# PacificBiosciences/pb-StarPhase

Measured on AMD Instinct MI355X. Metric: HiFi reads/sec diplotyped (HLA+CYP2D6), higher is better.
Workload: dtype int32; 1 GPU; BASELINE configs[1] + configs[2] as ONE sample per step: HLA-A/-B 10000 HiFi reads vs IMGT/HLA v0.14.1 (11,199 DNA alleles) + CYP2D6 2000 targeted reads (39 templates), the six configs[2] scenarios in turn; a new sample uploaded every step; reads -> diplotypes; hla_reads=10000, cyp2d6_reads=2000, cyp2d6_lanes=6, hla_lanes=2, cyp2d6_consensus=launch pairs

## Files before the change

### pb-starphase_amd/csrc/sp_consensus.hip

```cpp
#include "sp_internal.h"
#include <atomic>
#include <cstdlib>
#include "sp_wfa.hip.h"
#include <algorithm>
#include <cstddef>
#include <cstring>
#include <map>
#include <string>

namespace {

constexpr int CB = 64;
constexpr int CH = 32;
#ifndef SP_K8_WAVES
#define SP_K8_WAVES 8
#endif
#ifndef SP_K8_MIN_WAVES
#define SP_K8_MIN_WAVES 4
#endif
constexpr int CWAVES = SP_K8_WAVES;
#ifndef SP_K8_DBG_READS
#define SP_K8_DBG_READS 16384
#endif
#define SP_K8_DBG_LAUNCHES (4194304 / SP_K8_DBG_READS)
#ifndef SP_K8_CW
#define SP_K8_CW 256
#endif
constexpr int CW = SP_K8_CW;
static_assert(CW % 64 == 0 && CW >= 64 && CW <= 512, "window length");
constexpr int CWIN = 512;
constexpr int RWORDS = (2 * CW + 320) / 16;
constexpr int NQ = 56;
constexpr int NWORK = 4;
constexpr int MAXKIDS = 16;
constexpr int CLUSTER = 64;
constexpr int RSLICES = 16;
constexpr int RGROUP = 16;
constexpr int QSV = 2 * (CW + 1) * 5, QSL = 2 * CW * 4, QE = QSV + QSL + 2 * (CW + 1);
enum { F_ACTIVE = 1, F_FINISHED = 2, F_LOST = 4 };
enum { M_NONE = 0, M_INIT = 1, M_WINDOW = 2, M_EXPAND = 3 };

struct CWork {
    int32_t mode, done;
    int32_t node, in_slot;
    int32_t T, n, replay;
    int32_t dual, split_at;
    int32_t go[2];
    int32_t n_kids, pad;
    int32_t pre_go[2];
    int32_t kid_node[MAXKIDS];
    int8_t  kid_base[MAXKIDS][2];
    int8_t  kid_split[MAXKIDS];
    uint8_t spec[2][CW];
};
struct CNode {
    int32_t used, id, complete;
    int32_t T, cur;
    int32_t dual, split_at, stopped[2], len[2];
    int32_t n, a, q;
    int16_t have_out, la_valid;
    int32_t wcap;
    long long cost0;
    long long rest;
    long long rest_out;
    uint32_t ev[2][5];
    int32_t pex_n, pex_L;
    int8_t  pex_kid[MAXKIDS];
    int32_t pad_head[2];
    int32_t dc[CW + 1];
    uint8_t spec[2][CW];
    int32_t pad_[3];
    __device__ __forceinline__ long long cost_at(int j) const { return cost0 + (long long)dc[j]; }
};
constexpr int NODE_HEAD_WORDS = 40, NODE_WORDS = (int)(sizeof(CNode) / 4), NODE_TAPE_WORDS = NODE_WORDS - NODE_HEAD_WORDS;
static_assert(offsetof(CNode, dc) == 4 * NODE_HEAD_WORDS && sizeof(CNode) % 16 == 0, "CNode layout");
struct CSearch {
    int32_t threshold, farthest, next_id, best_node, inflight, max_queue, per_size, wo_constraint;
    int32_t windows, cut_windows, expansions, pops_mod;
    long long pops, best_final;
    long long ticks[4];
    long long step_ticks, gap_ticks, last_end;
    int32_t compound, compound_ok;
    long long gap_ctl_ticks;
    int32_t steps, side_windows, side_expansions, adopted;
#ifdef SP_K8_PF_PROBE
    int32_t pf_win, pf_replay, pf_exp, pf_pad;
    unsigned long long idle_mask;
#endif
};
struct ConsMeta { int32_t e, c0, flags, pad; };
struct ConsRes { int32_t best, dual, split_at, len1, len2, pad; };

constexpr int CMAXP = 24;
struct ConsParams {
    int n, first, first_block, n_blocks, rpw;
    int first_cluster, n_clusters;
    int acc_block;
    int min_count, delta, et, allow_dual, window, cmp_len; double min_af;
    int cap, cs;
    uint8_t* C;
    CWork* work; CSearch* srch; CNode* nodes;
    uint32_t* la;
    uint8_t* processed;
    uint8_t* out_cons;
    struct ConsRes* out_res; CSearch* out_srch;
};
struct ReadInfo { const uint32_t* w; const uint32_t* np; int n, off; int off0, pad; };
struct PlaceMemo { int valid, M, off, c0; uint32_t text[512 / 16 + 2]; };
template <int MAXP> struct ConsBatchT {
    ConsParams p[MAXP]; int n_prob;
    const ReadInfo* info;
    PlaceMemo* memo;
    uint16_t* H;
    ConsMeta* meta;
    unsigned long long* PV;
    uint32_t* PE;
    unsigned long long* PL;
    uint32_t* PC;
    uint32_t* PR;
    uint32_t* Q;
    unsigned long long* dbg;
    uint32_t* prog;
    unsigned long long* step_t;
    uint32_t* sync;
    uint32_t* ready;
    uint32_t step_cap;
    int total;
    int nside;
    int k8_compound;
};
template <> struct ConsBatchT<0> {
    const ConsParams* p; const int* block_prob; int n_prob;
    const ReadInfo* info; PlaceMemo* memo; uint16_t* H; ConsMeta* meta; unsigned long long* PV; uint32_t* PE; unsigned long long* PL; uint32_t* PC; uint32_t* PR; uint32_t* Q; unsigned long long* dbg; uint32_t* prog; unsigned long long* step_t; uint32_t* sync; uint32_t* ready; uint32_t step_cap; const int* cluster_prob; int total; int nside; int k8_compound;
};
struct ConsSetup { SeqSetView reads; const uint32_t* idx; const int32_t* offsets; int n, first, cmp_len, pad_; };

struct ReadView { const uint32_t* w; const uint32_t* np; int n; };

__device__ __forceinline__ int h_load(const uint16_t* H, size_t at) { const uint16_t v = H[at]; return v == 0xFFFF ? SP_NEG : (int)v; }
__device__ __forceinline__ void h_store(uint16_t* H, size_t at, int h) { H[at] = h < 0 ? (uint16_t)0xFFFF : (uint16_t)h; }

__device__ __forceinline__ int read_base(const ReadView& rv, int h) {
    const uint32_t sh = (uint32_t)(h & 15) << 1;
    if (rv.np && ((rv.np[h >> 4] >> sh) & 1u)) return 4;
    return (int)((rv.w[h >> 4] >> sh) & 3u);
}

__device__ __forceinline__ uint32_t vote_units(int d) { return d == 1 ? 12u : d == 2 ? 6u : d == 3 ? 4u : 3u; }

struct Dwfa { int H, e, c0, flags; };

template <class RB, class EXT>
__device__ __forceinline__ void dwfa_push_t(Dwfa& d, int n, RB rb, EXT extend, int T, int nb, int et, int lane) {
    const int k = lane - CH;
    if (d.H >= 0 && d.H + k == T - 1 && d.H < n && rb(d.H) == nb) d.H += 1;
    while (!__ballot(d.H >= 0 && d.H + k == T)) {
        const int c = d.H, up = spw::from_lower(d.H, SP_NEG), dn = spw::from_upper(d.H, SP_NEG);
        int best = SP_NEG;
        if (c >= 0 && c < n && c + k < T) best = c + 1;
        if (up >= 0 && up + k <= T && up + k >= 0 && up > best) best = up;
        if (dn >= 0 && dn < n && dn + 1 + k >= 0 && dn + 1 > best) best = dn + 1;
        if (!__ballot(best >= 0)) { d.flags |= F_LOST; return; }
        d.H = best; d.e += 1;
        extend(d, T);
    }
    if (et && __ballot(d.H == n)) d.flags |= F_FINISHED;
}

template <class EXT>
__device__ __forceinline__ void dwfa_catchup_t(Dwfa& d, int n, EXT extend, int span, int lane) {
    const int k = lane - CH;
    extend();
    while (!__ballot(d.H >= 0 && d.H + k == span)) {
        const int c = d.H, up = spw::from_lower(d.H, SP_NEG), dn = spw::from_upper(d.H, SP_NEG);
        int best = SP_NEG;
        if (c >= 0 && c < n && c + k < span) best = c + 1;
        if (up >= 0 && up + k <= span && up + k >= 0 && up > best) best = up;
        if (dn >= 0 && dn < n && dn + 1 + k >= 0 && dn + 1 > best) best = dn + 1;
        if (!__ballot(best >= 0)) { d.flags |= F_LOST; break; }
        d.H = best; d.e += 1;
        extend();
    }
}

template <class RB, class CA>
__device__ __noinline__ int find_start_scan(int rn, RB rb, CA ca, int off, int end, int W, int L, int lane) {
    const int ws = off - W > 0 ? off - W : 0, M = end - ws;
    if (L > rn) L = rn;
    if (M <= 0 || L <= 0 || off <= ws) return off < end ? off : end;
    unsigned long long peq[4];
    {
        const int code = lane < L ? rb(L - 1 - lane) : 7;
#pragma unroll
        for (int b = 0; b < 4; ++b) peq[b] = __ballot(code == b);
    }
    const int q = (M + CB - 1) / CB;
    const int jlo = lane * q + 1, jhi = min(M, jlo + q - 1);
    unsigned long long key = ~0ull;
    if (jlo <= M) {
        const unsigned long long ones = L == 64 ? ~0ull : ((1ull << L) - 1), top = 1ull << (L - 1);
        unsigned long long Pv = ones, Mv = 0;
        int score = L;
        const int centre = off - W / 2;
        for (int j = max(1, jlo - 2 * L); j <= jhi; ++j) {
            const int x = ca(end - j);
            const unsigned long long Eq = x == 0 ? peq[0] : x == 1 ? peq[1] : x == 2 ? peq[2] : peq[3];
            const unsigned long long Xv = Eq | Mv;
            const unsigned long long Xh = (((Eq & Pv) + Pv) ^ Pv) | Eq;
            unsigned long long Ph = Mv | ~(Xh | Pv), Mh = Pv & Xh;
            if (Ph & top) ++score; else if (Mh & top) --score;
            Ph <<= 1; Mh <<= 1;
            Pv = (Mh | ~(Xv | Ph)) & ones; Mv = Ph & Xv & ones;
            if (j >= jlo && j >= end - off) {
                const int p = end - j, dist = p > centre ? p - centre : centre - p;
                const unsigned long long kk = ((unsigned long long)score << 44) | ((unsigned long long)dist << 22) | (unsigned long long)p;
                key = kk < key ? kk : key;
            }
        }
    }
#pragma unroll
    for (int o = 32; o > 0; o >>= 1) { const unsigned long long other = __shfl_xor(key, o); key = other < key ? other : key; }
    return (int)(key & ((1ull << 22) - 1));
}

__device__ __noinline__ int find_start_diag(int pc, int L_, int M_, int off_, int end_, int W_, int lane, const uint32_t* tr_, uint8_t* score_) {
    const int L = __builtin_amdgcn_readfirstlane(L_), M = __builtin_amdgcn_readfirstlane(M_), off = __builtin_amdgcn_readfirstlane(off_), W = __builtin_amdgcn_readfirstlane(W_), end = __builtin_amdgcn_readfirstlane(end_);
    typedef __attribute__((address_space(3))) uint8_t lds_u8;
    spw::lds_cu32* tr = (spw::lds_cu32*)(uintptr_t)spw::lds_addr(tr_);
    lds_u8* score = (lds_u8*)(uintptr_t)spw::lds_addr(reinterpret_cast<const uint32_t*>(score_));
    const int i = lane + 1;
    int prev1 = i, prev2 = i;
    uint32_t tw = tr[0], tw_next = tw;
    const bool last_row = lane == L - 1;
    for (int d = 1; d <= L + M; ++d) {
        const int j = d - i;
        const int up = spw::from_lower(prev1, 0), diag = spw::from_lower(prev2, 0);
        if (j >= 1 && ((j - 1) & 15) == 0) tw = tw_next;
        int cur = i;
        if (j >= 1 && j <= M) {
            const int tc = (int)((tw >> (((j - 1) & 15) << 1)) & 3u);
            const int a = diag + (pc != tc ? 1 : 0), bmin = (up < prev1 ? up : prev1) + 1;
            cur = a < bmin ? a : bmin;
            if (last_row) score[j - 1] = (uint8_t)cur;
        }
        if (j >= 0 && (j & 15) == 0) tw_next = tr[j >> 4];
        prev2 = prev1; prev1 = cur;
    }
    spw::wave_lds_sync();
    const int centre = off - W / 2;
    unsigned long long key = ~0ull;
    for (int j = end - off + lane; j <= M; j += SP_WAVE) {
        if (j < 1) continue;
        const int p = end - j, dist = p > centre ? p - centre : centre - p;
        const unsigned long long kk = ((unsigned long long)score[j - 1] << 44) | ((unsigned long long)dist << 22) | (unsigned long long)p;
        key = kk < key ? kk : key;
    }
#pragma unroll
    for (int o = 32; o > 0; o >>= 1) { const unsigned long long other = __shfl_xor(key, o); key = other < key ? other : key; }
    return (int)(key & ((1ull << 22) - 1));
}

__device__ __noinline__ int find_start_diag2(int pa, int pb, int L_, int M_, int off_, int end_, int W_, int lane, const uint32_t* tr_, uint8_t* score_) {
    const int L = __builtin_amdgcn_readfirstlane(L_), M = __builtin_amdgcn_readfirstlane(M_), off = __builtin_amdgcn_readfirstlane(off_), W = __builtin_amdgcn_readfirstlane(W_), end = __builtin_amdgcn_readfirstlane(end_);
    typedef __attribute__((address_space(3))) uint8_t lds_u8;
    spw::lds_cu32* tr = (spw::lds_cu32*)(uintptr_t)spw::lds_addr(tr_);
    lds_u8* score = (lds_u8*)(uintptr_t)spw::lds_addr(reinterpret_cast<const uint32_t*>(score_));
    const int ia = 2 * lane + 1, ib = ia + 1;
    int a1 = ia, a2 = ia, b1 = ib, b2 = ib;
    uint32_t tw = tr[0], tw_next = tw;
    int t_prev = 0;
    for (int d = 1; d <= L + M; ++d) {
        const int ja = d - ia, jb = ja - 1;
        const int up_a = spw::from_lower(b1, 0), diag_a = spw::from_lower(b2, 0);
        if (ja >= 1 && ((ja - 1) & 15) == 0) tw = tw_next;
        int cur_a = ia, cur_b = ib, tc = 0;
        if (ja >= 1 && ja <= M) {
            tc = (int)((tw >> (((ja - 1) & 15) << 1)) & 3u);
            const int x = diag_a + (pa != tc ? 1 : 0), y = (up_a < a1 ? up_a : a1) + 1;
            cur_a = x < y ? x : y;
            if (ia == L) score[ja - 1] = (uint8_t)cur_a;
        }
        if (jb >= 1 && jb <= M) {
            const int x = a2 + (pb != t_prev ? 1 : 0), y = (a1 < b1 ? a1 : b1) + 1;
            cur_b = x < y ? x : y;
            if (ib == L) score[jb - 1] = (uint8_t)cur_b;
        }
        if (ja >= 0 && (ja & 15) == 0) tw_next = tr[ja >> 4];
        t_prev = tc;
        a2 = a1; a1 = cur_a; b2 = b1; b1 = cur_b;
    }
    spw::wave_lds_sync();
    const int centre = off - W / 2;
    unsigned long long key = ~0ull;
    for (int j = end - off + lane; j <= M; j += SP_WAVE) {
        if (j < 1) continue;
        const int p = end - j, dist = p > centre ? p - centre : centre - p;
        const unsigned long long kk = ((unsigned long long)score[j - 1] << 44) | ((unsigned long long)dist << 22) | (unsigned long long)p;
        key = kk < key ? kk : key;
    }
#pragma unroll
    for (int o = 32; o > 0; o >>= 1) { const unsigned long long other = __shfl_xor(key, o); key = other < key ? other : key; }
    return (int)(key & ((1ull << 22) - 1));
}

constexpr int ACT_CONS = 512;
constexpr int ACT_READ = 2 * (CW + 1) > 640 ? ((2 * (CW + 1) + 63) / 64) * 64 : 640;
struct ActScratch {
    uint8_t rcache[ACT_READ];
    uint32_t cpack[ACT_CONS / 16 + 2];
    uint32_t rpack[ACT_READ / 16 + 2];
    uint32_t npack[ACT_READ / 16 + 2];
    uint8_t score[ACT_CONS];
    const uint32_t* staged;
#ifdef SP_K8_TIMING
    long long tk[4];
#endif
};


template <class T> __device__ __forceinline__ T coh_load(const T* p) { return __hip_atomic_load(p, __ATOMIC_RELAXED, __HIP_MEMORY_SCOPE_AGENT); }
template <class T> __device__ __forceinline__ void coh_store(T* p, T v) { __hip_atomic_store(p, v, __ATOMIC_RELAXED, __HIP_MEMORY_SCOPE_AGENT); }
template <class T> __device__ __forceinline__ void put(T* p, T v, bool coh) { if (coh) coh_store(p, v); else *p = v; }

struct ConsAccess {
    const uint8_t* win; int w0; const uint8_t* C; int cap, split_at, i, ov_pos, ov_base;
    const uint32_t* pk;
    __device__ __forceinline__ bool word16(int pos, uint32_t& out) const {
        const int y = pos - w0;
        if (y < 0 || y + 16 > CWIN + CW || (ov_pos >= pos && ov_pos < pos + 16)) return false;
        out = __builtin_amdgcn_alignbit(pk[(y >> 4) + 1], pk[y >> 4], (uint32_t)(y & 15) << 1);
        return true;
    }
    __device__ __forceinline__ int at(int pos) const {
        if (pos == ov_pos) return ov_base;
        const int y = pos - w0;
        if ((unsigned)y < (unsigned)(CWIN + CW)) return (int)win[y];
        return (int)coh_load((i == 1 && pos < split_at) ? &C[pos] : &C[(size_t)i * cap + pos]);
    }
};

__device__ __noinline__ Dwfa activate_late(ReadView rv, ConsAccess cacc, ActScratch* Ap, PlaceMemo* memo, int off, int len, int window, int cmp_len, int et, int lane) {
    ActScratch& A = *Ap;
    typedef __attribute__((address_space(3))) uint32_t lds_u32;
    typedef __attribute__((address_space(3))) uint8_t lds_u8;
    lds_u32* const L_rpack = (lds_u32*)(uintptr_t)spw::lds_addr(A.rpack);
    lds_u32* const L_npack = (lds_u32*)(uintptr_t)spw::lds_addr(A.npack);
    lds_u32* const L_cpack = (lds_u32*)(uintptr_t)spw::lds_addr(A.cpack);
    lds_u32* const L_score32 = (lds_u32*)(uintptr_t)spw::lds_addr(reinterpret_cast<const uint32_t*>(A.score));
    lds_u8* const L_rcache = (lds_u8*)(uintptr_t)spw::lds_addr(reinterpret_cast<const uint32_t*>(A.rcache));
    Dwfa d;
#ifdef SP_K8_TIMING
    long long tq = wall_clock64();
#define ACT_T(k) do { const long long _n = wall_clock64(); if (lane == 0) A.tk[k] += _n - tq; tq = _n; } while (0)
#else
#define ACT_T(k) do { } while (0)
#endif
    auto ca = [&](int pos) { return cacc.at(pos); };
    const int ws = off - window > 0 ? off - window : 0;
    if (A.staged != rv.w) {
        const int rwords0 = ((rv.n < ACT_READ ? rv.n : ACT_READ) + 15) >> 4;
        for (int w = lane; w < ACT_READ / 16 + 2; w += SP_WAVE) { L_rpack[w] = w < rwords0 ? rv.w[w] : 0u; L_npack[w] = (rv.np && w < rwords0) ? rv.np[w] : 0u; }
        spw::wave_lds_sync();
        for (int x = lane; x < rv.n && x < ACT_READ; x += SP_WAVE) {
            const uint32_t sh = (uint32_t)(x & 15) << 1;
            L_rcache[x] = ((L_npack[x >> 4] >> sh) & 1u) ? (uint8_t)4 : (uint8_t)((L_rpack[x >> 4] >> sh) & 3u);
        }
        if (lane == 0) A.staged = rv.w;
    }
    spw::wave_lds_sync();
    auto rbc = [&](int h) { return h < ACT_READ ? (int)L_rcache[h] : read_base(rv, h); };
    ACT_T(0);
    {
        const int ws0 = off - window > 0 ? off - window : 0, M = len - ws0, L = cmp_len < rv.n ? cmp_len : rv.n;
        if (M <= 0 || L <= 0 || off <= ws0) d.c0 = off < len ? off : len;
        else if (M > ACT_CONS) d.c0 = find_start_scan(rv.n, rbc, ca, off, len, window, cmp_len, lane);
        else {
            for (int w = lane; w < ((M + 15) >> 4) + 1; w += SP_WAVE) {
                uint32_t word = 0, fw;
                const int left = M - w * 16;
                if (left <= 0) word = 0;
                else if (cacc.word16(len - w * 16 - 16, fw)) {
                    fw = ((fw >> 2) & 0x33333333u) | ((fw & 0x33333333u) << 2);
                    fw = ((fw >> 4) & 0x0F0F0F0Fu) | ((fw & 0x0F0F0F0Fu) << 4);
                    word = __builtin_bswap32(fw);
                    if (left < 16) word &= (1u << (left << 1)) - 1u;
                }
                else for (int b = 0; b < 16; ++b) { const int j = w * 16 + b + 1; if (j <= M) word |= (uint32_t)(ca(len - j) & 3) << (b << 1); }
                L_cpack[w] = word;
            }
            spw::wave_lds_sync();
            const int nw = ((M + 15) >> 4) + 1;
            PlaceMemo* mm = memo + cacc.i;
            auto peek = [](const int* q) { return __hip_atomic_load(q, __ATOMIC_RELAXED, __HIP_MEMORY_SCOPE_AGENT); };
            const uint32_t seen = lane < nw ? (uint32_t)peek(reinterpret_cast<const int*>(&mm->text[lane])) : 0u;
            const int m_c0 = peek(&mm->c0), m_valid = peek(&mm->valid), m_M = peek(&mm->M), m_off = peek(&mm->off);
            bool known = m_valid && m_M == M && m_off == off;
            if (known) known = __ballot(lane < nw && seen != L_cpack[lane]) == 0;
            ACT_T(0);
            int exact_c0 = -1;
            constexpr int LV_MAX = 12;
            const int lv_nd = M - L + 1 + 2 * LV_MAX;
            if (!known && rv.np == nullptr && M >= L && lv_nd <= 8 * SP_WAVE) {
                lds_u32* const ppack = L_score32;
                const int npw = (L + 15) >> 4;
                if (lane < 10) {
                    uint32_t pw = 0;
                    if (lane < npw) for (int b = 0; b < 16; ++b) { const int u = lane * 16 + b; if (u < L) pw |= (uint32_t)(rbc(L - 1 - u) & 3) << (b << 1); }
                    ppack[lane] = pw;
                }
                spw::wave_lds_sync();
                const int npl = (lv_nd + SP_WAVE - 1) / SP_WAVE, centre = off - window / 2;
                auto slide = [&](int r, int dd) {
                    const int lim = L < M - dd ? L : M - dd;
                    while (r < lim) {
                        const int t = r + dd;
                        const uint32_t pwd = __builtin_amdgcn_alignbit(ppack[(r >> 4) + 1], ppack[r >> 4], (uint32_t)(r & 15) << 1);
                        const uint32_t twd = __builtin_amdgcn_alignbit(L_cpack[(t >> 4) + 1], L_cpack[t >> 4], (uint32_t)(t & 15) << 1);
                        const uint32_t diff = pwd ^ twd;
                        const int same = diff ? (__builtin_ctz(diff) >> 1) : 16;
                        r += same;
                        if (same < 16) break;
                    }
                    return r < lim ? r : lim;
                };
                int reach[8];
#pragma unroll
                for (int c = 0; c < 8; ++c) {
                    const int x = c * SP_WAVE + lane, dd = x - LV_MAX;
                    reach[c] = (c < npl && x < lv_nd && dd >= 0 && dd <= M) ? slide(0, dd) : -1;
                }
                for (int e = 0; e <= LV_MAX; ++e) {
                    unsigned long long key = ~0ull;
#pragma unroll
                    for (int c = 0; c < 8; ++c) {
                        const int x = c * SP_WAVE + lane, dd = x - LV_MAX;
                        if (c < npl && x < lv_nd && dd >= 0 && dd + L >= len - off && dd <= M - L && reach[c] >= L) {
                            const int p = len - dd - L, dist = p > centre ? p - centre : centre - p;
                            const unsigned long long kk = ((unsigned long long)dist << 22) | (unsigned long long)p;
                            key = kk < key ? kk : key;
                        }
                    }
#pragma unroll
                    for (int o = 32; o > 0; o >>= 1) { const unsigned long long other = __shfl_xor(key, o); key = other < key ? other : key; }
                    if (key != ~0ull) { exact_c0 = (int)(key & ((1ull << 22) - 1)); break; }
                    if (e == LV_MAX) break;
                    int nxt[8];
#pragma unroll
                    for (int c = 0; c < 8; ++c) {
                        nxt[c] = -1;
                        if (c < npl) {
                            const int x = c * SP_WAVE + lane, dd = x - LV_MAX;
                            int left = __shfl_up(reach[c], 1), up = __shfl_down(reach[c], 1);
                            const int wrap_l = c > 0 ? __shfl(reach[c > 0 ? c - 1 : 0], SP_WAVE - 1) : -1, wrap_u = c + 1 < 8 ? __shfl(reach[c + 1 < 8 ? c + 1 : 7], 0) : -1;
                            if (lane == 0) left = wrap_l;
                            if (lane == SP_WAVE - 1) up = (c + 1 < npl) ? wrap_u : -1;
                            int best = reach[c] >= 0 ? reach[c] + 1 : -1;
                            if (up >= 0 && up + 1 > best) best = up + 1;
                            if (left > best) best = left;
                            if (x < lv_nd && dd <= M && best >= 0) {
                                const int lim = L < M - dd ? L : M - dd;
                                nxt[c] = slide(best < lim ? best : lim, dd);
                            }
                        }
                    }
#pragma unroll
                    for (int c = 0; c < 8; ++c) reach[c] = nxt[c];
                }
                spw::wave_lds_sync();
            }
            if (known) d.c0 = m_c0;
            else if (exact_c0 >= 0) {
                d.c0 = exact_c0;
                if (lane < nw) mm->text[lane] = L_cpack[lane];
                if (lane == 0) { mm->valid = 1; mm->M = M; mm->off = off; mm->c0 = d.c0; }
            }
            else {
                if (L <= SP_WAVE) d.c0 = find_start_diag(lane < L ? rbc(L - 1 - lane) : 7, L, M, off, len, window, lane, A.cpack, A.score);
                else d.c0 = find_start_diag2(2 * lane + 1 <= L ? rbc(L - 2 * lane - 1) : 7, 2 * lane + 2 <= L ? rbc(L - 2 * lane - 2) : 7, L, M, off, len, window, lane, A.cpack, A.score);
                if (lane < nw) mm->text[lane] = L_cpack[lane];
                if (lane == 0) { mm->valid = 1; mm->M = M; mm->off = off; mm->c0 = d.c0; }
            }
            spw::wave_lds_sync();
        }
    }
    ACT_T(1);
    d.H = lane == CH ? 0 : SP_NEG; d.e = 0; d.flags = F_ACTIVE | ((et && rv.n == 0) ? F_FINISHED : 0);
    const int c0 = d.c0, span = len - c0, cwinlen = len - ws;
    const bool packed = rv.np == nullptr && cwinlen <= ACT_CONS;
    if (span > 0 && !(d.flags & F_FINISHED) && !(et && rv.n <= span + CB) && packed) {
        for (int w = lane; w < ACT_CONS / 16 + 2; w += SP_WAVE) {
            uint32_t word = 0;
            const int left = cwinlen - w * 16;
            if (left <= 0) word = 0;
            else if (cacc.word16(ws + w * 16, word)) { if (left < 16) word &= (1u << (left << 1)) - 1u; }
            else { word = 0; for (int b = 0; b < 16; ++b) { const int x = w * 16 + b; if (x < cwinlen) word |= (uint32_t)(ca(ws + x) & 3) << (b << 1); } }
            L_cpack[w] = word;
        }
        spw::wave_lds_sync();
        ACT_T(2);
        const int kk = lane - CH, cbase = c0 - ws;
        dwfa_catchup_t(d, rv.n, [&]() {
            for (;;) {
                int left = rv.n - d.H; { const int l2 = span - (d.H + kk); left = l2 < left ? l2 : left; }
                const bool go = d.H >= 0 && left > 0;
                int nm = 0;
                if (go) {
                    const int pr = d.H, pc = cbase + d.H + kk;
                    const uint32_t a = __builtin_amdgcn_alignbit(L_rpack[(pr >> 4) + 1], L_rpack[pr >> 4], (uint32_t)(pr & 15) << 1);
                    const uint32_t b = __builtin_amdgcn_alignbit(L_cpack[(pc >> 4) + 1], L_cpack[pc >> 4], (uint32_t)(pc & 15) << 1);
                    const uint32_t x = a ^ b, mm = (x | (x >> 1)) & 0x55555555u;
                    nm = mm ? (__builtin_ctz(mm) >> 1) : 16;
                    nm = nm < left ? nm : left;
                    d.H += nm;
                }
                if (!__ballot(go && nm == 16 && left > 16)) break;
            }
        }, span, lane);
    } else if (span > 0 && !(d.flags & F_FINISHED) && !(et && rv.n <= span + CB)) {
        const int kk = lane - CH;
        dwfa_catchup_t(d, rv.n, [&]() {
            for (;;) {
                bool go = d.H >= 0 && d.H < rv.n && d.H + kk < span;
                if (go) { const int x = rbc(d.H); go = x < 4 && x == ca(d.c0 + d.H + kk); }
                if (!__ballot(go)) break;
                if (go) d.H += 1;
            }
        }, span, lane);
    } else {
        for (int Tl = 1; Tl <= span; ++Tl) {
            if (d.flags & (F_FINISHED | F_LOST)) break;
            dwfa_push_t(d, rv.n, rbc, [&](Dwfa& x, int Tc) {
                const int kk = lane - CH;
                for (;;) {
                    bool go = x.H >= 0 && x.H < rv.n && x.H + kk < Tc;
                    if (go) { const int b = rbc(x.H); go = b < 4 && b == ca(x.c0 + x.H + kk); }
                    if (!__ballot(go)) break;
                    if (go) x.H += 1;
                }
            }, Tl, ca(c0 + Tl - 1), et, lane);
        }
    }
    ACT_T(3);
    return d;
}

constexpr int KID_LA_KIDS = 4, KID_LA = CW / KID_LA_KIDS;
#ifndef SP_K8_KID_W0
#define SP_K8_KID_W0 32
#endif
constexpr int KID_W0 = SP_K8_KID_W0 < KID_LA ? SP_K8_KID_W0 : KID_LA;
#ifndef SP_K8_RAMP
#define SP_K8_RAMP 2
#endif
#ifndef SP_K8_KID_CALM
#define SP_K8_KID_CALM 6
#endif
constexpr int KID_CALM = SP_K8_KID_CALM;
struct UsedWords {
    int used, has_la, a_end, b_end, total;
    __device__ __forceinline__ UsedWords(int mode, int n, int n_kids) {
        used = mode == M_EXPAND ? n_kids : (mode == M_WINDOW ? n + 1 + n_kids : 1);
        has_la = mode != M_EXPAND || n_kids <= KID_LA_KIDS;
        a_end = 2 * used * 5; b_end = a_end + (has_la ? QSL : 0); total = b_end + 2 * used;
    }
    __device__ __forceinline__ int at(int c) const {
        if (c < a_end) { const int i = c / (used * 5), rem = c % (used * 5); return (i * (CW + 1) + rem / 5) * 5 + rem % 5; }
        if (c < b_end) return QSV + (c - a_end);
        const int r = c - b_end;
        return r < used ? QSV + QSL + r : QSV + QSL + (CW + 1) + (r - used);
    }
};
template <class BT> __device__ __forceinline__ uint32_t block_word(const BT& B, size_t blk, int o) {
    constexpr int EV = 2 * (CW + 1), EL = 2 * CW, EC = CW + 1;
    if (o < QSV) { const int e = o / 5, f = o % 5; return f < 4 ? (uint32_t)((B.PV[blk * EV + e] >> (16 * f)) & 0xFFFFull) : B.PE[blk * EV + e]; }
    if (o < QSV + QSL) { const int e = (o - QSV) / 4, f = (o - QSV) % 4; return (uint32_t)((B.PL[blk * EL + e] >> (16 * f)) & 0xFFFFull); }
    if (o < QSV + QSL + EC) return B.PC[blk * EC + (o - QSV - QSL)];
    return B.PR[blk * EC + (o - QSV - QSL - EC)];
}
#ifndef SP_K8_WRAMP0
#define SP_K8_WRAMP0 64
#endif
constexpr int WRAMP0 = SP_K8_WRAMP0;
constexpr int BULK_MARGIN_PLACED = 2;
constexpr int BULK_MARGIN = 8;
#ifndef SP_K8_AUTO_BATCHES
#define SP_K8_AUTO_BATCHES 1
#endif
constexpr int PERSIST_AUTO_BATCHES = SP_K8_AUTO_BATCHES;
#ifndef SP_K8_LIGHT
#define SP_K8_LIGHT 64
#endif
constexpr int PERSIST_LIGHT = SP_K8_LIGHT;
#ifndef SP_K8_DIRECT_BLOCKS
#define SP_K8_DIRECT_BLOCKS (680 * 8 / SP_K8_WAVES)
#endif
constexpr int DIRECT_BLOCKS = SP_K8_DIRECT_BLOCKS;
constexpr int32_t SP_K8_AGAIN = -777;
constexpr int PERSIST_BLOCKS = 128 * 8 / CWAVES;

template <int MAXP> __device__ __forceinline__ int block_problem(const ConsBatchT<MAXP>& B, int block) {
    int pi = 0;
    if constexpr (MAXP == 0) pi = B.block_prob[block];
    else {
#pragma unroll
        for (int i = 1; i < MAXP; ++i) if (i < B.n_prob && block >= B.p[i].first_block) pi = i;
    }
    return pi;
}
template <int MAXP> __device__ __forceinline__ int block_problem(const ConsBatchT<MAXP>& B) { return block_problem<MAXP>(B, (int)blockIdx.x); }

__device__ __forceinline__ size_t state_plane(int node, int slot, int cons) { return (size_t)((node * 2 + slot) * 2 + cons); }

__device__ __forceinline__ int read_cost(const Dwfa& a0, const Dwfa& a1, bool dualrun) {
    int c = -1;
    if (a0.flags & F_ACTIVE) c = a0.e;
    if (dualrun && (a1.flags & F_ACTIVE) && (c < 0 || a1.e < c)) c = a1.e;
    return c < 0 ? 0 : c;
}

template <int MAXP>
__device__ __forceinline__ void cons_step_body(const ConsBatchT<MAXP>& B, const int wrow) {
    __shared__ unsigned long long lv[2][CW + 1];
    __shared__ uint32_t le[2][CW + 1];
    __shared__ unsigned long long ll[2][CW];
    __shared__ uint32_t lc[CW + 1], lr[CW + 1];
    __shared__ uint8_t cwin[2][CWIN + CW];
    __shared__ uint32_t rwin[CWAVES][2][RWORDS + 2];
    __shared__ uint32_t cpk[2][(CWIN + CW) / 16 + 2];
    __shared__ ActScratch act[CWAVES];
    __shared__ CWork wk_s;
    const int pi = block_problem<MAXP>(B);
    const ConsParams P = B.p[pi];
    const bool coh = B.sync != nullptr;
    if (coh) {
        for (int x = threadIdx.x; x < (int)(sizeof(CWork) / 4); x += blockDim.x) ((uint32_t*)&wk_s)[x] = coh_load(((const uint32_t*)P.work) + x);
        __syncthreads();
    }
    const CWork* Wp = coh ? &wk_s : P.work + wrow;
    const int mode = Wp->mode;
    if (P.work->done || mode == M_NONE) return;
    if (wrow > 0 && P.n_blocks > DIRECT_BLOCKS) return;
    if (B.step_t && threadIdx.x == 0) atomicMin(&B.step_t[2 * pi], (unsigned long long)wall_clock64());
    const int lane = threadIdx.x & 63, wave = threadIdx.x >> 6;
    const int T = Wp->T, n = (mode == M_WINDOW || mode == M_EXPAND) ? Wp->n : 0;
    const int pre = mode == M_EXPAND ? n : 0;
    const int node = Wp->node, in_slot = Wp->in_slot;
    const int dual_in = Wp->dual, split_at = Wp->split_at;
    const int go0 = Wp->go[0], go1 = Wp->go[1];
    const int n_kids = (mode == M_EXPAND || mode == M_WINDOW) ? Wp->n_kids : 0;
    const uint8_t* Cn = P.C + (size_t)node * 2 * P.cs;
    for (int x = threadIdx.x; x < 2 * (CW + 1); x += blockDim.x) { (&lv[0][0])[x] = 0; (&le[0][0])[x] = 0; }
    for (int x = threadIdx.x; x < 2 * CW; x += blockDim.x) (&ll[0][0])[x] = 0;
    for (int x = threadIdx.x; x < CW + 1; x += blockDim.x) { lc[x] = 0; lr[x] = 0; }
    const int w0 = T - CWIN;
    for (int x = threadIdx.x; x < 2 * (CWIN + CW); x += blockDim.x) {
        const int i = x / (CWIN + CW), y = x % (CWIN + CW), pos = w0 + y;
        uint8_t v = 0;
        if (pos >= T) v = (pos - T < n) ? Wp->spec[dual_in ? i : 0][pos - T] : 0;
        else if (pos >= 0) v = coh_load((i == 1 && dual_in && pos >= split_at) ? &Cn[(size_t)P.cs + pos] : &Cn[pos]);
        cwin[i][y] = v;
    }
    __syncthreads();
    constexpr int CPW = (CWIN + CW) / 16 + 2;
    for (int x = threadIdx.x; x < 2 * CPW; x += blockDim.x) {
        const int i = x / CPW, w = x % CPW;
        uint32_t word = 0;
        for (int b = 0; b < 16; ++b) { const int y = w * 16 + b; if (y < CWIN + n) word |= (uint32_t)(cwin[i][y] & 3u) << (b << 1); }
        cpk[i][w] = word;
    }
    __syncthreads();
    const size_t plane = (size_t)B.total;
    for (int rr = 0; rr < P.rpw; ++rr) {
        const int r = (((int)blockIdx.x - P.first_block) * CWAVES + wave) * P.rpw + rr;
        if (r >= P.n) break;
        const size_t g = (size_t)P.first + r;
#ifdef SP_K8_TIMING
        const long long wt0 = wall_clock64();
        if (lane == 0) { act[wave].tk[0] = act[wave].tk[1] = act[wave].tk[2] = act[wave].tk[3] = 0; }
#endif
        const ReadInfo ri = B.info[g];
        ReadView rv; rv.w = ri.w; rv.np = ri.np; rv.n = ri.n;
        if (lane == 0) act[wave].staged = nullptr;
        Dwfa d0, d1;
        d0.H = SP_NEG; d0.e = 0; d0.c0 = 0; d0.flags = 0; d1 = d0;
        if (mode == M_INIT) {
            if (ri.off < 0) { d0.flags = F_ACTIVE | ((P.et && rv.n == 0) ? F_FINISHED : 0); d0.H = lane == CH ? 0 : SP_NEG; }
        } else {
            const size_t p0 = state_plane(node, in_slot, 0) * plane + g;
            const ConsMeta m0 = B.meta[p0];
            d0.H = h_load(B.H, p0 * CB + lane); d0.e = m0.e; d0.c0 = m0.c0; d0.flags = m0.flags;
            if (dual_in) {
                const size_t p1 = state_plane(node, in_slot, 1) * plane + g;
                const ConsMeta m1 = B.meta[p1];
                d1.H = h_load(B.H, p1 * CB + lane); d1.e = m1.e; d1.c0 = m1.c0; d1.flags = m1.flags;
            }
        }
        int rbase = 0;
        {
            int lo = 0x7FFFFFFF;
            if (d0.flags & F_ACTIVE) { const int x = T - d0.c0 - CB; lo = x < lo ? x : lo; }
            if (dual_in && (d1.flags & F_ACTIVE)) { const int x = T - d1.c0 - CB; lo = x < lo ? x : lo; }
            if (lo == 0x7FFFFFFF || lo < 0) lo = 0;
            rbase = (lo >> 4) << 4;
            const int w_first = rbase >> 4, w_last = (rv.n + 15) >> 4;
            if (lane < RWORDS + 2) {
                const int w = w_first + lane;
                rwin[wave][0][lane] = w <= w_last + 1 ? rv.w[w] : 0u;
                rwin[wave][1][lane] = (rv.np && w <= w_last + 1) ? rv.np[w] : 0u;
            }
            spw::wave_lds_sync();
        }
        auto rb = [&](int h) -> int {
            const int x = h - rbase;
            if ((unsigned)x < (unsigned)(RWORDS * 16)) {
                const uint32_t sh = (uint32_t)(x & 15) << 1;
                if ((rwin[wave][1][x >> 4] >> sh) & 1u) return 4;
                return (int)((rwin[wave][0][x >> 4] >> sh) & 3u);
            }
            return read_base(rv, h);
        };
        auto vote = [&](const Dwfa& a, const Dwfa& o, bool dualrun, int i, int col, int slot) {
            if (!(a.flags & F_ACTIVE) || (a.flags & (F_FINISHED | F_LOST))) return;
            if (dualrun && (o.flags & F_ACTIVE) && !(o.flags & F_LOST) && o.e < a.e) return;
            const int Tl = col - a.c0, k = lane - CH;
            const bool tip = a.H >= 0 && a.H + k == Tl;
            const int code = (tip && a.H < rv.n) ? rb(a.H) : 5;
            int dc = 0; unsigned long long word = 0;
#pragma unroll
            for (int b = 0; b < 4; ++b) { const bool s = __ballot(code == b) != 0; dc += s; word |= s ? (1ull << (16 * b)) : 0ull; }
            const bool ended = __ballot(tip) != 0 && __ballot(code == 4) == 0;
            if (lane == 0) {
                if (dc) atomicAdd(&lv[i][slot], word * vote_units(dc));
                else if (ended) atomicAdd(&le[i][slot], 12u);
            }
        };
        bool use_pk = mode == M_WINDOW;
        auto extender = [&](const ConsAccess& cacc, int i) {
            return [&cacc, i, &rb, wave, rbase, w0, lane, &use_pk, &rv](Dwfa& d, int Tc) {
                const int k = lane - CH;
                for (;;) {
                    int left = rv.n - d.H; { const int l2 = Tc - (d.H + k); left = l2 < left ? l2 : left; }
                    const bool go = d.H >= 0 && left > 0;
                    int nm = 0; bool more = false;
                    if (go) {
                        const int xr = d.H - rbase, yc = d.c0 + d.H + k - w0;
                        if (use_pk && xr >= 0 && xr < RWORDS * 16 && yc >= 0 && yc < CWIN + CW) {
                            const uint32_t a = __builtin_amdgcn_alignbit(rwin[wave][0][(xr >> 4) + 1], rwin[wave][0][xr >> 4], (uint32_t)(xr & 15) << 1);
                            const uint32_t nn = __builtin_amdgcn_alignbit(rwin[wave][1][(xr >> 4) + 1], rwin[wave][1][xr >> 4], (uint32_t)(xr & 15) << 1);
                            const uint32_t b = __builtin_amdgcn_alignbit(cpk[i][(yc >> 4) + 1], cpk[i][yc >> 4], (uint32_t)(yc & 15) << 1);
                            const uint32_t xo = a ^ b, mm = ((xo | (xo >> 1)) | nn) & 0x55555555u;
                            nm = mm ? (__builtin_ctz(mm) >> 1) : 16;
                            nm = nm < left ? nm : left;
                            more = nm == 16 && left > 16;
                        } else {
                            const int x = rb(d.H);
                            nm = (x < 4 && x == cacc.at(d.c0 + d.H + k)) ? 1 : 0;
                            more = nm == 1 && left > 1;
                        }
                        d.H += nm;
                    }
                    if (!__ballot(more)) break;
                }
            };
        };
        auto column = [&](Dwfa& a0, Dwfa& a1, bool dualrun, int g0, int g1, int nb0, int nb1, int len, const ConsAccess& c0a, const ConsAccess& c1a) {
            if (g0) {
                if (a0.flags & F_ACTIVE) { if (!(a0.flags & (F_FINISHED | F_LOST))) dwfa_push_t(a0, rv.n, rb, extender(c0a, c0a.i), len - a0.c0, nb0, P.et, lane); }
                else if (ri.off == len) { a0 = activate_late(rv, c0a, &act[wave], B.memo + 2 * ((size_t)wrow * plane + g), ri.off0, len, P.window, P.cmp_len, P.et, lane); spw::wave_lds_sync(); }
            }
            if (dualrun && g1) {
                if (a1.flags & F_ACTIVE) { if (!(a1.flags & (F_FINISHED | F_LOST))) dwfa_push_t(a1, rv.n, rb, extender(c1a, c1a.i), len - a1.c0, nb1, P.et, lane); }
                else if (ri.off == len) { a1 = activate_late(rv, c1a, &act[wave], B.memo + 2 * ((size_t)wrow * plane + g), ri.off0, len, P.window, P.cmp_len, P.et, lane); spw::wave_lds_sync(); }
            }
            if (dualrun) {
                const int both = (a0.flags & F_ACTIVE) && (a1.flags & F_ACTIVE) && !(a0.flags & F_LOST) && !(a1.flags & F_LOST);
                if (both) {
                    if (a0.e > a1.e + P.delta) a0.flags |= F_LOST;
                    else if (a1.e > a0.e + P.delta) a1.flags |= F_LOST;
                }
            }
        };
        auto final_extra = [&](const Dwfa& a0, const Dwfa& a1, bool dualrun, int len0, int len1) -> int {
            if (P.et) return 0;
            int best = -1;
#pragma unroll
            for (int i = 0; i < 2; ++i) {
                if (i == 1 && !dualrun) continue;
                const Dwfa& a = i ? a1 : a0;
                if (!(a.flags & F_ACTIVE)) continue;
                int s = a.e;
                if (!(a.flags & F_LOST)) {
                    const int k = lane - CH, Tl = (i ? len1 : len0) - a.c0;
                    int rest = (a.H >= 0 && a.H + k == Tl) ? rv.n - a.H : (1 << 30);
#pragma unroll
                    for (int o = 32; o > 0; o >>= 1) { const int other = __shfl_xor(rest, o); rest = other < rest ? other : rest; }
                    if (rest < (1 << 30)) s += rest;
                }
                if (best < 0 || s < best) best = s;
            }
            return best < 0 ? 0 : best - read_cost(a0, a1, dualrun);
        };
        auto store = [&](const Dwfa& a, int nd, int slot, int i) {
            const size_t p = state_plane(nd, slot, i) * plane + g;
            if (lane == 0) { ConsMeta m; m.e = a.e; m.c0 = a.c0; m.flags = a.flags; m.pad = 0; B.meta[p] = m; }
            h_store(B.H, p * CB + lane, a.H);
        };
        ConsAccess ca0, ca1;
        ca0.win = &cwin[0][0]; ca0.w0 = w0; ca0.C = Cn; ca0.cap = P.cs; ca0.split_at = split_at; ca0.i = 0; ca0.ov_pos = -1; ca0.ov_base = 0; ca0.pk = &cpk[0][0];
        ca1 = ca0; ca1.win = &cwin[1][0]; ca1.i = 1; ca1.pk = &cpk[1][0];

        auto win_pass = [&](Dwfa& d0, Dwfa& d1, const bool dualrun, const int go0, const int go1, const int n, const bool quiet) {
        if (!quiet && mode == M_INIT) { vote(d0, d1, false, 0, 0, 0); }
        auto match_run = [&](int x0, int i, int j0, int len) -> int {
            if (x0 < 0 || x0 + len + 16 > RWORDS * 16) return 0;
            const int nblk = (len + 15) >> 4;
            const int blk = lane < nblk ? lane : 0;
            const int x = x0 + (blk << 4), jj = j0 + (blk << 4);
            const uint32_t a = __builtin_amdgcn_alignbit(rwin[wave][0][(x >> 4) + 1], rwin[wave][0][x >> 4], (uint32_t)(x & 15) << 1);
            const uint32_t nn = __builtin_amdgcn_alignbit(rwin[wave][1][(x >> 4) + 1], rwin[wave][1][x >> 4], (uint32_t)(x & 15) << 1);
            const uint32_t b = __builtin_amdgcn_alignbit(cpk[i][CWIN / 16 + (jj >> 4) + 1], cpk[i][CWIN / 16 + (jj >> 4)], (uint32_t)(jj & 15) << 1);
            const uint32_t xr = a ^ b, mm = ((xr | (xr >> 1)) | nn) & 0x55555555u;
            int run = mm ? (__builtin_ctz(mm) >> 1) : 16;
            const int room = len - (blk << 4);
            run = run < room ? run : room;
            const unsigned long long stop = __ballot(lane < nblk && run < 16 && run < room);
            if (!stop) return len;
            const int t = __builtin_ctzll(stop);
            return (t << 4) + __builtin_amdgcn_readlane(run, t);
        };
        static_assert(sizeof(((ActScratch*)nullptr)->rcache) >= 2 * (CW + 1), "edit-count profile");
        uint16_t* const ewp = reinterpret_cast<uint16_t*>(act[wave].rcache);
        auto bulk_push = [&](Dwfa& d, int i, const ConsAccess& cacc, int Tl0, int cols, int jbase) -> bool {
            auto ext = extender(cacc, i);
            const int k = lane - CH, span = Tl0 + cols;
            int reached = Tl0;
            const bool record = jbase >= 0;
            if (record && lane == 0) ewp[jbase] = (uint16_t)d.e;
            for (;;) {
                ext(d, span);
                int far = spw::wave_max(d.H >= 0 ? d.H + k : -1);
                far = far < span ? far : span;
                if (record) for (int c = reached + 1 + lane; c <= far; c += SP_WAVE) ewp[jbase + c - Tl0] = (uint16_t)d.e;
                reached = far > reached ? far : reached;
                if (reached >= span) break;
                const int c = d.H, up = spw::from_lower(d.H, SP_NEG), dn = spw::from_upper(d.H, SP_NEG);
                int best = SP_NEG;
                if (c >= 0 && c < rv.n && c + k < span) best = c + 1;
                if (up >= 0 && up + k <= span && up + k >= 0 && up > best) best = up;
                if (dn >= 0 && dn < rv.n && dn + 1 + k >= 0 && dn + 1 > best) best = dn + 1;
                if (!__ballot(best >= 0)) return false;
                d.H = best; d.e += 1;
            }
            spw::wave_lds_sync();
            return true;
        };
        int bulk = -1;
        int wsave_H = 0, wsave_e = 0, wsave_j = 0;
        int want_bulk = BULK_MARGIN;
        int j = 0;
#ifdef SP_K8_TIMING
        int slow_cols = 0, multi_tip = 0, zero_run = 0, fast_iters = 0;
        long long tb_fast = 0, tb_col = 0, tb_vote = 0, tb_mark = 0, tb_bulk = 0;
#ifdef SP_K8_DBG_PARTS
        const long long tb_pre = wall_clock64() - wt0;
#define K8_T0() tb_mark = wall_clock64()
#define K8_T(acc) do { const long long _n = wall_clock64(); acc += _n - tb_mark; tb_mark = _n; } while (0)
#else
#define K8_T0() tb_mark = clock64()
#define K8_T(acc) do { const long long _n = clock64(); acc += _n - tb_mark; tb_mark = _n; } while (0)
#endif
#else
#define K8_T0() do { } while (0)
#define K8_T(acc) do { } while (0)
#endif
        while (j < n) {
            K8_T0();
            if (want_bulk > 0) {
                const int margin = want_bulk; want_bulk = 0;
                if (!quiet && mode == M_WINDOW && dualrun && go0 && go1 && n - j >= 8 && (d0.flags & F_ACTIVE) && (d1.flags & F_ACTIVE) &&
                    !((d0.flags | d1.flags) & (F_FINISHED | F_LOST)) && (d0.e >= d1.e + margin || d1.e >= d0.e + margin)) {
                    const int wi = d0.e > d1.e ? 0 : 1;
                    Dwfa& w = wi ? d1 : d0;
                    const int Tl0 = T + j - w.c0;
                    if ((!P.et || rv.n > Tl0 + (n - j) + CB) && w.e < 60000) {
                        wsave_H = w.H; wsave_e = w.e; wsave_j = j;
                        if (bulk_push(w, wi, wi ? ca1 : ca0, Tl0, n - j, j)) { bulk = wi; w.e = wsave_e; }
                        else { w.H = wsave_H; w.e = wsave_e; }
                    }
                }
            }
            K8_T(tb_bulk);
            int m = n - j;
            int tl0 = -1, th0 = 0, tl1 = -1, th1 = 0;
#pragma unroll
            for (int i = 0; i < 2; ++i) {
                if (i == 1 && !dualrun) continue;
                if (!(i ? go1 : go0)) continue;
                if (i == bulk) continue;
                if (m == 0) continue;
                const Dwfa& a = i ? d1 : d0;
                if (a.flags & F_ACTIVE) {
                    if (a.flags & (F_FINISHED | F_LOST)) continue;
                    const int Tl = T + j - a.c0, k = lane - CH;
                    const unsigned long long tm = __ballot(a.H >= 0 && a.H + k == Tl);
                    if (__builtin_popcountll(tm) != 1) {
#ifdef SP_K8_TIMING
                        multi_tip += 1;
#endif
                        m = 0; continue; }
                    const int tl = __builtin_ctzll(tm), h = __builtin_amdgcn_readlane(a.H, tl);
                    int room = rv.n - h; room = room < m ? room : m;
                    const int run = room > 0 ? match_run(h - rbase, i, j, room) : 0;
                    m = run < m ? run : m;
                    if (i) { tl1 = tl; th1 = h; } else { tl0 = tl; th0 = h; }
                } else if (ri.off > T + j && ri.off <= T + n) {
                    const int before = ri.off - T - 1 - j;
                    m = before < m ? before : m;
                }
            }
            if (m > 0) {
#pragma unroll
                for (int i = 0; i < 2; ++i) {
                    const int tl = i ? tl1 : tl0, th = i ? th1 : th0;
                    if (tl < 0) continue;
                    Dwfa& a = i ? d1 : d0; const Dwfa& o = i ? d0 : d1;
                    bool speaks = true;
                    if (dualrun && (o.flags & F_ACTIVE) && !(o.flags & F_LOST) && o.e < a.e) speaks = false;
                    if (speaks && !quiet) for (int x = lane + 1; x <= m; x += SP_WAVE) {
                        const int pos = th + x;
                        if (pos < rv.n) { const int code = rb(pos); if (code < 4) atomicAdd(&lv[i][j + x], 12ull << (16 * code)); }
                        else if (!P.et) atomicAdd(&le[i][j + x], 12u);
                    }
                    if (lane == tl) a.H += m;
                    if (P.et && th + m == rv.n) a.flags |= F_FINISHED;
                }
                if (bulk >= 0) {
                    Dwfa& w = bulk ? d1 : d0; const Dwfa& b = bulk ? d0 : d1;
                    if (!(w.flags & F_LOST)) {
                        int hit = -1;
                        if (!(b.flags & F_LOST)) {
                            const int thr = b.e + P.delta;
                            for (int base = 0; base < m; base += SP_WAVE) {
                                const int x = j + 1 + base + lane;
                                const unsigned long long over = __ballot(x <= j + m && (int)ewp[x] > thr);
                                if (over) { hit = j + 1 + base + __builtin_ctzll(over); break; }
                            }
                        }
                        if (hit >= 0) { w.flags |= F_LOST; w.e = (int)ewp[hit]; } else w.e = (int)ewp[j + m];
                    }
                }
                j += m;
                K8_T(tb_fast);
#ifdef SP_K8_TIMING
                fast_iters += 1;
#endif
                continue;
            }
            K8_T(tb_fast);
#ifdef SP_K8_TIMING
            slow_cols += 1;
#endif
            const int before = read_cost(d0, d1, dualrun);
            const int active_before = (d0.flags & F_ACTIVE) + (d1.flags & F_ACTIVE);
            if (bulk >= 0) {
                Dwfa& w = bulk ? d1 : d0; const Dwfa& b = bulk ? d0 : d1;
                if (!(w.flags & F_LOST)) w.e = (int)ewp[j + 1];
                column(d0, d1, dualrun, bulk != 0, bulk != 1, cwin[0][CWIN + j], cwin[1][CWIN + j], T + j + 1, ca0, ca1);
                if (!(w.flags & F_LOST) && ((b.flags & F_LOST) || w.e <= b.e)) {
                    w.H = wsave_H; w.e = wsave_e;
                    (void)bulk_push(w, bulk, bulk ? ca1 : ca0, T + wsave_j - w.c0, j + 1 - wsave_j, -1);
                    bulk = -1;
                }
            } else
                column(d0, d1, dualrun, go0, go1, cwin[0][CWIN + j], cwin[1][CWIN + j], T + j + 1, ca0, ca1);
            const int grow = read_cost(d0, d1, dualrun) - before;
            if (grow && lane == 0 && !quiet) atomicAdd(&lc[j + 1], (uint32_t)grow);
            K8_T(tb_col);
            if (!quiet && go0 && bulk != 0) vote(d0, d1, dualrun, 0, T + j + 1, j + 1);
            if (!quiet && dualrun && go1 && bulk != 1) vote(d1, d0, dualrun, 1, T + j + 1, j + 1);
            K8_T(tb_vote);
            j += 1;
            if (bulk < 0 && (d0.flags & F_ACTIVE) + (d1.flags & F_ACTIVE) != active_before) want_bulk = BULK_MARGIN_PLACED;
        }
#pragma unroll
        for (int i = 0; i < 2; ++i) {
            if (quiet) continue;
            if (mode == M_WINDOW && n_kids > 0) continue;
            if (i == 1 && !dualrun) continue;
            if (mode != M_INIT && !(i ? go1 : go0)) continue;
            const Dwfa& a = i ? d1 : d0; const Dwfa& o = i ? d0 : d1;
            if (!(a.flags & F_ACTIVE) || (a.flags & (F_FINISHED | F_LOST))) continue;
            if (dualrun && (o.flags & F_ACTIVE) && !(o.flags & F_LOST) && o.e < a.e) continue;
            const int Tl = T + n - a.c0, k = lane - CH;
            unsigned long long tips = __ballot(a.H >= 0 && a.H + k == Tl && a.H < rv.n);
            for (int cnt = 0; tips && cnt < 2; ++cnt) {
                const int tl = __builtin_ctzll(tips); tips &= tips - 1;
                const int h = __builtin_amdgcn_readlane(a.H, tl);
                for (int x = lane; x < CW - 1 && h + 1 + x < rv.n; x += SP_WAVE) {
                    const int b = rb(h + 1 + x);
                    if (b < 4) atomicAdd(&ll[i][x], 1ull << (16 * b));
                }
            }
        }
        {
            const int len0 = go0 || mode == M_INIT ? T + n : coh_load(&P.nodes[node].len[0]), len1 = go1 ? T + n : coh_load(&P.nodes[node].len[1]);
            const int extra = final_extra(d0, d1, dualrun, len0, len1);
            if (extra && lane == 0 && !quiet) atomicAdd(&lr[n], (uint32_t)extra);
        }
        if (!quiet) {
            const int out_slot = mode == M_INIT ? in_slot : in_slot ^ 1;
            store(d0, node, out_slot, 0);
            if (dualrun) store(d1, node, out_slot, 1);
        }
        spw::wave_lds_sync();
#ifdef SP_K8_TIMING
#ifdef SP_K8_DBG_PARTS
        if (!quiet && B.dbg && lane == 0 && Wp->pad < SP_K8_DBG_LAUNCHES / 2 && g < SP_K8_DBG_READS) {
#else
        if (!quiet && B.dbg && lane == 0 && Wp->pad < SP_K8_DBG_LAUNCHES && g < SP_K8_DBG_READS) {
#endif
            const unsigned long long dt = (unsigned long long)(wall_clock64() - wt0);
            const unsigned long long placed = ri.off > T && ri.off <= T + n;
            auto cl = [](long long v, long long cap) { return (unsigned long long)(v > cap ? cap : v); };
#ifdef SP_K8_DBG_PARTS
            B.dbg[((size_t)Wp->pad * SP_K8_DBG_READS + g) * 2] = cl((long long)dt, 0xFFFFFF) | (cl(slow_cols, 511) << 24) | (cl(multi_tip, 511) << 33) | (placed << 42) | ((unsigned long long)mode << 43) |
                                                            (cl(n, 511) << 45);
            B.dbg[((size_t)Wp->pad * SP_K8_DBG_READS + g) * 2 + 1] = cl(tb_pre >> 1, 1023) | (cl(tb_fast >> 1, 4095) << 10) | (cl(tb_col >> 1, 4095) << 22) | (cl(tb_vote >> 1, 4095) << 34) |
                                                            (cl(tb_bulk >> 1, 4095) << 46) | (cl(fast_iters, 63) << 58);
            (void)tb_pre;
#elif defined(SP_K8_DBG_EDITS)
            B.dbg[(size_t)Wp->pad * SP_K8_DBG_READS + g] = cl((long long)dt, 0xFFFFFF) | (cl((act[wave].tk[0] + act[wave].tk[2]) >> 5, 511) << 24) | (cl(act[wave].tk[1] >> 5, 511) << 33) | (placed << 42) |
                                                            ((unsigned long long)mode << 43) | (cl(n, 511) << 45) | (cl(act[wave].tk[3] >> 5, 1023) << 54);
#else
            B.dbg[(size_t)Wp->pad * SP_K8_DBG_READS + g] = cl((long long)dt, 0xFFFFFF) | (cl(slow_cols, 511) << 24) | (cl(multi_tip, 511) << 33) | (placed << 42) | ((unsigned long long)mode << 43) |
                                                            (cl(n, 511) << 45) | (cl(tb_col >> 10, 1023) << 54);
#endif
            (void)tb_fast; (void)tb_vote; (void)tb_bulk; (void)fast_iters;
        }
#endif
        };
        auto expand_kids = [&](const Dwfa& d0, const Dwfa& d1, const int TB, const int s0) {
            const int base_cost = read_cost(d0, d1, dual_in != 0);
            for (int k = 0; k < n_kids; ++k) {
                Dwfa e0 = d0, e1 = d1;
                const int kb0 = Wp->kid_base[k][0], kb1 = Wp->kid_base[k][1], ksplit = Wp->kid_split[k];
                if (ksplit) e1 = e0;
                const bool kdual = dual_in || ksplit;
                ConsAccess k0 = ca0, k1 = ca1;
                k0.ov_pos = kb0 >= 0 ? TB : -1; k0.ov_base = kb0;
                k1.ov_pos = kb1 >= 0 ? TB : -1; k1.ov_base = kb1;
                if (ksplit) { k1.i = 0; }
                column(e0, e1, kdual, kb0 >= 0, kb1 >= 0, kb0, kb1, TB + 1, k0, k1);
                if (kb0 >= 0) vote(e0, e1, kdual, 0, TB + 1, s0 + k);
                if (kdual && kb1 >= 0) vote(e1, e0, kdual, 1, TB + 1, s0 + k);
                if (n_kids <= KID_LA_KIDS && (P.n < 256 || (r & 3) == 0)) {
#pragma unroll
                    for (int i = 0; i < 2; ++i) {
                        if (i == 1 && !kdual) continue;
                        if ((i ? kb1 : kb0) < 0) continue;
                        const Dwfa& a = i ? e1 : e0; const Dwfa& o = i ? e0 : e1;
                        if (!(a.flags & F_ACTIVE) || (a.flags & (F_FINISHED | F_LOST))) continue;
                        if (kdual && (o.flags & F_ACTIVE) && !(o.flags & F_LOST) && o.e < a.e) continue;
                        const int Tl = TB + 1 - a.c0, kd = lane - CH;
                        unsigned long long tips = __ballot(a.H >= 0 && a.H + kd == Tl && a.H < rv.n);
                        unsigned long long* const kl = &ll[0][0] + (size_t)(k * 2 + i) * KID_LA;
                        for (int cnt = 0; tips && cnt < 2; ++cnt) {
                            const int tl = __builtin_ctzll(tips); tips &= tips - 1;
                            const int h = __builtin_amdgcn_readlane(a.H, tl);
                            for (int x = lane; x < KID_LA - 1 && h + 1 + x < rv.n; x += SP_WAVE) {
                                const int b = rb(h + 1 + x);
                                if (b < 4) atomicAdd(&kl[x], 1ull << (16 * b));
                            }
                        }
                    }
                }
                const int grow = read_cost(e0, e1, kdual) - base_cost;
                const int len0 = kb0 >= 0 ? TB + 1 : (go0 ? TB : coh_load(&P.nodes[node].len[0]));
                const int len1 = kb1 >= 0 ? TB + 1 : (go1 ? TB : coh_load(&P.nodes[node].len[1]));
                const int extra = final_extra(e0, e1, kdual, len0, len1);
                if (lane == 0) { if (grow) atomicAdd(&lc[s0 + k], (uint32_t)grow); if (extra) atomicAdd(&lr[s0 + k], (uint32_t)extra); }
                const int kn = Wp->kid_node[k];
                store(e0, kn, 0, 0);
                if (kdual) store(e1, kn, 0, 1);
            }
            spw::wave_lds_sync();
        };
        if (mode == M_EXPAND) {
            if (pre > 0) { use_pk = true; win_pass(d0, d1, dual_in != 0, Wp->pre_go[0], Wp->pre_go[1], pre, true); use_pk = false; }
            expand_kids(d0, d1, T + pre, 0);
#ifdef SP_K8_DBG_PARTS
            if (B.dbg && lane == 0 && Wp->pad < SP_K8_DBG_LAUNCHES / 2 && g < SP_K8_DBG_READS) {
                const unsigned long long dt = (unsigned long long)(wall_clock64() - wt0);
                B.dbg[((size_t)Wp->pad * SP_K8_DBG_READS + g) * 2] = (dt > 0xFFFFFF ? 0xFFFFFFull : dt) | ((unsigned long long)(n_kids > 511 ? 511 : n_kids) << 24) | (3ull << 43) | ((unsigned long long)(pre > 511 ? 511 : pre) << 45);
                B.dbg[((size_t)Wp->pad * SP_K8_DBG_READS + g) * 2 + 1] = 0;
            }
#endif
            continue;
        }

        win_pass(d0, d1, dual_in != 0, go0, go1, n, false);
        if (n_kids > 0) {
            use_pk = false;
            if (lane == 0) act[wave].staged = nullptr;
            spw::wave_lds_sync();
            expand_kids(d0, d1, T + n, n + 1);
        }
    }
    __syncthreads();
    const UsedWords uw(mode, n, n_kids);
    if (P.n_blocks <= DIRECT_BLOCKS) {
        const size_t blk = (size_t)P.acc_block + (size_t)wrow;
        for (int x = threadIdx.x; x < 2 * uw.used; x += blockDim.x) {
            const int i = x / uw.used, e = i * (CW + 1) + x % uw.used;
            const unsigned long long v = (&lv[0][0])[e]; const uint32_t w = (&le[0][0])[e];
            if (v) atomicAdd(&B.PV[blk * 2 * (CW + 1) + e], v);
            if (w) atomicAdd(&B.PE[blk * 2 * (CW + 1) + e], w);
        }
        if (uw.has_la) for (int x = threadIdx.x; x < 2 * CW; x += blockDim.x) { const unsigned long long v = (&ll[0][0])[x]; if (v) atomicAdd(&B.PL[blk * 2 * CW + x], v); }
        for (int x = threadIdx.x; x < uw.used; x += blockDim.x) {
            if (lc[x]) atomicAdd(&B.PC[blk * (CW + 1) + x], lc[x]);
            if (lr[x]) atomicAdd(&B.PR[blk * (CW + 1) + x], lr[x]);
        }
        if (B.step_t && threadIdx.x == 0) atomicMax(&B.step_t[2 * pi + 1], (unsigned long long)wall_clock64());
        return;
    }
    for (int x = threadIdx.x; x < 2 * uw.used; x += blockDim.x) {
        const int i = x / uw.used, e = i * (CW + 1) + x % uw.used;
        B.PV[(size_t)blockIdx.x * 2 * (CW + 1) + e] = (&lv[0][0])[e];
        B.PE[(size_t)blockIdx.x * 2 * (CW + 1) + e] = (&le[0][0])[e];
    }
    if (uw.has_la) for (int x = threadIdx.x; x < 2 * CW; x += blockDim.x) B.PL[(size_t)blockIdx.x * 2 * CW + x] = (&ll[0][0])[x];
    for (int x = threadIdx.x; x < uw.used; x += blockDim.x) { B.PC[(size_t)blockIdx.x * (CW + 1) + x] = lc[x]; B.PR[(size_t)blockIdx.x * (CW + 1) + x] = lr[x]; }
    if (B.step_t && threadIdx.x == 0) atomicMax(&B.step_t[2 * pi + 1], (unsigned long long)wall_clock64());
}

template <int MAXP>
__global__ void __launch_bounds__(CWAVES * SP_WAVE, SP_K8_MIN_WAVES) cons_step_kernel(ConsBatchT<MAXP> B) { cons_step_body<MAXP>(B, (int)blockIdx.y); }
template <int MAXP>
__global__ void __launch_bounds__(CWAVES * SP_WAVE, 2) cons_step_wide_kernel(ConsBatchT<MAXP> B) { cons_step_body<MAXP>(B, (int)blockIdx.y); }

template <int MAXP>
__global__ void __launch_bounds__(512) cons_reduce_kernel(ConsBatchT<MAXP> B) {
    const int cluster = (int)blockIdx.x / RSLICES, slice = (int)blockIdx.x % RSLICES;
    int pi = 0;
    if constexpr (MAXP == 0) pi = B.cluster_prob[cluster];
    else {
#pragma unroll
        for (int i = 1; i < MAXP; ++i) if (i < B.n_prob && cluster >= B.p[i].first_cluster) pi = i;
    }
    const ConsParams P = B.p[pi];
    const int mode = P.work->mode;
    if (P.work->done || mode == M_NONE) return;
    const UsedWords uw(mode, mode == M_WINDOW ? P.work->n : 0, mode == M_EXPAND ? P.work->n_kids : 0);
    if (P.n_blocks <= DIRECT_BLOCKS) return;
    const int cl = cluster - P.first_cluster;
    const int members = P.n_blocks - cl * CLUSTER < CLUSTER ? P.n_blocks - cl * CLUSTER : CLUSTER;
    const size_t blk0 = (size_t)P.first_block + (size_t)cl * CLUSTER;
    constexpr int NG = CLUSTER / RGROUP;
    const int per = (uw.total + RSLICES - 1) / RSLICES;
    const int c_lo = slice * per, c_hi = c_lo + per < uw.total ? c_lo + per : uw.total;
    for (int idx = threadIdx.x; idx < (c_hi - c_lo) * NG; idx += blockDim.x) {
        const int o = uw.at(c_lo + idx / NG), m0 = (idx % NG) * RGROUP;
        uint32_t v[RGROUP];
#pragma unroll
        for (int m = 0; m < RGROUP; ++m) v[m] = m0 + m < members ? block_word(B, blk0 + m0 + m, o) : 0u;
        uint32_t sum = 0;
#pragma unroll
        for (int m = 0; m < RGROUP; ++m) sum += v[m];
#pragma unroll
        for (int d = 1; d < NG; d <<= 1) sum += __shfl_xor(sum, d);
        if (idx % NG == 0) B.Q[(size_t)cluster * QE + o] = sum;
    }
}

struct ColVotes { uint32_t w[4], end; };

__device__ __forceinline__ int col_candidates(const uint32_t* w5, int col, int cap, int et, int min_count, double min_af, int out[4]) {
    if (col >= cap) return 0;
    int order[4] = { 0, 1, 2, 3 };
#pragma unroll
    for (int a = 0; a < 4; ++a)
#pragma unroll
        for (int b = a + 1; b < 4; ++b) if (w5[order[b]] > w5[order[a]]) { const int t = order[a]; order[a] = order[b]; order[b] = t; }
    const uint32_t w1 = w5[order[0]], total = w5[0] + w5[1] + w5[2] + w5[3];
    const bool go = et ? w1 > 0 : (total > w5[4] && w1 > 0);
    if (!go) return 0;
    uint32_t need = 12u * (uint32_t)min_count; if (w1 < need) need = w1;
    int n = 0;
    out[n++] = order[0];
#pragma unroll
    for (int a = 1; a < 4; ++a) { const uint32_t w = w5[order[a]]; if (w > 0 && w >= need && (double)w >= min_af * (double)total) out[n++] = order[a]; }
    return n;
}

__device__ __forceinline__ int col_candidates_packed(const uint32_t* w5, int col, int cap, int et, int min_count, double min_af, uint32_t& packed) {
    packed = 0;
    if (col >= cap) return 0;
    uint32_t wa = w5[0], wb = w5[1], wc = w5[2], wd = w5[3]; uint32_t ca = 0, cb = 1, cc = 2, cd = 3;
#define SP_CSW(x, y, cx, cy) if (y > x) { const uint32_t tw_ = x; x = y; y = tw_; const uint32_t tc_ = cx; cx = cy; cy = tc_; }
    SP_CSW(wa, wb, ca, cb) SP_CSW(wa, wc, ca, cc) SP_CSW(wa, wd, ca, cd) SP_CSW(wb, wc, cb, cc) SP_CSW(wb, wd, cb, cd) SP_CSW(wc, wd, cc, cd)
#undef SP_CSW
    const uint32_t total = wa + wb + wc + wd;
    const bool go = et ? wa > 0 : (total > w5[4] && wa > 0);
    if (!go) return 0;
    uint32_t need = 12u * (uint32_t)min_count; if (wa < need) need = wa;
    int n = 1; packed = ca;
    const double floor_w = min_af * (double)total;
    if (wb > 0 && wb >= need && (double)wb >= floor_w) { packed |= cb << (2 * n); ++n; }
    if (wc > 0 && wc >= need && (double)wc >= floor_w) { packed |= cc << (2 * n); ++n; }
    if (wd > 0 && wd >= need && (double)wd >= floor_w) { packed |= cd << (2 * n); ++n; }
    return n;
}

template <int MAXP>
__device__ __forceinline__ void cons_control_body(const ConsBatchT<MAXP>& B) {
    extern __shared__ uint8_t proc[];
    __shared__ uint32_t acc[QE];
    uint32_t (*sv)[CW + 1][5] = reinterpret_cast<uint32_t (*)[CW + 1][5]>(acc);
    uint32_t (*sl)[CW][4] = reinterpret_cast<uint32_t (*)[CW][4]>(acc + QSV);
    uint32_t* sc = acc + QSV + QSL; uint32_t* sr = sc + (CW + 1);
    __shared__ CNode nh[NQ];
    __shared__ CWork wks[NWORK];
    __shared__ CSearch ss;
    __shared__ int copy_from[NWORK], copy_len[NWORK], need_la[NWORK], replay_of[NWORK];
    struct KidCopy { int from, T, n, nk, dual; int8_t node[4], b0[4], b1[4], sp[4]; uint8_t spec[2][CW]; };
    static_assert(KID_LA_KIDS <= 4, "KidCopy");
    __shared__ KidCopy kcopy[NWORK];
    const int pi = blockIdx.x;
    const ConsParams P = B.p[pi];
    const int tid = threadIdx.x;
    const bool coh = B.sync != nullptr;
    const int nside = (coh || P.n_blocks > DIRECT_BLOCKS) ? 0 : (B.nside < NWORK - 1 ? B.nside : NWORK - 1);
    const int n_orders = 1 + nside;
    CWork& wk = wks[0];
    const long long tk0 = wall_clock64();
    for (int x = tid; x < NQ * NODE_HEAD_WORDS; x += blockDim.x)
        ((uint32_t*)&nh[x / NODE_HEAD_WORDS])[x % NODE_HEAD_WORDS] = ((const uint32_t*)&P.nodes[x / NODE_HEAD_WORDS])[x % NODE_HEAD_WORDS];
    for (int x = tid; x < n_orders * (int)(sizeof(CWork) / 4); x += blockDim.x) ((uint32_t*)wks)[x] = ((const uint32_t*)P.work)[x];
    for (int x = tid; x < (int)(sizeof(CSearch) / 4); x += blockDim.x) ((uint32_t*)&ss)[x] = ((const uint32_t*)P.srch)[x];
    const int proc_words = (P.cap + 2 + 3) / 4;
    for (int x = tid; x < proc_words; x += blockDim.x) ((uint32_t*)proc)[x] = ((const uint32_t*)P.processed)[x];
    for (int x = tid; x < QE; x += blockDim.x) acc[x] = 0;
    if (tid < NWORK) { copy_from[tid] = -1; copy_len[tid] = 0; need_la[tid] = -1; replay_of[tid] = -1; kcopy[tid].nk = 0; if (tid >= n_orders) wks[tid].mode = M_NONE; }
    __syncthreads();
    if (wk.done) return;
    auto tape_word_used = [](const CNode& x, int w) {
        if (!x.used) return false;
        if (w == 0) return true;
        if (x.n <= 0) return false;
        if (w < CW + 1) return w <= x.n;
        const int sw = w - (CW + 1);
        return sw < 2 * (CW / 4) && (sw % (CW / 4)) * 4 < x.n;
    };
    for (int x = tid; x < NQ * NODE_TAPE_WORDS; x += blockDim.x) {
        const int k = x / NODE_TAPE_WORDS, w = x % NODE_TAPE_WORDS;
        if (tape_word_used(nh[k], w)) ((uint32_t*)&nh[k])[NODE_HEAD_WORDS + w] = ((const uint32_t*)&P.nodes[k])[NODE_HEAD_WORDS + w];
    }
    auto load_votes = [&](const int w) {
        const int mode_in = wks[w].mode, n_in = (mode_in == M_WINDOW || mode_in == M_EXPAND) ? wks[w].n : 0;
        if (mode_in == M_NONE) return;
        const UsedWords uw(mode_in, n_in, wks[w].n_kids);
        if (P.n_blocks <= DIRECT_BLOCKS) {
            const int u = uw.used, ev = 2 * u, el = uw.has_la ? 2 * CW : 0, E = ev + ev + el + u + u;
            const size_t blk = (size_t)P.acc_block + (size_t)w;
            for (int c = tid; c < E; c += blockDim.x) {
                if (c < ev || (c >= 2 * ev && c < 2 * ev + el)) {
                    const bool exact = c < ev;
                    const int e = exact ? (c / u) * (CW + 1) + c % u : c - 2 * ev;
                    unsigned long long* src = exact ? B.PV + blk * 2 * (CW + 1) + e : B.PL + blk * 2 * CW + e;
                    const unsigned long long sum = coh ? __hip_atomic_exchange(src, 0ull, __ATOMIC_RELAXED, __HIP_MEMORY_SCOPE_AGENT) : *src;
                    if (sum) {
                        if (!coh) *src = 0ull;
                        uint32_t* dst = exact ? acc + e * 5 : acc + QSV + e * 4;
#pragma unroll
                        for (int f = 0; f < 4; ++f) dst[f] = (uint32_t)((sum >> (16 * f)) & 0xFFFFull);
                    }
                } else {
                    uint32_t* src; uint32_t* dst;
                    if (c < 2 * ev) { const int cc = c - ev, e = (cc / u) * (CW + 1) + cc % u; src = B.PE + blk * 2 * (CW + 1) + e; dst = acc + e * 5 + 4; }
                    else if (c < 2 * ev + el + u) { const int e = c - 2 * ev - el; src = B.PC + blk * (CW + 1) + e; dst = acc + QSV + QSL + e; }
                    else { const int e = c - 2 * ev - el - u; src = B.PR + blk * (CW + 1) + e; dst = acc + QSV + QSL + (CW + 1) + e; }
                    const uint32_t sum = coh ? __hip_atomic_exchange(src, 0u, __ATOMIC_RELAXED, __HIP_MEMORY_SCOPE_AGENT) : *src;
                    if (sum) { if (!coh) *src = 0u; *dst = sum; }
                }
            }
        } else {
            const int parts = P.n_clusters;
            for (int c = tid; c < uw.total; c += blockDim.x) {
                const int o = uw.at(c);
                uint32_t sum = 0;
                for (int c0 = 0; c0 < parts; c0 += 8) {
                    uint32_t v[8];
#pragma unroll
                    for (int q = 0; q < 8; ++q) v[q] = c0 + q < parts ? B.Q[(size_t)(P.first_cluster + c0 + q) * QE + o] : 0u;
#pragma unroll
                    for (int q = 0; q < 8; ++q) sum += v[q];
                }
                acc[o] = sum;
            }
        }
    };
    const int lane = tid & (SP_WAVE - 1);
    auto cands = [&](const uint32_t* w5, int col, int out[4]) { return col_candidates(w5, col, P.cap, P.et, P.min_count, P.min_af, out); };
    auto node_free = [&](int k) {
        const int np = nh[k].pex_n;
        for (int j = 0; j < np; ++j) { CNode& c = nh[nh[k].pex_kid[j]]; c.used = 0; c.complete = 0; }
        nh[k].pex_n = 0; nh[k].used = 0; nh[k].complete = 0;
    };
    uint8_t* Cb = P.C;
    int la_fresh = -1;
    auto trim_queue = [&]() {
        for (;;) {
            const bool waits = lane < NQ && nh[lane].used == 1 && !nh[lane].complete;
            const int wlen = waits ? nh[lane].T + nh[lane].q : 0;
            const bool live = waits && wlen >= ss.threshold;
            if (waits && !live) node_free(lane);
            if (__builtin_popcountll(__ballot(live)) <= ss.max_queue) break;
            int shortest = live ? wlen : 0x7FFFFFFF;
#pragma unroll
            for (int o = 32; o > 0; o >>= 1) { const int other = __shfl_xor(shortest, o); shortest = other < shortest ? other : shortest; }
            if (lane == 0) ss.threshold = shortest + 1;
            spw::wave_lds_sync();
        }
    };
    auto adopt = [&](const int parent, const int n_kids, const bool kids_wait, auto kid) {
        const int others = __builtin_popcountll(__ballot(lane < NQ && nh[lane].used == 1 && !nh[lane].complete)) - 1 - (kids_wait ? n_kids : 0);
        const int kid_w0 = others <= KID_CALM ? KID_LA : KID_W0;
        if (lane < n_kids) {
            CNode& c = nh[kid(lane)];
            c.used = 1; c.id = ss.next_id + lane;
            c.wcap = n_kids <= KID_LA_KIDS ? kid_w0 : WRAMP0;
        }
        spw::wave_lds_sync();
        if (lane == 0) {
            ss.next_id += n_kids;
            nh[parent].pex_n = 0;
            node_free(parent);
            ss.expansions += 1;
        }
        spw::wave_lds_sync();
        trim_queue();
    };
    struct Plan { int kind, nk, nc0, nc1, cut, L; uint32_t cd0, cd1; bool ends; };
    auto cands_p = [&](const uint32_t* w5, int col, uint32_t& packed) { return col_candidates_packed(w5, col, P.cap, P.et, P.min_count, P.min_af, packed); };
    auto plan_of = [&](const CNode& x) -> Plan {
        Plan p;
        const bool has = x.q > 0 || x.n > 0, stood = !has || (x.a == x.n && x.have_out);
        p.cut = stood ? -1 : x.a;
        p.L = (has && stood ? x.T + x.n : x.T) + (p.cut > 0 ? p.cut : 0);
        p.nc0 = p.nc1 = 0; p.cd0 = p.cd1 = 0; p.ends = false;
        if (!x.stopped[0]) { p.nc0 = cands_p(x.ev[0], p.L, p.cd0); p.ends = p.ends || p.nc0 == 0; }
        if (x.dual && !x.stopped[1]) { p.nc1 = cands_p(x.ev[1], p.L, p.cd1); p.ends = p.ends || p.nc1 == 0; }
        if (!x.dual) p.nk = p.nc0 + (P.allow_dual ? p.nc0 * (p.nc0 - 1) / 2 : 0);
        else p.nk = (p.nc0 || p.nc1) ? (p.nc0 ? p.nc0 : 1) * (p.nc1 ? p.nc1 : 1) : 0;
        p.kind = p.nk == 0 ? 0 : p.nk == 1 ? 1 : 2;
        return p;
    };
    auto kid_of = [&](const Plan& pl, const int dual, const int k, int& b0, int& b1, int& sp) {
        auto code = [](uint32_t packed, int j) { return (int)((packed >> (2 * j)) & 3u); };
        sp = 0;
        if (!dual) {
            if (k < pl.nc0) { b0 = code(pl.cd0, k); b1 = -1; }
            else { int pa = 0, pb = 1; for (int j = pl.nc0; j < k; ++j) if (++pb >= pl.nc0) { ++pa; pb = pa + 1; } b0 = code(pl.cd0, pa); b1 = code(pl.cd0, pb); sp = 1; }
        } else { const int n1 = pl.nc1 ? pl.nc1 : 1, a2 = k / n1, b2 = k - a2 * n1; b0 = pl.nc0 ? code(pl.cd0, a2) : -1; b1 = pl.nc1 ? code(pl.cd1, b2) : -1; }
    };
    auto kids_from_sums = [&](const CWork& w, const int mark, const int L, const long long par_cost, const int my_j, const int s0) {
        if (my_j >= 0) {
            const CNode& par = nh[w.node];
            const int k = my_j;
            CNode& c = nh[w.kid_node[k]];
            c.used = mark; c.complete = 0; c.id = 0; c.T = L + 1; c.cur = 0; c.pex_n = 0; c.pex_L = 0;
            c.dual = par.dual || w.kid_split[k]; c.split_at = w.kid_split[k] ? L : par.split_at;
#pragma unroll
            for (int i = 0; i < 2; ++i) {
                const bool was_going = (i == 0 || par.dual) && !par.stopped[i];
                int st = par.stopped[i], ln = par.len[i];
                if (w.kid_base[k][i] >= 0) { st = 0; ln = L + 1; }
                else if (was_going) { st = 1; ln = L; }
                c.stopped[i] = st; c.len[i] = ln;
            }
            if (!c.dual) c.stopped[1] = 1;
            c.n = c.a = c.q = 0; c.have_out = 0; c.la_valid = w.n_kids <= KID_LA_KIDS ? 1 : 0; c.wcap = WRAMP0;
            c.cost0 = par_cost + (long long)sc[s0 + k]; c.dc[0] = 0; c.rest = sr[s0 + k]; c.rest_out = 0;
            for (int i = 0; i < 2; ++i) for (int bq = 0; bq < 5; ++bq) c.ev[i][bq] = sv[i][s0 + k][bq];
        }
        if (w.n_kids <= KID_LA_KIDS) {
            const uint32_t* flat = &sl[0][0][0];
            for (int y = lane; y < w.n_kids * 2 * KID_LA * 4; y += SP_WAVE) {
                const int k = y / (2 * KID_LA * 4), i = (y / (KID_LA * 4)) & 1, xb = y % (KID_LA * 4);
                P.la[(size_t)w.kid_node[k] * 2 * CW * 4 + (size_t)i * CW * 4 + xb] = flat[y];
            }
            __threadfence_block();
        }
        spw::wave_lds_sync();
    };
    auto take_result = [&](const int w) {
        const CWork& wo = wks[w];
        const int mode_in = wo.mode, n_in = (mode_in == M_WINDOW || mode_in == M_EXPAND) ? wo.n : 0;
        const bool side = w > 0;
        if (mode_in == M_INIT) {
            la_fresh = wo.node;
            CNode& x = nh[wo.node];
            if (lane == 0) {
                x.used = 1; x.id = ss.next_id++; x.complete = 0; x.T = 0; x.cur = wo.in_slot; x.dual = 0; x.split_at = -1;
                x.stopped[0] = 0; x.stopped[1] = 1; x.len[0] = x.len[1] = 0; x.n = x.a = x.q = 0; x.have_out = 0; x.la_valid = 1; x.wcap = CW;
                x.cost0 = 0; x.dc[0] = 0; x.rest = sr[0]; x.rest_out = 0; x.pex_n = 0; x.pex_L = 0;
            }
            if (lane < 10) x.ev[lane / 5][lane % 5] = sv[lane / 5][0][lane % 5];
            for (int y = lane; y < 2 * CW * 4; y += SP_WAVE) P.la[(size_t)wo.node * 2 * CW * 4 + y] = (&sl[0][0][0])[y];
        } else if (mode_in == M_WINDOW) {
            CNode& x = nh[wo.node];
            const int n = n_in, T = wo.T;
            int a = n;
            if (!wo.replay && n > 1) {
                for (int base = 0; base < n; base += SP_WAVE) {
                    const int col = base + lane;
                    bool ok = true;
                    if (col >= 1 && col < n) {
#pragma unroll
                        for (int i = 0; i < 2; ++i) {
                            if (i == 1 && !x.dual) continue;
                            if (!wo.go[i]) continue;
                            int c4[4];
                            const int nc = cands(sv[i][col], T + col, c4);
                            if (nc != 1 || c4[0] != wo.spec[i][col]) ok = false;
                        }
                    }
                    const unsigned long long bad = __ballot(!ok);
                    if (bad) { a = base + __builtin_ctzll(bad); break; }
                }
            }
            for (int col = lane; col < a; col += SP_WAVE) {
#pragma unroll
                for (int i = 0; i < 2; ++i) if ((i == 0 || x.dual) && wo.go[i]) put(&Cb[((size_t)wo.node * 2 + i) * P.cs + T + col], wo.spec[i][col], coh);
            }
            if (!wo.replay) {
                long long carry = 0;
                for (int base = 0; base < a; base += SP_WAVE) {
                    const int col = base + lane;
                    long long c = col < a ? (long long)sc[col + 1] : 0;
#pragma unroll
                    for (int o = 1; o < SP_WAVE; o <<= 1) { const long long up = __shfl_up(c, o); if (lane >= o) c += up; }
                    if (col < a) x.dc[col + 1] = (int32_t)(carry + c);
                    carry += __shfl(c, SP_WAVE - 1);
                }
                for (int col = lane; col < n; col += SP_WAVE) { x.spec[0][col] = wo.spec[0][col]; x.spec[1][col] = wo.spec[1][col]; }
            }
            if (lane < 10) x.ev[lane / 5][lane % 5] = sv[lane / 5][a][lane % 5];
            if (lane == 0) {
                ss.windows += 1; if (a < n) ss.cut_windows += 1;
                x.n = n; x.a = wo.replay ? n : a;
                x.have_out = (a == n) ? (wo.n_kids > 0 ? 2 : 1) : 0;
                if (a == n) x.rest_out = sr[n];
            }
            if (wo.n_kids > 0) {
                spw::wave_lds_sync();
                bool take = a == n && B.k8_compound != 2;
                int my_j = -1, nk = 0;
                if (take) {
                    Plan pl;
                    pl.nc0 = pl.nc1 = 0; pl.cd0 = pl.cd1 = 0; bool ends = false;
                    if (!x.stopped[0]) { pl.nc0 = cands_p(sv[0][n], T + n, pl.cd0); ends = ends || pl.nc0 == 0; }
                    if (x.dual && !x.stopped[1]) { pl.nc1 = cands_p(sv[1][n], T + n, pl.cd1); ends = ends || pl.nc1 == 0; }
                    if (!x.dual) nk = pl.nc0 + (P.allow_dual ? pl.nc0 * (pl.nc0 - 1) / 2 : 0);
                    else nk = (pl.nc0 || pl.nc1) ? (pl.nc0 ? pl.nc0 : 1) * (pl.nc1 ? pl.nc1 : 1) : 0;
                    take = !ends && nk >= 2 && nk <= wo.n_kids;
                    if (take) {
                        bool found = true;
                        if (lane < nk) {
                            int b0, b1, sp;
                            kid_of(pl, x.dual, lane, b0, b1, sp);
                            for (int j = 0; j < wo.n_kids; ++j) if (wo.kid_base[j][0] == b0 && wo.kid_base[j][1] == b1 && wo.kid_split[j] == sp) my_j = j;
                            found = my_j >= 0;
                        }
                        take = __ballot(!found) == 0;
                    }
                }
                if (take) {
                    kids_from_sums(wo, 2, T + n, x.cost_at(n), lane < nk ? my_j : -1, n + 1);
                    for (int k = 0; k < nk; ++k) { const int j = __builtin_amdgcn_readlane(my_j, k); if (lane == 0) x.pex_kid[k] = (int8_t)wo.kid_node[j]; }
                    if (lane < wo.n_kids) { bool mine = false; for (int k = 0; k < nk; ++k) mine = mine || __builtin_amdgcn_readlane(my_j, k) == lane; if (!mine) { nh[wo.kid_node[lane]].used = 0; nh[wo.kid_node[lane]].complete = 0; } }
                    if (lane == 0) {
                        x.pex_n = nk; x.pex_L = T + n; ss.compound_ok += 1;
                        KidCopy& kc = kcopy[w];
                        kc.from = wo.node; kc.T = T; kc.n = n; kc.nk = nk; kc.dual = x.dual;
                    }
                    if (lane < nk) { KidCopy& kc = kcopy[w]; kc.node[lane] = (int8_t)wo.kid_node[my_j]; kc.b0[lane] = wo.kid_base[my_j][0]; kc.b1[lane] = wo.kid_base[my_j][1]; kc.sp[lane] = wo.kid_split[my_j]; }
                    for (int col = lane; col < n; col += SP_WAVE) { kcopy[w].spec[0][col] = wo.spec[0][col]; kcopy[w].spec[1][col] = wo.spec[1][col]; }
                } else if (lane < wo.n_kids) { nh[wo.kid_node[lane]].used = 0; nh[wo.kid_node[lane]].complete = 0; }
                spw::wave_lds_sync();
            } else if (a == n) {
                if (!side) la_fresh = wo.node;
                for (int y = lane; y < 2 * CW * 4; y += SP_WAVE) P.la[(size_t)wo.node * 2 * CW * 4 + y] = (&sl[0][0][0])[y];
                if (side) __threadfence_block();
            }
        } else if (mode_in == M_EXPAND) {
#ifdef SP_K8_TRACE
            if (lane == 0 && pi == 0) { printf("EXP%s L %d pre %d kids %d parcost %lld :", side ? " (side)" : "", wo.T + n_in, n_in, wo.n_kids, nh[wo.node].cost_at(nh[wo.node].q)); for (int k = 0; k < wo.n_kids; ++k) printf(" [%d/%d sc %u sr %u ev %u %u %u %u %u]", wo.kid_base[k][0], wo.kid_base[k][1], sc[k], sr[k], sv[0][k][0], sv[0][k][1], sv[0][k][2], sv[0][k][3], sv[0][k][4]); printf("\n"); }
#endif
            const long long par_cost = nh[wo.node].cost_at(nh[wo.node].q);
            if (!side) {
                kids_from_sums(wo, 1, wo.T + n_in, par_cost, lane < wo.n_kids ? lane : -1, 0);
                adopt(wo.node, wo.n_kids, true, [&](int k) { return (int)wo.kid_node[k]; });
            } else {
                kids_from_sums(wo, 2, wo.T + n_in, par_cost, lane < wo.n_kids ? lane : -1, 0);
                if (lane == 0) {
                    CNode& par = nh[wo.node];
                    par.pex_n = wo.n_kids; par.pex_L = wo.T + n_in;
                    for (int k = 0; k < wo.n_kids; ++k) par.pex_kid[k] = (int8_t)wo.kid_node[k];
                }
            }
        }
        spw::wave_lds_sync();
    };
    auto copy_window_kids = [&](const int w) {
        const KidCopy& kc = kcopy[w];
        if (kc.nk <= 0) return;
        const int whole = kc.T >> 4, L = kc.T + kc.n;
        for (int k = 0; k < kc.nk; ++k) {
            const bool split = kc.sp[k] != 0;
            for (int i = 0; i < 2; ++i) {
                if (i == 1 && !(kc.dual || split)) continue;
                const int si = (i == 1 && split) ? 0 : i;
                const uint8_t* srow = P.C + ((size_t)kc.from * 2 + si) * P.cs;
                uint8_t* dst = P.C + ((size_t)kc.node[k] * 2 + i) * P.cs;
                for (int y = tid; y < whole; y += blockDim.x) reinterpret_cast<uint4*>(dst)[y] = reinterpret_cast<const uint4*>(srow)[y];
                for (int y = (whole << 4) + tid; y <= L; y += blockDim.x) {
                    int v;
                    if (y < kc.T) v = srow[y];
                    else if (y < L) v = kc.spec[kc.dual ? si : 0][y - kc.T];
                    else v = i ? kc.b1[k] : kc.b0[k];
                    if (v >= 0) dst[y] = (uint8_t)v;
                }
            }
        }
    };
    for (int w = n_orders - 1; w >= 0; --w) {
        if (wks[w].mode == M_NONE) continue;
        load_votes(w);
        __syncthreads();
        if (tid < SP_WAVE) take_result(w);
        __syncthreads();
        copy_window_kids(w);
        if (w > 0) {
            for (int x = tid; x < QE; x += blockDim.x) acc[x] = 0;
            __syncthreads();
        }
    }
    const long long tk1 = wall_clock64();
    long long tk2 = tk1, tk3 = tk1;
#ifdef SP_K8_SEARCH_TICKS
    long long ts_pick = 0, ts_block = 0, ts_iters = 0;
#endif
    if (tid < SP_WAVE) {
        tk2 = wall_clock64();
        if (lane == 0) { const int steps_made = wk.pad + 1; for (int w = 0; w < n_orders; ++w) { wks[w].mode = M_NONE; wks[w].n = 0; wks[w].replay = 0; wks[w].n_kids = 0; } wk.pad = steps_made; }
        spw::wave_lds_sync();
        auto act = [&](const int xi, const int w, const Plan& pl, unsigned long long& free_bits) -> int {
            CNode& x = nh[xi];
            CWork& W = wks[w];
            const bool side = w > 0;
            const int cut = pl.cut;
            if ((x.q > 0 || x.n > 0) && cut < 0) {
                const int xn = x.n;
                if (xn > 1) x.wcap = SP_K8_RAMP * x.wcap < CW ? SP_K8_RAMP * x.wcap : CW;
                const long long c_end = x.cost_at(xn);
                const int la_ok = x.have_out == 1 ? 1 : 0;
                x.T += xn; x.cur ^= 1; x.cost0 = c_end; x.dc[0] = 0; x.rest = x.rest_out; x.n = x.a = x.q = 0; x.have_out = 0; x.la_valid = la_ok;
            }
            const int dual = x.dual, cur = x.cur, split_at = x.split_at, xT = x.T;
            const int pre_go0 = !x.stopped[0] ? 1 : 0, pre_go1 = (dual && !x.stopped[1]) ? 1 : 0;
            auto order_replay = [&]() {
                W.mode = M_WINDOW; W.node = xi; W.in_slot = cur; W.T = xT; W.n = x.a; W.replay = 1;
                W.dual = dual; W.split_at = split_at; W.go[0] = pre_go0; W.go[1] = pre_go1;
                replay_of[w] = xi;
                ss.inflight = xi;
            };
#ifdef SP_K8_NO_PRE
            if (!side && cut >= 0 && (SP_K8_NO_PRE == 0 || (SP_K8_NO_PRE == 1 && dual) || (SP_K8_NO_PRE == 2 && !dual))) { order_replay(); return 1; }
#endif
            const int L = pl.L;
            if (!side) {
                if (!x.stopped[0] && pl.nc0 == 0) { x.stopped[0] = 1; x.len[0] = L; }
                if (dual && !x.stopped[1] && pl.nc1 == 0) { x.stopped[1] = 1; x.len[1] = L; }
            }
            if (pl.nk == 0) {
                if (cut >= 0) { order_replay(); return 1; }
                const long long fc = x.cost0 + (P.et ? 0 : x.rest);
                if (ss.best_node < 0 || fc < ss.best_final) { if (ss.best_node >= 0) node_free(ss.best_node); ss.best_node = xi; ss.best_final = fc; x.complete = 1; }
                else node_free(xi);
                return 0;
            }
            const int nc0 = pl.nc0, nc1 = pl.nc1;
            auto code = [](uint32_t packed, int j) { return (int)((packed >> (2 * j)) & 3u); };
            if (pl.nk == 1 && cut >= 0) { order_replay(); return 1; }
            if (pl.nk == 1) {
                const int b0 = nc0 ? code(pl.cd0, 0) : -1, b1 = (dual && nc1) ? code(pl.cd1, 0) : -1;
                W.mode = M_WINDOW; W.node = xi; W.in_slot = cur; W.T = L; W.replay = 0; W.dual = dual; W.split_at = split_at;
                W.go[0] = b0 >= 0; W.spec[0][0] = (uint8_t)(b0 >= 0 ? b0 : 0); W.go[1] = b1 >= 0; W.spec[1][0] = (uint8_t)(b1 >= 0 ? b1 : 0);
                need_la[w] = x.la_valid ? xi : -1;
                W.n = 1;
                x.n = 0; x.a = 0; x.q = 0;
                if (!side) ss.inflight = xi;
                return 1;
            }
            W.mode = M_EXPAND; W.node = xi; W.in_slot = cur; W.T = xT; W.n = cut > 0 ? cut : 0; W.dual = dual; W.split_at = split_at; W.replay = 0;
            W.go[0] = nc0 > 0; W.go[1] = nc1 > 0; W.pre_go[0] = pre_go0; W.pre_go[1] = pre_go1;
            if (cut > 0) replay_of[w] = xi;
            int made = 0;
            for (int k = 0; k < pl.nk && made < MAXKIDS; ++k) {
                if (!free_bits) break;
                int b0, b1, sp;
                kid_of(pl, dual, k, b0, b1, sp);
                const int kn = __builtin_ctzll(free_bits); free_bits &= free_bits - 1;
                nh[kn].used = side ? 2 : 1; nh[kn].complete = 0; nh[kn].pex_n = 0;
                W.kid_node[made] = kn; W.kid_base[made][0] = (int8_t)b0; W.kid_base[made][1] = (int8_t)b1; W.kid_split[made] = (int8_t)sp;
                ++made;
            }
            W.n_kids = made;
            copy_from[w] = xi; copy_len[w] = L;
            return 1;
        };
        unsigned long long main_kids = 0;
        for (int guard = 0; ; ++guard) {
            if (guard > 100000) { if (lane == 0) wk.done = 1; break; }
#ifdef SP_K8_SEARCH_TICKS
            const long long ts0 = wall_clock64(); ts_iters += 1;
#endif
            int xi = ss.inflight;
            if (xi < 0) {
                long long kc = 0x7FFFFFFFFFFFFFFFll; int kt = -1, kid = 0x7FFFFFFF, kx = -1;
                if (lane < NQ && nh[lane].used == 1 && !nh[lane].complete) { const CNode& p = nh[lane]; kc = p.cost_at(p.q); kt = p.T + p.q; kid = p.id; kx = lane; }
                auto less = [](long long c1, int t1, int i1, long long c2, int t2, int i2) { return c1 < c2 || (c1 == c2 && (t1 > t2 || (t1 == t2 && i1 < i2))); };
                long long bc = kc; int bt = kt, bid = kid, bx = kx;
                long long sc2 = 0x7FFFFFFFFFFFFFFFll; int st2 = -1, sid2 = 0x7FFFFFFF, sx2 = -1;
                const unsigned long long waiting = __ballot(kx >= 0);
                if (__builtin_popcountll(waiting) == 1) {
                    const int only = __builtin_ctzll(waiting);
                    bc = ((long long)__builtin_amdgcn_readlane((int)(kc >> 32), only) << 32) | (unsigned int)__builtin_amdgcn_readlane((int)kc, only);
                    bt = __builtin_amdgcn_readlane(kt, only); bid = __builtin_amdgcn_readlane(kid, only); bx = only;
                    xi = only;
                } else {
#pragma unroll
                    for (int o = 32; o > 0; o >>= 1) {
                        const long long oc = __shfl_xor(bc, o); const int ot = __shfl_xor(bt, o), oi = __shfl_xor(bid, o), ox = __shfl_xor(bx, o);
                        if (ox >= 0 && (bx < 0 || less(oc, ot, oi, bc, bt, bid))) { bc = oc; bt = ot; bid = oi; bx = ox; }
                    }
                    xi = bx;
                    if (xi < 0) { if (lane == 0) wk.done = 1; break; }
                    sc2 = (kx == xi) ? 0x7FFFFFFFFFFFFFFFll : kc; st2 = kt; sid2 = kid; sx2 = (kx == xi) ? -1 : kx;
#pragma unroll
                    for (int o = 32; o > 0; o >>= 1) {
                        const long long oc = __shfl_xor(sc2, o); const int ot = __shfl_xor(st2, o), oi = __shfl_xor(sid2, o), ox = __shfl_xor(sx2, o);
                        if (ox >= 0 && (sx2 < 0 || less(oc, ot, oi, sc2, st2, sid2))) { sc2 = oc; st2 = ot; sid2 = oi; sx2 = ox; }
                    }
                }
                CNode& x = nh[xi];
                if (ss.best_node >= 0 && bc >= ss.best_final) { if (lane == 0) wk.done = 1; break; }
                const int linear0 = x.a - x.q;
                bool again = false, freed = false;
                int Lc = bt;
                for (;;) {
                    const int L = Lc, q = x.q, a = x.a;
                    const int wo = ss.wo_constraint;
                    const int jc = wo - 1 - ss.pops_mod;
                    const int linear = a - q;
                    const int want = linear > 0 ? (linear < SP_WAVE ? linear : SP_WAVE) : 1;
                    bool can = lane < want && L + lane >= ss.threshold && proc[L + lane] < ss.per_size && lane <= jc;
                    if (can && (lane > 0 || again)) {
                        const long long cj = x.cost_at(q + lane);
                        can = (sx2 < 0 || less(cj, L + lane, ss.next_id + lane - 1, sc2, st2, sid2)) && !(ss.best_node >= 0 && cj >= ss.best_final);
                    }
                    const unsigned long long no = ~__ballot(can);
                    const int m = no ? __builtin_ctzll(no) : SP_WAVE;
                    if (m == 0) { if (!again) { if (lane == 0) node_free(xi); freed = true; } break; }
                    if (lane < m) proc[L + lane] += 1;
                    if (lane == 0) {
                        ss.pops += m;
                        { int pm = ss.pops_mod + m; if (pm >= wo) pm %= wo; ss.pops_mod = pm; }
                        if (L + m - 1 > ss.farthest) ss.farthest = L + m - 1;
                        if (jc < m && ss.farthest > ss.threshold) ss.threshold = ss.farthest;
                        if (linear > 0) { x.q = q + m; x.id = ss.next_id + m - 1; ss.next_id += m; }
                    }
                    spw::wave_lds_sync();
                    if (!(linear > 0 && m == SP_WAVE && q + m < a)) break;
                    again = true; Lc = L + m;
                }
                if (freed) { spw::wave_lds_sync(); continue; }
                if (linear0 > 0) continue;
            } else if (lane == 0) ss.inflight = -1;
            spw::wave_lds_sync();
            int stop = 0;
#ifdef SP_K8_SEARCH_TICKS
            const long long ts1 = wall_clock64(); ts_pick += ts1 - ts0;
#endif
            {
                const CNode& x = nh[xi];
                if (x.q < x.a) {
                    if (lane == 0) { nh[xi].q += 1; nh[xi].id = ss.next_id++; }
                    spw::wave_lds_sync();
                    continue;
                }
                if (x.pex_n > 0) {
                    const int np = x.pex_n;
                    if (lane == 0) ss.adopted += 1;
                    adopt(xi, np, false, [&](int k) { return (int)nh[xi].pex_kid[k]; });
                    continue;
                }
            }
            const unsigned long long free_before = __ballot(lane < NQ && !nh[lane].used);
            unsigned long long free_nodes = free_before;
            if (lane == 0) { const Plan pl = plan_of(nh[xi]); stop = act(xi, 0, pl, free_nodes); }
            stop = __builtin_amdgcn_readfirstlane(stop);
            free_nodes = ((unsigned long long)(unsigned int)__builtin_amdgcn_readfirstlane((int)(free_nodes >> 32)) << 32) | (unsigned int)__builtin_amdgcn_readfirstlane((int)free_nodes);
            main_kids = free_before & ~free_nodes;
            spw::wave_lds_sync();
#ifdef SP_K8_SEARCH_TICKS
            ts_block += wall_clock64() - ts1;
#endif
            if (stop) break;
        }
        spw::wave_lds_sync();
        if (lane == 0 && !wk.done && wk.mode != M_NONE) ss.steps += 1;
        if (nside > 0 && !wk.done && wk.mode != M_NONE && __builtin_popcountll(__ballot(lane < NQ && nh[lane].used == 1 && !nh[lane].complete)) > 1) {
            Plan pl; pl.kind = 0; pl.nk = 0;
            bool cand = false;
            long long kc = 0x7FFFFFFFFFFFFFFFll; int kt = -1, kid = 0x7FFFFFFF;
            if (lane < NQ && nh[lane].used == 1 && !nh[lane].complete && lane != wk.node && !((main_kids >> lane) & 1ull) && nh[lane].q >= nh[lane].a && nh[lane].pex_n == 0) {
                const CNode& x = nh[lane];
                const int Lq = x.T + x.q;
                if (Lq >= ss.threshold && Lq < P.cap + 2 && proc[Lq] < ss.per_size) {
                    pl = plan_of(x);
                    cand = !pl.ends && ((pl.kind == 1 && pl.cut < 0) || (pl.kind == 2 && pl.nk <= MAXKIDS));
                    if (cand) { kc = x.cost_at(x.q); kt = Lq; kid = x.id; }
                }
            }
            const unsigned long long cm = __ballot(cand);
            if (cm) {
                auto less = [](long long c1, int t1, int i1, long long c2, int t2, int i2) { return c1 < c2 || (c1 == c2 && (t1 > t2 || (t1 == t2 && i1 < i2))); };
                int my_rank = 0;
                for (unsigned long long m = cm; m; m &= m - 1) {
                    const int b = __builtin_ctzll(m);
                    const long long oc = ((long long)__builtin_amdgcn_readlane((int)(kc >> 32), b) << 32) | (unsigned int)__builtin_amdgcn_readlane((int)kc, b);
                    const int ot = __builtin_amdgcn_readlane(kt, b), oi = __builtin_amdgcn_readlane(kid, b);
                    if (b != lane && less(oc, ot, oi, kc, kt, kid)) ++my_rank;
                }
                const unsigned long long free_nodes = __ballot(lane < NQ && !nh[lane].used);
                const int hidden = __builtin_popcountll(__ballot(lane < NQ && nh[lane].used == 2)), n_free = __builtin_popcountll(free_nodes);
                const int room = NQ - (ss.max_queue + 1) - MAXKIDS;
                const int n_cand = __builtin_popcountll(cm);
                int my_w = 0, my_skip = 0, accepted = 0, taken = 0, n_sw = 0, n_se = 0;
                for (int r = 0; r < n_cand && accepted < nside; ++r) {
                    const unsigned long long who = __ballot(cand && my_rank == r);
                    if (!who) continue;
                    const int b = __builtin_ctzll(who);
                    const int bkind = __builtin_amdgcn_readlane(pl.kind, b), bnk = __builtin_amdgcn_readlane(pl.nk, b);
                    if (bkind == 2 && (hidden + taken + bnk > room || n_free - taken < bnk + MAXKIDS)) continue;
                    if (lane == b) { my_w = 1 + accepted; my_skip = taken; }
                    ++accepted;
                    if (bkind == 2) { taken += bnk; ++n_se; } else ++n_sw;
                }
                if (lane == 0) { ss.side_windows += n_sw; ss.side_expansions += n_se; }
                if (my_w > 0) {
                    unsigned long long mine = free_nodes;
                    for (int j = 0; j < my_skip; ++j) mine &= mine - 1;
                    (void)act(lane, my_w, pl, mine);
                }
            }
        }
        spw::wave_lds_sync();
        for (int w = 0; w < n_orders; ++w) {
            const int ro = replay_of[w];
            if (ro >= 0) {
                const CNode& x = nh[ro];
                for (int jq = lane; jq < x.a; jq += SP_WAVE) { wks[w].spec[0][jq] = x.spec[0][jq]; wks[w].spec[1][jq] = x.spec[1][jq]; }
            }
        }
#ifdef SP_K8_PF_PROBE
        if (wk.mode == M_WINDOW || wk.mode == M_EXPAND) {
            bool idle = lane < NQ && nh[lane].used == 1 && !nh[lane].complete && lane != wk.node && nh[lane].q >= nh[lane].a;
            if (wk.mode == M_EXPAND) for (int k = 0; k < wk.n_kids; ++k) if (wk.kid_node[k] == lane) idle = false;
            const unsigned long long mask = __ballot(idle);
            if (lane == 0) {
                if ((ss.idle_mask >> wk.node) & 1ull) { if (wk.mode == M_EXPAND) ss.pf_exp += 1; else if (wk.replay) ss.pf_replay += 1; else ss.pf_win += 1; }
                ss.idle_mask = mask;
            }
        }
#endif
        spw::wave_lds_sync();
        tk3 = wall_clock64();
        for (int w = 0; w < n_orders; ++w) {
            const int nl = need_la[w];
            if (nl < 0) continue;
            CWork& W = wks[w];
            const uint32_t* la = (w == 0 && nl == la_fresh) ? &sl[0][0][0] : P.la + (size_t)nl * 2 * CW * 4;
            const int lim = nh[nl].wcap;
            const int hidden = __builtin_popcountll(__ballot(lane < NQ && nh[lane].used == 2)), n_free = __builtin_popcountll(__ballot(lane < NQ && !nh[lane].used));
            const int n_waiting = __builtin_popcountll(__ballot(lane < NQ && nh[lane].used == 1 && !nh[lane].complete));
            const bool may_branch = B.k8_compound && !coh && P.n_blocks <= DIRECT_BLOCKS && (lim < CW || n_waiting > 1 || B.k8_compound == 3) && hidden + KID_LA_KIDS <= NQ - (ss.max_queue + 1) - MAXKIDS && n_free >= KID_LA_KIDS + MAXKIDS;
            int nn = lim, bcol = -1, bn0 = 0, bn1 = 0; uint32_t bc0 = 0, bc1 = 0;
            for (int base = 0; base < lim; base += SP_WAVE) {
                const int col = base + lane;
                bool have = col >= 1 && col < lim && W.T + col < P.cap;
                int pick[2] = { 0, 0 };
                int n2[2] = { 0, 0 }; uint32_t pc[2] = { 0, 0 };
                if (have) {
#pragma unroll
                    for (int i = 0; i < 2; ++i) {
                        if (!W.go[i]) continue;
                        const uint4 wv = *reinterpret_cast<const uint4*>(la + ((size_t)i * CW + (col - 1)) * 4);
                        uint32_t wa = wv.x, wb = wv.y, wc = wv.z, wd = wv.w, ca = 0, cb = 1, cc = 2, cd = 3;
#define SP_CSW(x, y, cx, cy) if (y > x) { const uint32_t tw_ = x; x = y; y = tw_; const uint32_t tc_ = cx; cx = cy; cy = tc_; }
                        SP_CSW(wa, wb, ca, cb) SP_CSW(wa, wc, ca, cc) SP_CSW(wa, wd, ca, cd) SP_CSW(wb, wc, cb, cc) SP_CSW(wb, wd, cb, cd) SP_CSW(wc, wd, cc, cd)
#undef SP_CSW
                        if (wa == 0) have = false;
                        pick[i] = (int)ca;
                        const double share = B.k8_compound >= 10 ? 0.01 * (double)B.k8_compound : 0.25;
                        const double fair = (share > P.min_af ? share : P.min_af) * (double)(wa + wb + wc + wd);
                        int m = 1; uint32_t pk = ca;
                        if (wb >= 2 && (double)wb >= fair) { pk |= cb << (2 * m); ++m; }
                        if (wc >= 2 && (double)wc >= fair) { pk |= cc << (2 * m); ++m; }
                        if (wd >= 2 && (double)wd >= fair) { pk |= cd << (2 * m); ++m; }
                        n2[i] = m; pc[i] = pk;
                    }
                }
                unsigned long long miss = __ballot(!have);
                if (base == 0) miss &= ~1ull;
                int first = miss ? __builtin_ctzll(miss) : SP_WAVE;
                const unsigned long long brm = may_branch ? __ballot(have && col >= 1 && col <= CW - KID_LA_KIDS - 1 && (n2[0] > 1 || n2[1] > 1)) : 0ull;
                const int fb = brm ? __builtin_ctzll(brm) : SP_WAVE;
                if (fb < first) {
                    const int c0 = W.go[0] ? __builtin_amdgcn_readlane(n2[0], fb) : 0, c1 = (W.dual && W.go[1]) ? __builtin_amdgcn_readlane(n2[1], fb) : 0;
                    const int kids = !W.dual ? c0 + (P.allow_dual ? c0 * (c0 - 1) / 2 : 0) : (c0 ? c0 : 1) * (c1 ? c1 : 1);
                    if (kids >= 2 && kids <= KID_LA_KIDS) {
                        bcol = base + fb; bn0 = c0; bn1 = c1;
                        bc0 = (uint32_t)__builtin_amdgcn_readlane((int)pc[0], fb); bc1 = (uint32_t)__builtin_amdgcn_readlane((int)pc[1], fb);
                        first = fb;
                    }
                }
                if (col >= 1 && lane < first) { W.spec[0][col] = (uint8_t)pick[0]; W.spec[1][col] = (uint8_t)pick[1]; }
                if (miss || bcol >= 0) { nn = base + first; break; }
            }
            if (lane == 0) {
                W.n = nn < lim ? nn : lim;
            }
            if (bcol >= 1) {
                const unsigned long long free_mask = __ballot(lane < NQ && !nh[lane].used);
                if (lane == 0 && W.n == bcol) {
                    Plan fp; fp.nc0 = bn0; fp.nc1 = bn1; fp.cd0 = bc0; fp.cd1 = bc1;
                    const int kids = !W.dual ? bn0 + (P.allow_dual ? bn0 * (bn0 - 1) / 2 : 0) : (bn0 ? bn0 : 1) * (bn1 ? bn1 : 1);
                    unsigned long long fm = free_mask;
                    int made = 0;
                    for (int k = 0; k < kids && fm; ++k) {
                        int b0, b1, sp;
                        kid_of(fp, W.dual, k, b0, b1, sp);
                        const int kn = __builtin_ctzll(fm); fm &= fm - 1;
                        nh[kn].used = 2; nh[kn].complete = 0; nh[kn].pex_n = 0;
                        W.kid_node[made] = kn; W.kid_base[made][0] = (int8_t)b0; W.kid_base[made][1] = (int8_t)b1; W.kid_split[made] = (int8_t)sp;
                        ++made;
                    }
                    W.n_kids = made;
                    ss.compound += 1;
                }
                spw::wave_lds_sync();
            }
        }
    }
    __syncthreads();
    for (int w = 0; w < n_orders; ++w) {
        if (copy_from[w] < 0) continue;
        const CWork& W = wks[w];
        const int cfrom = copy_from[w], clen = copy_len[w];
        for (int k = 0; k < W.n_kids; ++k) {
            const int kn = W.kid_node[k];
            const bool split = W.kid_split[k] != 0;
            for (int i = 0; i < 2; ++i) {
                if (i == 1 && !(W.dual || split)) continue;
                const uint4* src = reinterpret_cast<const uint4*>(P.C + ((size_t)cfrom * 2 + ((i == 1 && split) ? 0 : i)) * P.cs);
                uint8_t* dst = P.C + ((size_t)kn * 2 + i) * P.cs;
                const int whole = clen >> 4, tail = clen & 15;
                for (int y = tid; y < whole + (tail ? 1 : 0); y += blockDim.x) {
                    uint4 v;
                    if (coh) {
                        const unsigned long long* s8 = reinterpret_cast<const unsigned long long*>(src + y);
                        const unsigned long long lo = coh_load(s8), hi = coh_load(s8 + 1);
                        v.x = (uint32_t)lo; v.y = (uint32_t)(lo >> 32); v.z = (uint32_t)hi; v.w = (uint32_t)(hi >> 32);
                    } else v = src[y];
                    if (y == whole && W.kid_base[k][i] >= 0) reinterpret_cast<uint8_t*>(&v)[tail] = (uint8_t)W.kid_base[k][i];
                    if (coh) {
                        unsigned long long* d8 = reinterpret_cast<unsigned long long*>(reinterpret_cast<uint4*>(dst) + y);
                        coh_store(d8, (unsigned long long)v.x | ((unsigned long long)v.y << 32)); coh_store(d8 + 1, (unsigned long long)v.z | ((unsigned long long)v.w << 32));
                    } else reinterpret_cast<uint4*>(dst)[y] = v;
                }
                if (tid == 0 && tail == 0 && W.kid_base[k][i] >= 0) put(&dst[clen], (uint8_t)W.kid_base[k][i], coh);
            }
        }
    }
    if (tid == 0) {
        const long long tk4 = wall_clock64(); ss.ticks[0] += tk1 - tk0; ss.ticks[1] += tk2 - tk1; ss.ticks[2] += tk3 - tk2; ss.ticks[3] += tk4 - tk3;
        if (B.step_t) {
            const long long st0 = (long long)coh_load(&B.step_t[2 * pi]), st1 = (long long)coh_load(&B.step_t[2 * pi + 1]);
            if (st1 > 0 && st0 <= st1) {
                ss.step_ticks += st1 - st0;
                if (ss.last_end > 0 && st0 >= ss.last_end) ss.gap_ticks += st0 - ss.last_end;
                if (tk0 >= st1) { ss.gap_ticks += tk0 - st1; ss.gap_ctl_ticks += tk0 - st1; }
            }
            put(&B.step_t[2 * pi], ~0ull, coh); put(&B.step_t[2 * pi + 1], 0ull, coh);
            ss.last_end = tk4;
        }
    }
#ifdef SP_K8_SEARCH_TICKS
    if (tid == 0) { ss.ticks[0] += 100 * ts_iters - (tk1 - tk0); ss.ticks[1] += ts_pick - (tk2 - tk1); ss.ticks[3] += ts_block - (wall_clock64() - tk3); }
#endif
    __syncthreads();
    for (int x = tid; x < NQ * NODE_HEAD_WORDS; x += blockDim.x)
        put(&((uint32_t*)&P.nodes[x / NODE_HEAD_WORDS])[x % NODE_HEAD_WORDS], ((const uint32_t*)&nh[x / NODE_HEAD_WORDS])[x % NODE_HEAD_WORDS], coh);
    for (int x = tid; x < NQ * NODE_TAPE_WORDS; x += blockDim.x) {
        const int k = x / NODE_TAPE_WORDS, w = x % NODE_TAPE_WORDS;
        if (tape_word_used(nh[k], w)) ((uint32_t*)&P.nodes[k])[NODE_HEAD_WORDS + w] = ((const uint32_t*)&nh[k])[NODE_HEAD_WORDS + w];
    }
    for (int x = tid; x < n_orders * (int)(sizeof(CWork) / 4); x += blockDim.x) put(&((uint32_t*)P.work)[x], ((const uint32_t*)wks)[x], coh);
    for (int x = tid; x < (int)(sizeof(CSearch) / 4); x += blockDim.x) ((uint32_t*)P.srch)[x] = ((const uint32_t*)&ss)[x];
    for (int x = tid; x < proc_words; x += blockDim.x) ((uint32_t*)P.processed)[x] = ((const uint32_t*)proc)[x];
    if (tid == 0 && B.prog) {
        __hip_atomic_store(B.prog + 2 * pi, (uint32_t)wk.pad, __ATOMIC_RELAXED, __HIP_MEMORY_SCOPE_SYSTEM);
        if (wk.done) __hip_atomic_store(B.prog + 2 * pi + 1, 1u, __ATOMIC_RELAXED, __HIP_MEMORY_SCOPE_SYSTEM);
    }
}

template <int MAXP>
__global__ void __launch_bounds__(1024) cons_control_kernel(ConsBatchT<MAXP> B) { cons_control_body<MAXP>(B); }

constexpr long long PERSIST_TIMEOUT = 400000000ll;
constexpr double PERSIST_READY_S = 0.5;
__device__ __forceinline__ bool persist_wait(const uint32_t* word, uint32_t at_least, uint32_t* abort_word) {
    const long long t0 = wall_clock64();
    for (uint32_t spins = 1;; ++spins) {
        if (__hip_atomic_load(word, __ATOMIC_RELAXED, __HIP_MEMORY_SCOPE_AGENT) >= at_least) return true;
        __builtin_amdgcn_s_sleep(1);
        if ((spins & 63u) == 0) {
            if (__hip_atomic_load(abort_word, __ATOMIC_RELAXED, __HIP_MEMORY_SCOPE_AGENT)) return false;
            if (wall_clock64() - t0 > PERSIST_TIMEOUT) { __hip_atomic_store(abort_word, 1u, __ATOMIC_RELAXED, __HIP_MEMORY_SCOPE_AGENT); return false; }
        }
    }
}

template <int MAXP>
__global__ void __launch_bounds__(CWAVES * SP_WAVE, SP_K8_MIN_WAVES) cons_step_persist_kernel(ConsBatchT<MAXP> B) {
    __shared__ int go_on;
    const int pi = block_problem<MAXP>(B);
    uint32_t* sy = B.sync + 4 * pi; uint32_t* abort_word = B.sync + 4 * B.n_prob;
    for (uint32_t k = 1;; ++k) {
        if (threadIdx.x == 0) go_on = persist_wait(sy + 0, k - 1, abort_word) ? 1 : 0;
        __syncthreads();
        if (!go_on) break;
        if (coh_load(&B.p[pi].work->done)) break;
        cons_step_body<MAXP>(B, 0);
        asm volatile("s_waitcnt vmcnt(0)" ::: "memory");
        __syncthreads();
        if (threadIdx.x == 0) __hip_atomic_fetch_add(sy + 1, 1u, __ATOMIC_RELAXED, __HIP_MEMORY_SCOPE_AGENT);
    }
}

template <int MAXP>
__global__ void __launch_bounds__(1024) cons_control_persist_kernel(ConsBatchT<MAXP> B) {
    __shared__ int go_on;
    const int pi = blockIdx.x;
    const uint32_t nb = (uint32_t)B.p[pi].n_blocks;
    uint32_t* sy = B.sync + 4 * pi; uint32_t* abort_word = B.sync + 4 * B.n_prob;
    if (threadIdx.x == 0 && B.ready) __hip_atomic_fetch_add(B.ready, 1u, __ATOMIC_RELAXED, __HIP_MEMORY_SCOPE_SYSTEM);
    for (uint32_t k = 1;; ++k) {
        if (threadIdx.x == 0) {
            go_on = persist_wait(sy + 1, nb * k, abort_word) ? 1 : 0;
            if (go_on && k > B.step_cap) { __hip_atomic_store(abort_word, 2u, __ATOMIC_RELAXED, __HIP_MEMORY_SCOPE_AGENT); go_on = 0; }
        }
        __syncthreads();
        if (!go_on) break;
        __builtin_amdgcn_fence(__ATOMIC_ACQUIRE, "agent");
        cons_control_body<MAXP>(B);
        asm volatile("s_waitcnt vmcnt(0)" ::: "memory");
        __syncthreads();
        const bool done = coh_load(&B.p[pi].work->done) != 0;
        if (threadIdx.x == 0) __hip_atomic_store(sy + 0, k, __ATOMIC_RELAXED, __HIP_MEMORY_SCOPE_AGENT);
        if (done) break;
    }
    if (threadIdx.x == 0 && B.prog) {
        const uint32_t ab = __hip_atomic_load(abort_word, __ATOMIC_RELAXED, __HIP_MEMORY_SCOPE_AGENT);
        if (ab) __hip_atomic_store(B.prog + 2 * pi + 1, 1u + ab, __ATOMIC_RELAXED, __HIP_MEMORY_SCOPE_SYSTEM);
    }
}

__global__ void cons_setup_kernel(ConsSetup S, ReadInfo* __restrict__ info) {
    const int r = blockIdx.x * blockDim.x + threadIdx.x;
    if (r >= S.n) return;
    const uint32_t rid = S.idx ? S.idx[r] : (uint32_t)r;
    ReadInfo ri;
    ri.w = S.reads.words + S.reads.word_off[rid];
    ri.np = S.reads.nplane ? S.reads.nplane + S.reads.word_off[rid] : nullptr;
    ri.n = S.reads.len[rid]; ri.off0 = S.offsets ? S.offsets[r] : -1; ri.off = ri.off0 < 0 ? -1 : ri.off0 + max(0, min(S.cmp_len, ri.n)); ri.pad = 0;
    info[S.first + r] = ri;
}

__global__ void cons_setup_many_kernel(const ConsSetup* __restrict__ S, int n_prob, int total, ReadInfo* __restrict__ info) {
    const int t = blockIdx.x * blockDim.x + threadIdx.x;
    if (t >= total) return;
    int lo = 0, hi = n_prob - 1;
    while (lo < hi) { const int mid = (lo + hi + 1) >> 1; if (S[mid].first <= t) lo = mid; else hi = mid - 1; }
    while (lo + 1 < n_prob && S[lo].n == 0 && S[lo + 1].first <= t) ++lo;
    const ConsSetup& q = S[lo];
    const int r = t - q.first;
    if (r < 0 || r >= q.n) return;
    const uint32_t rid = q.idx ? q.idx[r] : (uint32_t)r;
    ReadInfo ri;
    ri.w = q.reads.words + q.reads.word_off[rid];
    ri.np = q.reads.nplane ? q.reads.nplane + q.reads.word_off[rid] : nullptr;
    ri.n = q.reads.len[rid]; ri.off0 = q.offsets ? q.offsets[r] : -1; ri.off = ri.off0 < 0 ? -1 : ri.off0 + max(0, min(q.cmp_len, ri.n)); ri.pad = 0;
    info[t] = ri;
}

template <int MAXP>
__global__ void __launch_bounds__(SP_WAVE) cons_finalize_kernel(ConsBatchT<MAXP> B, uint8_t* is_cons1, int32_t* score1, int32_t* score2) {
    const int vblock = (int)blockIdx.x / CWAVES, wave = (int)blockIdx.x % CWAVES;
    const int pi = block_problem<MAXP>(B, vblock);
    const ConsParams P = B.p[pi];
    const int lane = threadIdx.x;
    const int best = P.srch->best_node;
    const size_t plane = (size_t)B.total;
    if (vblock == P.first_block && wave == 0) {
        for (int x = threadIdx.x; x < (int)(sizeof(CSearch) / 4); x += blockDim.x) ((uint32_t*)P.out_srch)[x] = ((const uint32_t*)P.srch)[x];
        if (threadIdx.x == 0) {
            ConsRes r; r.best = best; r.dual = 0; r.split_at = -1; r.len1 = r.len2 = 0; r.pad = 0;
            if (best >= 0) { const CNode* x = P.nodes + best; r.dual = x->dual; r.split_at = x->split_at; r.len1 = x->len[0]; r.len2 = x->dual ? x->len[1] : 0; }
            *P.out_res = r;
        }
        if (best >= 0) {
            const uint8_t* src = P.C + (size_t)best * 2 * P.cs;
#pragma unroll
            for (int i = 0; i < 2; ++i) {
                const uint32_t* s4 = reinterpret_cast<const uint32_t*>(src + (size_t)i * P.cs);
                uint8_t* dst = P.out_cons + (size_t)i * P.cap;
                for (int x = (int)threadIdx.x * 4; x < P.cap; x += (int)blockDim.x * 4) {
                    const uint32_t w = s4[x >> 2];
#pragma unroll
                    for (int q = 0; q < 4; ++q) if (x + q < P.cap) dst[x + q] = (uint8_t)(w >> (8 * q));
                }
            }
        }
    }
    for (int rr = 0; rr < P.rpw; ++rr) {
        const int r = ((vblock - P.first_block) * CWAVES + wave) * P.rpw + rr;
        if (r >= P.n) break;
        const size_t g = (size_t)P.first + r;
        int sc[2] = { -1, -1 };
        if (best >= 0) {
            const CNode* x = P.nodes + best;
            const int n = B.info[g].n, cur = x->cur, dual = x->dual;
#pragma unroll
            for (int i = 0; i < 2; ++i) {
                if (i == 1 && !dual) continue;
                const size_t p = state_plane(best, cur, i) * plane + g;
                const ConsMeta m = B.meta[p];
                if (!(m.flags & F_ACTIVE) || (m.flags & F_LOST)) continue;
                int e = m.e;
                if (!P.et) {
                    const int h = h_load(B.H, p * CB + lane), k = lane - CH;
                    int rest = (h >= 0 && h + k == x->len[i] - m.c0) ? n - h : (1 << 30);
#pragma unroll
                    for (int o = 32; o > 0; o >>= 1) { const int other = __shfl_xor(rest, o); rest = other < rest ? other : rest; }
                    if (rest < (1 << 30)) e += rest;
                }
                sc[i] = e;
            }
        }
        if (lane == 0) {
            score1[g] = sc[0]; score2[g] = sc[1];
            is_cons1[g] = !(sc[1] >= 0 && (sc[0] < 0 || sc[1] < sc[0]));
        }
    }
}

}

constexpr int PERSIST_MAX_BATCHES = 4;
struct PersistLease {
    int device = -1, taken = 0;
    static std::atomic<int>& used(int device) { static std::atomic<int> u[64]; return u[device & 63]; }
    static std::atomic<int>& batches(int device) { static std::atomic<int> b[64]; return b[device & 63]; }
    bool take(int dev, int budget, int want, int max_batches) {
        if (batches(dev).fetch_add(1) >= max_batches) { batches(dev).fetch_sub(1); return false; }
        std::atomic<int>& u = used(dev);
        int cur = u.load();
        while (cur + want <= budget) if (u.compare_exchange_weak(cur, cur + want)) { device = dev; taken = want; return true; }
        batches(dev).fetch_sub(1);
        return false;
    }
    void give_back() { if (taken) { used(device).fetch_sub(taken); batches(device).fetch_sub(1); taken = 0; } }
    ~PersistLease() { give_back(); }
};

template <int MAXP>
static int32_t run_chunk(sp_ctx* ctx, uint32_t n_prob, const sp_cons_problem* probs, sp_cons_output* outs) {
    hipStream_t st = ctx->stream;
    HostMarks hm(ctx);
    ConsBatchT<MAXP> B; std::memset(&B, 0, sizeof B);
    B.n_prob = (int)n_prob;
    std::vector<ConsParams> hp(n_prob);
    std::vector<int> block_prob, cluster_prob;
    std::vector<ConsSetup> setup(n_prob);
    std::vector<uint32_t> h_idx; std::vector<int32_t> h_off;
    std::vector<size_t> idx_at(n_prob), off_at(n_prob), c_at(n_prob), proc_at(n_prob);
    size_t total = 0, c_bytes = 0, proc_bytes = 0; int max_cap = 0, n_blocks = 0, n_clusters = 0;
    std::vector<int> expect(n_prob, 0);
    PersistLease lease;
    int persist_rpw = 0;
    int nside = std::max(0, std::min(ctx->k8_side_orders, NWORK - 1));
    {
        uint64_t nb_all = 0;
        for (uint32_t p = 0; p < n_prob; ++p) nb_all += ((probs[p].read_idx ? probs[p].n : probs[p].reads->n) + CWAVES - 1) / CWAVES;
        if (nb_all * CWAVES > (uint64_t)ctx->k8_side_max_blocks * 8) nside = 0;
    }
    struct InFlight {
        int dev; bool cand; int others = 0;
        static std::atomic<int>& count(int d) { static std::atomic<int> c[64]; return c[d & 63]; }
        static std::atomic<int>& cands(int d) { static std::atomic<int> c[64]; return c[d & 63]; }
        static std::atomic<long long>& overlap_ns(int d) { static std::atomic<long long> t[64]; return t[d & 63]; }
        static long long now_ns() { return std::chrono::duration_cast<std::chrono::nanoseconds>(std::chrono::steady_clock::now().time_since_epoch()).count(); }
        bool recent_overlap = false;
        InFlight(int d, bool candidate) : dev(d), cand(candidate) {
            others = count(dev).fetch_add(1);
            const long long t = now_ns();
            if (cand && cands(dev).fetch_add(1) > 0) overlap_ns(dev).store(t);
            const long long last = overlap_ns(dev).load();
            recent_overlap = last != 0 && t - last < 1000000000ll;
        }
        ~InFlight() { count(dev).fetch_sub(1); if (cand) cands(dev).fetch_sub(1); }
    } in_flight(ctx->device, n_prob > 0 && n_prob <= 8 && [&] { uint64_t f = 2 * (uint64_t)n_prob; for (uint32_t p = 0; p < n_prob; ++p) f += ((probs[p].read_idx ? probs[p].n : probs[p].reads->n) + CWAVES - 1) / CWAVES; return f > (uint64_t)PERSIST_LIGHT; }());
    uint64_t footprint = 2 * (uint64_t)n_prob;
    for (uint32_t p = 0; p < n_prob; ++p) footprint += ((probs[p].read_idx ? probs[p].n : probs[p].reads->n) + CWAVES - 1) / CWAVES;
    const bool light = footprint <= (uint64_t)PERSIST_LIGHT;
    const bool persist_wanted = ctx->k8_persistent == 1 || (ctx->k8_persistent == 2 && n_prob <= 8 && ctx->hw_queues_effective >= 16 && ctx->k8_persist_failures < 3 &&
                                                            !in_flight.recent_overlap && light);
    if (ctx->k8_persist_backoff > 0) --ctx->k8_persist_backoff;
    else if (persist_wanted && n_prob > 0) {
        bool small = true;
        for (uint32_t p = 0; p < n_prob; ++p) {
            const uint32_t n = probs[p].read_idx ? probs[p].n : probs[p].reads->n;
            const uint32_t nb = (n + CWAVES - 1) / CWAVES;
            small = small && nb <= (uint32_t)PERSIST_BLOCKS;
        }
        constexpr int WG_PER_CU = SP_K8_MIN_WAVES * 4 / CWAVES;
        int budget = WG_PER_CU * std::max(0, ctx->num_cus - 32); const int ctl = 2 * (int)n_prob;
        { const char* e = std::getenv("SP_K8_BUDGET"); if (e && *e) budget = std::atoi(e); }
        if (small && ctl < budget) {
            for (int scale = 1; scale <= 4 && !persist_rpw; ++scale) {
                uint64_t nb = 0;
                for (uint32_t p = 0; p < n_prob; ++p) { const uint32_t n = probs[p].read_idx ? probs[p].n : probs[p].reads->n; nb += (n + CWAVES * scale - 1) / (CWAVES * scale); }
                if ((int64_t)nb + ctl <= budget && lease.take(ctx->device, budget, (int)nb + ctl, (ctx->k8_persistent == 2 && !light) ? PERSIST_AUTO_BATCHES : PERSIST_MAX_BATCHES)) persist_rpw = scale;
                else if ((int64_t)nb + ctl <= budget) break;
            }
        }
    }
    for (uint32_t p = 0; p < n_prob; ++p) {
        const sp_cons_problem& q = probs[p];
        const uint32_t n = q.read_idx ? q.n : q.reads->n;
        ConsParams& P = hp[p];
        P.n = (int)n; P.cap = (int)outs[p].cap - 1;
        P.cs = (std::max(P.cap, 1) + 1 + 15) & ~15;
        P.first = (int)total; P.first_block = n_blocks;
        P.min_count = q.cfg.min_count; P.delta = q.cfg.dual_max_ed_delta; P.et = q.cfg.allow_early_termination != 0; P.allow_dual = q.cfg.allow_dual != 0;
        P.window = q.cfg.offset_window; P.cmp_len = q.cfg.offset_compare_length; P.min_af = q.cfg.min_af;
        P.rpw = persist_rpw ? persist_rpw : n > 65536 ? 4 : n > 32768 ? 2 : 1;
        const uint32_t per_block = (uint32_t)(CWAVES * P.rpw);
        const uint32_t nb = (n + per_block - 1) / per_block;
        P.n_blocks = (int)nb;
        P.first_cluster = n_clusters; P.n_clusters = (int)((nb + CLUSTER - 1) / CLUSTER);
        n_clusters += P.n_clusters;
        n_blocks += (int)nb;
        if (MAXP == 0) { block_prob.insert(block_prob.end(), nb, (int)p); cluster_prob.insert(cluster_prob.end(), (size_t)P.n_clusters, (int)p); }
        setup[p].reads = q.reads->view(); setup[p].n = (int)n; setup[p].first = (int)total;
        total += (size_t)nb * per_block;
        idx_at[p] = h_idx.size(); if (q.read_idx) h_idx.insert(h_idx.end(), q.read_idx, q.read_idx + n);
        off_at[p] = h_off.size(); if (q.offsets) h_off.insert(h_off.end(), q.offsets, q.offsets + n);
        c_at[p] = c_bytes; c_bytes += (size_t)NQ * 2 * (size_t)P.cs;
        proc_at[p] = proc_bytes; proc_bytes += ((size_t)std::max(P.cap, 1) + 2 + 15) & ~(size_t)15;
        max_cap = std::max(max_cap, P.cap);
        int reach = 0;
        for (uint32_t i = 0; i < n; ++i) {
            const uint32_t r = q.read_idx ? q.read_idx[i] : i;
            const int o = q.offsets && q.offsets[i] > 0 ? q.offsets[i] : 0;
            reach = std::max(reach, o + (r < q.reads->h_len.size() ? q.reads->h_len[r] : P.cap));
        }
        expect[p] = std::min(P.cap, reach);
    }
    if (n_blocks == 0) return SP_OK;
    const size_t planes = (size_t)NQ * 4;
    size_t in_bytes = 0, out_bytes = 0, zero_bytes = 0;
    auto place = [](size_t& total_bytes, size_t bytes) { const size_t at = (total_bytes + 15) & ~(size_t)15; total_bytes = at + bytes; return at; };
    const size_t in_idx = place(in_bytes, sizeof(uint32_t) * h_idx.size()), in_off = place(in_bytes, sizeof(int32_t) * h_off.size());
    const size_t in_work = place(in_bytes, sizeof(CWork) * NWORK * n_prob), in_srch = place(in_bytes, sizeof(CSearch) * n_prob);
    const size_t in_probs = place(in_bytes, MAXP == 0 ? sizeof(ConsParams) * n_prob : 0), in_bp = place(in_bytes, sizeof(int) * block_prob.size());
    const size_t in_cp = place(in_bytes, sizeof(int) * cluster_prob.size());
    const size_t in_setup = place(in_bytes, n_prob > 8 ? sizeof(ConsSetup) * n_prob : 0);
    const size_t out_srch = place(out_bytes, sizeof(CSearch) * n_prob), out_res = place(out_bytes, sizeof(ConsRes) * n_prob);
    const size_t out_is1 = place(out_bytes, total), out_sc = place(out_bytes, sizeof(int32_t) * 2 * total);
    std::vector<size_t> out_cons(n_prob);
    for (uint32_t p = 0; p < n_prob; ++p) out_cons[p] = place(out_bytes, (size_t)2 * std::max(hp[p].cap, 1));
    const size_t zero_nodes = place(zero_bytes, sizeof(CNode) * NQ * n_prob), zero_proc = place(zero_bytes, proc_bytes), zero_info = place(zero_bytes, sizeof(ReadInfo) * total), zero_memo = place(zero_bytes, sizeof(PlaceMemo) * 2 * total * (size_t)(1 + nside));
    const size_t zero_sync = place(zero_bytes, sizeof(uint32_t) * (4 * (size_t)n_prob + 4));
    uint8_t* d_in = (uint8_t*)sp_pool(ctx, "cons_in", in_bytes + 16); uint8_t* h_in = (uint8_t*)sp_host_pool(ctx, "cons_in", in_bytes + 16);
    uint8_t* d_out = (uint8_t*)sp_pool(ctx, "cons_out", out_bytes + 16); uint8_t* h_out = (uint8_t*)sp_host_pool(ctx, "cons_out", out_bytes + 16);
    uint8_t* d_zero = (uint8_t*)sp_pool(ctx, "cons_zero", zero_bytes + 16);
    if (!d_in || !h_in || !d_out || !h_out || !d_zero) return sp_fail(ctx, SP_ERR_OUT_OF_MEMORY, "sp_consensus staging");
    uint32_t* d_idx = (uint32_t*)(d_in + in_idx); int32_t* d_off = (int32_t*)(d_in + in_off);
    uint8_t* d_C = (uint8_t*)sp_pool(ctx, "cons_C", c_bytes);
    CWork* d_work = (CWork*)(d_in + in_work);
    CSearch* d_srch = (CSearch*)(d_in + in_srch);
    CNode* d_nodes = (CNode*)(d_zero + zero_nodes);
    uint32_t* d_la = (uint32_t*)sp_pool(ctx, "cons_la", sizeof(uint32_t) * (size_t)NQ * 2 * CW * 4 * n_prob);
    uint8_t* d_proc = d_zero + zero_proc;
    ReadInfo* d_info = (ReadInfo*)(d_zero + zero_info);
    B.memo = (PlaceMemo*)(d_zero + zero_memo);
    B.sync = persist_rpw ? (uint32_t*)(d_zero + zero_sync) : nullptr;
    B.info = d_info; B.total = (int)total;
    B.H = (uint16_t*)sp_pool(ctx, "cons_H", sizeof(uint16_t) * planes * total * CB);
    B.meta = (ConsMeta*)sp_pool(ctx, "cons_meta", sizeof(ConsMeta) * planes * total);
    const size_t wblocks = (size_t)n_blocks + (size_t)NWORK * n_prob;
    B.PV = (unsigned long long*)sp_pool(ctx, "cons_pv", sizeof(unsigned long long) * wblocks * 2 * (CW + 1));
    B.PE = (uint32_t*)sp_pool(ctx, "cons_pe", sizeof(uint32_t) * wblocks * 2 * (CW + 1));
    B.PL = (unsigned long long*)sp_pool(ctx, "cons_pl", sizeof(unsigned long long) * wblocks * 2 * CW);
    B.PC = (uint32_t*)sp_pool(ctx, "cons_pc", sizeof(uint32_t) * wblocks * (CW + 1));
    B.PR = (uint32_t*)sp_pool(ctx, "cons_pr", sizeof(uint32_t) * wblocks * (CW + 1));
    B.Q = (uint32_t*)sp_pool(ctx, "cons_q", sizeof(uint32_t) * (size_t)n_clusters * QE);
#ifdef SP_K8_TIMING
    B.dbg = (unsigned long long*)sp_pool(ctx, "cons_dbg", (size_t)SP_K8_DBG_LAUNCHES * SP_K8_DBG_READS * 8);
    (void)hipMemsetAsync(B.dbg, 0, (size_t)SP_K8_DBG_LAUNCHES * SP_K8_DBG_READS * 8, st);
#endif
    uint8_t* d_is1 = d_out + out_is1;
    int32_t* d_sc = (int32_t*)(d_out + out_sc);
    B.step_t = nullptr;
    if (ctx->profiling) {
        B.step_t = (unsigned long long*)sp_pool(ctx, "cons_step_t", sizeof(unsigned long long) * 2 * n_prob);
        if (B.step_t) {
            std::vector<unsigned long long> init((size_t)2 * n_prob);
            for (uint32_t p = 0; p < n_prob; ++p) { init[2 * p] = ~0ull; init[2 * p + 1] = 0ull; }
            unsigned long long* h_st = (unsigned long long*)sp_host_pool(ctx, "cons_step_t", sizeof(unsigned long long) * 2 * n_prob);
            if (h_st) { std::memcpy(h_st, init.data(), init.size() * 8); (void)hipMemcpyAsync(B.step_t, h_st, init.size() * 8, hipMemcpyHostToDevice, st); } else B.step_t = nullptr;
        }
    }
    uint32_t* h_prog = (uint32_t*)sp_host_pool(ctx, "cons_prog", sizeof(uint32_t) * 2 * n_prob);
    if (!h_prog) return sp_fail(ctx, SP_ERR_OUT_OF_MEMORY, "sp_consensus progress words");
    std::memset(h_prog, 0, sizeof(uint32_t) * 2 * n_prob);
    { void* dp = nullptr; SP_HIP_CHECK(ctx, hipHostGetDevicePointer(&dp, h_prog, 0)); B.prog = (uint32_t*)dp; }
    CWork* h_work = (CWork*)sp_host_pool(ctx, "cons_work", sizeof(CWork) * n_prob);
    CWork* h_work0 = (CWork*)(h_in + in_work); CSearch* h_srch0 = (CSearch*)(h_in + in_srch);
    const CSearch* h_srch = (const CSearch*)(h_out + out_srch);
    if (!d_idx || !d_off || !d_C || !d_work || !d_srch || !d_nodes || !d_la || !d_proc || !d_info || !B.H || !B.meta || !B.PV || !B.PE || !B.PL || !B.PC || !B.PR || !B.Q ||
        !h_work)
        return sp_fail(ctx, SP_ERR_OUT_OF_MEMORY, "sp_consensus buffers");
    for (uint32_t p = 0; p < n_prob; ++p) {
        setup[p].idx = probs[p].read_idx ? d_idx + idx_at[p] : nullptr;
        setup[p].offsets = probs[p].offsets ? d_off + off_at[p] : nullptr; setup[p].cmp_len = probs[p].cfg.offset_compare_length; setup[p].pad_ = 0;
        hp[p].C = d_C + c_at[p]; hp[p].work = d_work + (size_t)p * NWORK; hp[p].srch = d_srch + p; hp[p].nodes = d_nodes + (size_t)p * NQ;
        hp[p].la = d_la + (size_t)p * NQ * 2 * CW * 4; hp[p].processed = d_proc + proc_at[p];
        hp[p].acc_block = n_blocks + (int)p * NWORK;
        hp[p].out_cons = d_out + out_cons[p]; hp[p].out_res = (ConsRes*)(d_out + out_res) + p; hp[p].out_srch = (CSearch*)(d_out + out_srch) + p;
    }
    if constexpr (MAXP == 0) {
        std::memcpy(h_in + in_probs, hp.data(), sizeof(ConsParams) * n_prob);
        std::memcpy(h_in + in_bp, block_prob.data(), sizeof(int) * block_prob.size());
        std::memcpy(h_in + in_cp, cluster_prob.data(), sizeof(int) * cluster_prob.size());
        B.p = (const ConsParams*)(d_in + in_probs); B.block_prob = (const int*)(d_in + in_bp); B.cluster_prob = (const int*)(d_in + in_cp);
    } else {
        for (uint32_t p = 0; p < n_prob; ++p) B.p[p] = hp[p];
    }
    for (uint32_t p = 0; p < n_prob; ++p) {
        std::memset(&h_work0[(size_t)p * NWORK], 0, sizeof(CWork) * NWORK);
        CWork& w = h_work0[(size_t)p * NWORK]; w.mode = M_INIT; w.node = 0; w.in_slot = 0; w.split_at = -1;
        CSearch& s = h_srch0[p]; std::memset(&s, 0, sizeof s); s.best_node = -1; s.inflight = -1;
        const sp_cons_config& cf = probs[p].cfg;
        s.max_queue = cf.max_queue_size > 0 ? std::min(cf.max_queue_size, NQ - MAXKIDS - 2) : 20;
        s.per_size = cf.max_capacity_per_size > 0 ? std::min(cf.max_capacity_per_size, 255) : 10;
        s.wo_constraint = cf.max_nodes_wo_constraint > 0 ? cf.max_nodes_wo_constraint : 1000;
    }
    if (!h_idx.empty()) std::memcpy(h_in + in_idx, h_idx.data(), sizeof(uint32_t) * h_idx.size());
    if (!h_off.empty()) std::memcpy(h_in + in_off, h_off.data(), sizeof(int32_t) * h_off.size());
    if (n_prob > 8) std::memcpy(h_in + in_setup, setup.data(), sizeof(ConsSetup) * n_prob);
    SP_HIP_CHECK(ctx, hipMemcpyAsync(d_in, h_in, in_bytes, hipMemcpyHostToDevice, st));
    SP_HIP_CHECK(ctx, hipMemsetAsync(d_zero, 0, zero_bytes, st));
    {
        const size_t nb = (size_t)n_blocks, np = (size_t)n_prob * NWORK;
        SP_HIP_CHECK(ctx, hipMemsetAsync(B.PV + nb * 2 * (CW + 1), 0, sizeof(unsigned long long) * np * 2 * (CW + 1), st));
        SP_HIP_CHECK(ctx, hipMemsetAsync(B.PE + nb * 2 * (CW + 1), 0, sizeof(uint32_t) * np * 2 * (CW + 1), st));
        SP_HIP_CHECK(ctx, hipMemsetAsync(B.PL + nb * 2 * CW, 0, sizeof(unsigned long long) * np * 2 * CW, st));
        SP_HIP_CHECK(ctx, hipMemsetAsync(B.PC + nb * (CW + 1), 0, sizeof(uint32_t) * np * (CW + 1), st));
        SP_HIP_CHECK(ctx, hipMemsetAsync(B.PR + nb * (CW + 1), 0, sizeof(uint32_t) * np * (CW + 1), st));
    }
    if (n_prob > 8) hipLaunchKernelGGL(cons_setup_many_kernel, dim3((unsigned)((total + 255) / 256)), dim3(256), 0, st, (const ConsSetup*)(d_in + in_setup), (int)n_prob, (int)total, d_info);
    else for (uint32_t p = 0; p < n_prob; ++p)
        if (setup[p].n) hipLaunchKernelGGL(cons_setup_kernel, dim3((setup[p].n + 255) / 256), dim3(256), 0, st, setup[p], d_info);

    B.nside = persist_rpw ? 0 : nside;
    B.k8_compound = ctx->k8_compound;
    const dim3 grid((uint32_t)n_blocks, (uint32_t)(1 + B.nside)), block(CWAVES * SP_WAVE);
    const bool one_round = n_blocks <= (ctx->num_cus + ctx->num_cus / 4) * (8 / CWAVES);
    size_t proc_lds = ((size_t)max_cap + 2 + 15) & ~(size_t)15;
    {
        hipFuncAttributes fa;
        SP_HIP_CHECK(ctx, hipFuncGetAttributes(&fa, (const void*)cons_control_kernel<MAXP>));
        if (fa.sharedSizeBytes + proc_lds > 160 * 1024) return sp_fail(ctx, SP_ERR_TOO_LONG, "sp_consensus: cap must stay below ~65,000");
    }
    SP_HIP_CHECK(ctx, hipFuncSetAttribute((const void*)cons_control_kernel<MAXP>, hipFuncAttributeMaxDynamicSharedMemorySize, (int)proc_lds));
    uint64_t pairs = 0;
    bool persist_ran = false;
    hm.mark("host:k8_prologue");
    double t_launch = 0.0;
    {
        ProfScope ps(ctx, "cons_steps", total);
        const uint64_t limit = (uint64_t)64 * (uint64_t)(max_cap + 2) + 1024;
        const uint32_t ahead = 3;
        bool need_reduce = false;
        for (uint32_t p = 0; p < n_prob; ++p) need_reduce = need_reduce || hp[p].n_blocks > DIRECT_BLOCKS;
        volatile uint32_t* prog = h_prog;
        bool finished = false;
        if (persist_rpw) {
            if (!ctx->ctl_stream && hipStreamCreateWithFlags(&ctx->ctl_stream, hipStreamNonBlocking) != hipSuccess) return sp_fail(ctx, SP_ERR_HIP, "sp_consensus: control stream");
            const bool own_step_stream = ctx->hw_queues_effective < 16;
            if (own_step_stream && !ctx->pst_stream && hipStreamCreateWithFlags(&ctx->pst_stream, hipStreamNonBlocking) != hipSuccess) return sp_fail(ctx, SP_ERR_HIP, "sp_consensus: step stream");
            if (own_step_stream && !ctx->ev_join2 && hipEventCreateWithFlags(&ctx->ev_join2, hipEventDisableTiming) != hipSuccess) return sp_fail(ctx, SP_ERR_HIP, "sp_consensus: events");
            const hipStream_t step_st = own_step_stream ? ctx->pst_stream : st;
            if (!ctx->ev_fork && (hipEventCreateWithFlags(&ctx->ev_fork, hipEventDisableTiming) != hipSuccess || hipEventCreateWithFlags(&ctx->ev_join, hipEventDisableTiming) != hipSuccess))
                return sp_fail(ctx, SP_ERR_HIP, "sp_consensus: events");
            SP_HIP_CHECK(ctx, hipFuncSetAttribute((const void*)cons_control_persist_kernel<MAXP>, hipFuncAttributeMaxDynamicSharedMemorySize, (int)proc_lds));
            SP_HIP_CHECK(ctx, hipEventRecord(ctx->ev_fork, st));
            SP_HIP_CHECK(ctx, hipStreamWaitEvent(ctx->ctl_stream, ctx->ev_fork, 0));
            if (own_step_stream) SP_HIP_CHECK(ctx, hipStreamWaitEvent(step_st, ctx->ev_fork, 0));
            uint32_t* h_ready = (uint32_t*)sp_host_pool(ctx, "cons_ready", 64);
            if (!h_ready) return sp_fail(ctx, SP_ERR_OUT_OF_MEMORY, "sp_consensus ready word");
            *(volatile uint32_t*)h_ready = 0;
            { void* dp = nullptr; SP_HIP_CHECK(ctx, hipHostGetDevicePointer(&dp, h_ready, 0)); B.ready = (uint32_t*)dp; }
            B.step_cap = (uint32_t)std::min<uint64_t>(limit, 0xFFFFFFFFull);
            auto drain = [&]() { (void)hipStreamSynchronize(ctx->ctl_stream); if (own_step_stream) (void)hipStreamSynchronize(step_st); (void)hipStreamSynchronize(st); };
            hipLaunchKernelGGL(cons_control_persist_kernel<MAXP>, dim3(n_prob), dim3(1024), proc_lds, ctx->ctl_stream, B);
            bool all_ready = true;
            {
                const auto t_wait = std::chrono::steady_clock::now();
                const bool forced = std::getenv("SP_K8_FORCE_READY_TIMEOUT") != nullptr;
                while (forced || *(volatile uint32_t*)h_ready < n_prob) {
                    __builtin_ia32_pause();
                    if (forced || std::chrono::duration<double>(std::chrono::steady_clock::now() - t_wait).count() > PERSIST_READY_S) { all_ready = false; break; }
                }
            }
            if (all_ready) {
                hipLaunchKernelGGL(cons_step_persist_kernel<MAXP>, dim3((uint32_t)n_blocks), block, 0, step_st, B);
                hipError_t e3 = hipGetLastError();
                if (e3 == hipSuccess) e3 = hipEventRecord(ctx->ev_join, ctx->ctl_stream);
                if (e3 == hipSuccess && own_step_stream) e3 = hipEventRecord(ctx->ev_join2, step_st);
                if (e3 == hipSuccess) e3 = hipStreamWaitEvent(st, ctx->ev_join, 0);
                if (e3 == hipSuccess && own_step_stream) e3 = hipStreamWaitEvent(st, ctx->ev_join2, 0);
                if (e3 != hipSuccess) {
                    const uint32_t one = 1;
                    if (!ctx->copy_stream) (void)hipStreamCreateWithFlags(&ctx->copy_stream, hipStreamNonBlocking);
                    if (ctx->copy_stream) { (void)hipMemcpyAsync(B.sync + 4 * n_prob, &one, 4, hipMemcpyHostToDevice, ctx->copy_stream); (void)hipStreamSynchronize(ctx->copy_stream); }
                    drain();
                    return sp_fail(ctx, SP_ERR_HIP, std::string("sp_consensus: persistent launch: ") + hipGetErrorString(e3));
                }
                finished = true; persist_ran = true;
            } else {
                const uint32_t one = 1;
                if (!ctx->copy_stream && hipStreamCreateWithFlags(&ctx->copy_stream, hipStreamNonBlocking) != hipSuccess) { drain(); return sp_fail(ctx, SP_ERR_HIP, "sp_consensus: copy stream"); }
                (void)hipMemcpyAsync(B.sync + 4 * n_prob, &one, 4, hipMemcpyHostToDevice, ctx->copy_stream);
                (void)hipStreamSynchronize(ctx->copy_stream);
                (void)hipStreamSynchronize(ctx->ctl_stream);
                lease.give_back();
                ctx->k8_persist_failures += 1; ctx->k8_persist_backoff = 64;
                ctx->warning = "persistent consensus kernels: the control workgroups of a batch found no free CUs within " + std::to_string(PERSIST_READY_S) +
                               " s (another process on this device?): the batch ran launch by launch, and so will the next 64";
                (void)hipMemsetAsync(B.sync, 0, sizeof(uint32_t) * (4 * (size_t)n_prob + 1), st);
                std::memset(h_prog, 0, sizeof(uint32_t) * 2 * n_prob);
                B.sync = nullptr; B.ready = nullptr;
                persist_rpw = 0;
            }
        }
        while (!finished) {
            const auto tl0 = std::chrono::steady_clock::now();
            if (one_round) hipLaunchKernelGGL(cons_step_wide_kernel<MAXP>, grid, block, 0, st, B);
            else hipLaunchKernelGGL(cons_step_kernel<MAXP>, grid, block, 0, st, B);
            if (need_reduce) hipLaunchKernelGGL(cons_reduce_kernel<MAXP>, dim3((uint32_t)n_clusters * RSLICES), dim3(512), 0, st, B);
            hipLaunchKernelGGL(cons_control_kernel<MAXP>, dim3(n_prob), dim3(1024), proc_lds, st, B);
            t_launch += std::chrono::duration<double, std::milli>(std::chrono::steady_clock::now() - tl0).count();
            ++pairs;
            uint64_t spins = 0;
            for (;;) {
                bool all = true; uint32_t slowest = 0xFFFFFFFFu;
                for (uint32_t p = 0; p < n_prob; ++p) if (!prog[2 * p + 1]) { all = false; const uint32_t v = prog[2 * p]; slowest = v < slowest ? v : slowest; }
                if (all) { finished = true; break; }
                if (pairs - slowest <= ahead) break;
                __builtin_ia32_pause();
                if ((++spins & 0xFFFFF) == 0) {
                    const hipError_t q = hipStreamQuery(st);
                    if (q != hipSuccess && q != hipErrorNotReady) return sp_fail(ctx, SP_ERR_HIP, std::string("sp_consensus: ") + hipGetErrorString(q));
                    if (q == hipSuccess) {
                        bool all2 = true; uint32_t slow2 = 0xFFFFFFFFu;
                        for (uint32_t p = 0; p < n_prob; ++p) if (!prog[2 * p + 1]) { all2 = false; const uint32_t v = prog[2 * p]; slow2 = v < slow2 ? v : slow2; }
                        if (all2) { finished = true; break; }
                        if (pairs - slow2 <= ahead) break;
                        return sp_fail(ctx, SP_ERR_HIP, "sp_consensus: the device stopped reporting progress");
                    }
                }
            }
            if (!finished && pairs >= limit) return sp_fail(ctx, SP_ERR_HIP, "sp_consensus: the search did not finish");
        }
    }
#define SP_K8_CHECK(expr) do { const hipError_t e_ = (expr); if (e_ != hipSuccess) { if (persist_ran) { (void)hipStreamSynchronize(ctx->ctl_stream); if (ctx->pst_stream) (void)hipStreamSynchronize(ctx->pst_stream); (void)hipStreamSynchronize(st); } \
        return sp_fail(ctx, SP_ERR_HIP, std::string(#expr) + ": " + hipGetErrorString(e_)); } } while (0)
    SP_K8_CHECK(hipGetLastError());
    hm.mark("host:k8_loop");
    if (ctx->profiling) { auto& e = ctx->prof["host:k8_launch"]; e.ms += t_launch; e.launches += (uint32_t)(2 * pairs); }
    hipLaunchKernelGGL(cons_finalize_kernel<MAXP>, dim3((uint32_t)n_blocks * CWAVES), dim3(SP_WAVE), 0, st, B, d_is1, d_sc, d_sc + total);
    SP_K8_CHECK(hipMemcpyAsync(h_out, d_out, out_bytes, hipMemcpyDeviceToHost, st));
    const uint8_t* h_is1 = h_out + out_is1; const int32_t* h_sc = (const int32_t*)(h_out + out_sc); const ConsRes* h_res = (const ConsRes*)(h_out + out_res);
    SP_K8_CHECK(hipStreamSynchronize(st));
    SP_K8_CHECK(hipGetLastError());
#undef SP_K8_CHECK
    lease.give_back();
    if (persist_ran) {
        for (uint32_t p = 0; p < n_prob; ++p) {
            if (h_prog[2 * p + 1] == 2u) {
                ctx->k8_persist_failures += 1; ctx->k8_persist_backoff = 64;
                if (ctx->k8_persistent == 2) {
                    ctx->warning = "persistent consensus kernels: the kernels of a batch waited for each other for more than four seconds (another process on this device?): the batch ran "
                                   "again launch by launch, and so will the next 64";
                    return SP_K8_AGAIN;
                }
                return sp_fail(ctx, SP_ERR_HIP, "sp_consensus: the persistent kernels of a batch waited for each other for more than four seconds and gave up");
            }
            if (h_prog[2 * p + 1] == 3u) return sp_fail(ctx, SP_ERR_HIP, "sp_consensus: the search did not finish");
            pairs = std::max<uint64_t>(pairs, h_prog[2 * p]);
        }
        ctx->prof["cons_persistent_batches"].cells += 1;
    }
    hm.mark("host:k8_result_wait");
#ifdef SP_K8_TIMING
    if (std::getenv("SP_K8_DUMP")) {
        std::vector<unsigned long long> h((size_t)SP_K8_DBG_LAUNCHES * SP_K8_DBG_READS);
        (void)hipMemcpy(h.data(), B.dbg, h.size() * 8, hipMemcpyDeviceToHost);
        FILE* f = std::fopen(std::getenv("SP_K8_DUMP"), "ab");
        if (f) { const unsigned long long tot = total; std::fwrite(&tot, 8, 1, f); std::fwrite(h.data(), 8, h.size(), f); std::fclose(f); }
    }
#endif
    {
        uint64_t cut = 0, ex = 0, pops = 0;
        for (uint32_t p = 0; p < n_prob; ++p) { cut += (uint64_t)h_srch[p].cut_windows; ex += (uint64_t)h_srch[p].expansions; pops += (uint64_t)h_srch[p].pops; }
        ctx->prof["cons_windows"].cells += pairs; ctx->prof["cons_windows"].launches += 3 * pairs;
        ctx->prof["cons_cut_windows"].cells += cut; ctx->prof["cons_expansions"].cells += ex; ctx->prof["cons_columns"].cells += pops;
        for (uint32_t p = 0; p < n_prob; ++p) {
            ctx->prof["cons_side_windows"].cells += (uint64_t)h_srch[p].side_windows; ctx->prof["cons_side_expansions"].cells += (uint64_t)h_srch[p].side_expansions;
            ctx->prof["cons_adopted"].cells += (uint64_t)h_srch[p].adopted;
            ctx->prof["cons_compound"].cells += (uint64_t)h_srch[p].compound; ctx->prof["cons_compound_ok"].cells += (uint64_t)h_srch[p].compound_ok;
        }
#ifdef SP_K8_PF_PROBE
        {
            uint64_t c0 = 0, c1 = 0, c2 = 0;
            for (uint32_t p = 0; p < n_prob; ++p) {
                const uint64_t st = (uint64_t)h_srch[p].windows + (uint64_t)h_srch[p].expansions, w = (uint64_t)h_srch[p].pf_win + (uint64_t)h_srch[p].pf_replay, e = (uint64_t)h_srch[p].pf_exp;
                c0 = std::max(c0, st); c1 = std::max(c1, st - w); c2 = std::max(c2, st - w - e);
                ctx->prof["cons_pf_win"].cells += (uint64_t)h_srch[p].pf_win; ctx->prof["cons_pf_replay"].cells += (uint64_t)h_srch[p].pf_replay; ctx->prof["cons_pf_exp"].cells += e;
                ctx->prof["cons_all_windows"].cells += (uint64_t)h_srch[p].windows;
            }
            ctx->prof["cons_pf_chain"].cells += c0; ctx->prof["cons_pf_chain_win"].cells += c1; ctx->prof["cons_pf_chain_all"].cells += c2;
        }
#endif
        static const char* tick_names[4] = { "cons_ticks_reduce", "cons_ticks_result", "cons_ticks_search", "cons_ticks_tail" };
        for (int k = 0; k < 4; ++k) { long long m = 0; for (uint32_t p = 0; p < n_prob; ++p) m = std::max(m, h_srch[p].ticks[k]); ctx->prof[tick_names[k]].cells += (uint64_t)m; }
        if (B.step_t) {
            long long best = -1; uint32_t bp = 0;
            for (uint32_t p = 0; p < n_prob; ++p) {
                const long long tot = h_srch[p].step_ticks + h_srch[p].gap_ticks + h_srch[p].ticks[0] + h_srch[p].ticks[1] + h_srch[p].ticks[2] + h_srch[p].ticks[3];
                if (tot > best) { best = tot; bp = p; }
            }
            ctx->prof["cons_path_step_ticks"].cells += (uint64_t)h_srch[bp].step_ticks; ctx->prof["cons_path_gap_ticks"].cells += (uint64_t)h_srch[bp].gap_ticks; ctx->prof["cons_path_gap_ctl_ticks"].cells += (uint64_t)h_srch[bp].gap_ctl_ticks;
            ctx->prof["cons_path_control_ticks"].cells += (uint64_t)(h_srch[bp].ticks[0] + h_srch[bp].ticks[1] + h_srch[bp].ticks[2] + h_srch[bp].ticks[3]);
            ctx->prof["cons_path_steps"].cells += (uint64_t)h_srch[bp].steps;
        }
    }
    static const char dec[4] = { 'A', 'C', 'G', 'T' };
    int32_t rc = SP_OK;
    for (uint32_t p = 0; p < n_prob; ++p) {
        const ConsParams& P = hp[p]; sp_cons_output& o = outs[p];
        const ConsRes& res = h_res[p];
        const int best = res.best, len1 = res.len1, len2 = res.len2, dual = res.dual, split_at = res.split_at;
        if (best >= 0) {
            const uint8_t* c = h_out + out_cons[p];
            for (int x2 = 0; x2 < len1; ++x2) o.cons1[x2] = dec[c[x2] & 3];
            for (int x2 = 0; x2 < len2; ++x2) o.cons2[x2] = dec[(x2 < split_at ? c[x2] : c[(size_t)P.cap + x2]) & 3];
        }
        o.cons1[len1] = '\0'; o.cons2[len2] = '\0';
        for (int r = 0; r < P.n; ++r) { o.is_cons1[r] = h_is1[P.first + r]; o.score1[r] = h_sc[P.first + r]; o.score2[r] = h_sc[total + P.first + r]; }
        o.result.is_dual = dual; o.result.len1 = len1; o.result.len2 = len2; o.result.split_at = split_at;
        o.result.gave_up = best < 0 ? 1 : 0; o.result.best_total = 1; o.result.split_w2 = 0; o.result.split_total = 1;
        o.result.nodes_expanded = h_srch[p].pops;
        if (len1 >= P.cap || len2 >= P.cap) { o.status = SP_ERR_CAPACITY; rc = SP_ERR_CAPACITY; }
    }
    if (rc != SP_OK) sp_fail(ctx, rc, "sp_consensus: a consensus reached cap");
    hm.mark("host:k8_epilogue");
    return rc;
}

static int32_t run_batch(sp_ctx* ctx, uint32_t n_prob, const sp_cons_problem* probs, sp_cons_output* outs) {
    for (uint32_t p = 0; p < n_prob; ++p) {
        const sp_cons_problem& q = probs[p]; sp_cons_output& o = outs[p];
        if (!q.reads || !o.cons1 || !o.cons2 || o.cap == 0 || !o.is_cons1 || !o.score1 || !o.score2) return sp_fail(ctx, SP_ERR_INVALID_ARG, "sp_consensus: null argument");
        if (q.cfg.offset_compare_length > 128 || q.cfg.offset_compare_length < 0 || q.cfg.offset_window < 0 || q.cfg.min_count < 0 ||
            (q.cfg.offset_compare_length > 64 && q.cfg.offset_window + q.cfg.offset_compare_length > ACT_CONS))
            return sp_fail(ctx, SP_ERR_INVALID_ARG, "sp_consensus: offset_compare_length must be in [0, 128] (in [0, 64] when offset_window + offset_compare_length exceeds 512)");
        if (o.cap >= (1u << 22)) return sp_fail(ctx, SP_ERR_TOO_LONG, "sp_consensus: cap must be below 4,194,304");
        if (q.reads->max_len >= 65535) return sp_fail(ctx, SP_ERR_TOO_LONG, "sp_consensus: sequences must be shorter than 65,535 bases");
        std::memset(&o.result, 0, sizeof o.result); o.result.split_at = -1; o.result.best_total = 1; o.status = SP_OK;
        o.cons1[0] = o.cons2[0] = '\0';
        const uint32_t n = q.read_idx ? q.n : q.reads->n;
        if (q.read_idx) for (uint32_t i = 0; i < n; ++i) if (q.read_idx[i] >= q.reads->n) return sp_fail(ctx, SP_ERR_INVALID_ARG, "sp_consensus: read index out of range");
    }
    SP_HIP_CHECK(ctx, hipSetDevice(ctx->device));
    int32_t rc = SP_OK;
    const uint32_t big = 4096;
    for (uint32_t at = 0; at < n_prob; at += big) {
        const uint32_t k = std::min<uint32_t>(big, n_prob - at);
        auto run = [&]() { return k <= 4 ? run_chunk<4>(ctx, k, probs + at, outs + at) : k <= 8 ? run_chunk<8>(ctx, k, probs + at, outs + at)
                                  : k <= CMAXP ? run_chunk<CMAXP>(ctx, k, probs + at, outs + at) : run_chunk<0>(ctx, k, probs + at, outs + at); };
        int32_t e = run();
        if (e == SP_K8_AGAIN) e = run();
        if (e != SP_OK && e != SP_ERR_CAPACITY) return e;
        if (e != SP_OK) rc = e;
    }
    return rc;
}

extern "C" {

int32_t sp_consensus_batch(sp_ctx* ctx, uint32_t n_problems, const sp_cons_problem* problems, sp_cons_output* outputs) {
    if (!ctx) return SP_ERR_INVALID_ARG;
    if (n_problems == 0) return SP_OK;
    if (!problems || !outputs) return sp_fail(ctx, SP_ERR_INVALID_ARG, "sp_consensus_batch: null argument");
    return run_batch(ctx, n_problems, problems, outputs);
}

int32_t sp_consensus_dual_batch(sp_ctx* ctx, uint32_t n_problems, const sp_cons_problem* problems, sp_cons_output* outputs) {
    if (!ctx) return SP_ERR_INVALID_ARG;
    if (n_problems == 0) return SP_OK;
    if (!problems || !outputs) return sp_fail(ctx, SP_ERR_INVALID_ARG, "sp_consensus_dual_batch: null argument");
    std::vector<sp_cons_problem> pr(problems, problems + n_problems);
    for (auto& q : pr) q.cfg.allow_dual = 1;
    return run_batch(ctx, n_problems, pr.data(), outputs);
}

int32_t sp_consensus(sp_ctx* ctx, const sp_seqset* reads, const uint32_t* read_idx, uint32_t n, const int32_t* offsets,
                     const sp_cons_config* cfg, char* cons1, char* cons2, uint32_t cap,
                     uint8_t* is_cons1, int32_t* score1, int32_t* score2, sp_cons_result* result) {
    if (!ctx) return SP_ERR_INVALID_ARG;
    if (!reads || !cfg || !result) return sp_fail(ctx, SP_ERR_INVALID_ARG, "sp_consensus: null argument");
    sp_cons_problem q; q.reads = reads; q.read_idx = read_idx; q.n = n; q.offsets = offsets; q.cfg = *cfg;
    sp_cons_output o; std::memset(&o, 0, sizeof o);
    o.cons1 = cons1; o.cons2 = cons2; o.cap = cap; o.is_cons1 = is_cons1; o.score1 = score1; o.score2 = score2;
    const int32_t rc = run_batch(ctx, 1, &q, &o);
    *result = o.result;
    return rc;
}

int32_t sp_consensus_dual(sp_ctx* ctx, const sp_seqset* reads, const uint32_t* read_idx, uint32_t n, const int32_t* offsets,
                          const sp_cons_config* cfg, char* cons1, char* cons2, uint32_t cap,
                          uint8_t* is_cons1, int32_t* score1, int32_t* score2, sp_cons_result* result) {
    if (!ctx) return SP_ERR_INVALID_ARG;
    if (!reads || !cfg || !result) return sp_fail(ctx, SP_ERR_INVALID_ARG, "sp_consensus_dual: null argument");
    sp_cons_problem q; q.reads = reads; q.read_idx = read_idx; q.n = n; q.offsets = offsets; q.cfg = *cfg;
    sp_cons_output o; std::memset(&o, 0, sizeof o);
    o.cons1 = cons1; o.cons2 = cons2; o.cap = cap; o.is_cons1 = is_cons1; o.score1 = score1; o.score2 = score2;
    const int32_t rc = sp_consensus_dual_batch(ctx, 1, &q, &o);
    *result = o.result;
    return rc;
}

int32_t sp_consensus_priority_many(sp_ctx* ctx, uint32_t n_jobs, sp_priority_job* jobs) {
    if (!ctx) return SP_ERR_INVALID_ARG;
    if (n_jobs && !jobs) return sp_fail(ctx, SP_ERR_INVALID_ARG, "sp_consensus_priority_many: null argument");
    struct Item { std::vector<uint32_t> members; uint32_t level; std::string key; int retry = 0; std::vector<std::string> kept; std::vector<uint8_t> have; };
    struct JobState { std::vector<Item> work, done; int half = 0; bool live = false; };
    static const double retry_min_af[4] = { 0.15, 0.20, 0.30, 0.40 };
    std::vector<JobState> S(n_jobs);
    for (uint32_t j = 0; j < n_jobs; ++j) {
        sp_priority_job& J = jobs[j];
        J.status = SP_OK; J.gave_up = 0;
        const sp_priority_problem* pr = J.problem;
        if (!pr || !J.n_groups || !J.group_of || !J.cons || !pr->levels || pr->n_levels == 0 || J.cap < 2) { J.status = SP_ERR_INVALID_ARG; continue; }
        bool ok = true;
        for (uint32_t l = 0; l < pr->n_levels; ++l) if (!pr->levels[l] || pr->levels[l]->n != pr->n) ok = false;
        if (!ok) { J.status = SP_ERR_INVALID_ARG; continue; }
        *J.n_groups = 0;
        if (pr->n == 0) continue;
        S[j].half = pr->cfg.offset_window / 2; S[j].live = true;
        std::map<int32_t, std::vector<uint32_t>> by_seed;
        for (uint32_t r = 0; r < pr->n; ++r) by_seed[pr->seeds ? (pr->seeds[r] < 0 ? -1 : pr->seeds[r]) : -1].push_back(r);
        uint32_t ord = 0;
        for (auto& kv : by_seed) { Item it; it.members = kv.second; it.level = 0; it.key = std::string(1, (char)('a' + std::min<uint32_t>(ord, 25))) + std::to_string(ord); ++ord; S[j].work.push_back(std::move(it)); }
    }
    auto rebased = [&](uint32_t j, const std::vector<uint32_t>& m, uint32_t level, std::vector<int32_t>& out) -> bool {
        const sp_priority_problem* pr = jobs[j].problem;
        const int32_t* src = pr->offsets ? pr->offsets[level] : nullptr;
        if (!src) return false;
        int64_t mn = INT64_MAX;
        for (uint32_t r : m) mn = std::min<int64_t>(mn, src[r] < 0 ? 0 : src[r]);
        out.resize(m.size());
        for (size_t i = 0; i < m.size(); ++i) { const int64_t o = src[m[i]] < 0 ? 0 : src[m[i]]; out[i] = o == mn ? -1 : (int32_t)(o - mn + (mn == 0 ? 0 : S[j].half)); }
        return true;
    };
    for (;;) {
        std::vector<std::pair<uint32_t, size_t>> at;
        for (uint32_t j = 0; j < n_jobs; ++j) if (S[j].live) for (size_t x = 0; x < S[j].work.size(); ++x) at.push_back({ j, x });
        const size_t k = at.size();
        if (k == 0) break;
        std::vector<sp_cons_problem> P(k); std::vector<sp_cons_output> O(k);
        std::vector<std::vector<int32_t>> offs(k), s1(k), s2(k); std::vector<std::vector<uint8_t>> is1(k); std::vector<std::vector<char>> text(k);
        for (size_t x = 0; x < k; ++x) {
            const uint32_t j = at[x].first; const Item& it = S[j].work[at[x].second];
            const sp_priority_problem* pr = jobs[j].problem;
            const sp_seqset* set = pr->levels[it.level];
            int32_t longest = 0; for (uint32_t r : it.members) longest = std::max(longest, set->h_len[r]);
            const bool has_off = rebased(j, it.members, it.level, offs[x]);
            int32_t far = 0; if (has_off) for (int32_t o : offs[x]) far = std::max(far, o);
            const uint32_t c = (uint32_t)longest + (uint32_t)far + 66;
            s1[x].resize(it.members.size()); s2[x].resize(it.members.size()); is1[x].resize(it.members.size()); text[x].assign((size_t)2 * c, 0);
            P[x].reads = set; P[x].read_idx = it.members.data(); P[x].n = (uint32_t)it.members.size(); P[x].offsets = has_off ? offs[x].data() : nullptr;
            P[x].cfg = pr->cfg; P[x].cfg.allow_dual = 1;
            if (it.retry > 0) P[x].cfg.min_af = retry_min_af[it.retry - 1];
            std::memset(&O[x], 0, sizeof O[x]);
            O[x].cons1 = text[x].data(); O[x].cons2 = text[x].data() + c; O[x].cap = c; O[x].is_cons1 = is1[x].data(); O[x].score1 = s1[x].data(); O[x].score2 = s2[x].data();
        }
        const int32_t rc = sp_consensus_dual_batch(ctx, (uint32_t)k, P.data(), O.data());
        if (rc != SP_OK) return rc;
        std::vector<std::vector<Item>> next(n_jobs);
        for (size_t x = 0; x < k; ++x) {
            const uint32_t j = at[x].first; Item& it = S[j].work[at[x].second];
            const sp_priority_problem* pr = jobs[j].problem;
            const uint32_t NL = pr->n_levels;
            if (O[x].result.gave_up && !pr->cfg.no_retry_ladder && !it.members.empty()) {
                int step = it.retry;
                while (step < 4 && retry_min_af[step] <= pr->cfg.min_af) ++step;
                if (step < 4) { it.retry = step + 1; next[j].push_back(std::move(it)); continue; }
            }
            if (O[x].result.gave_up) jobs[j].gave_up += 1;
            std::vector<uint32_t> g1, g2;
            for (size_t i = 0; i < it.members.size(); ++i) (is1[x][i] ? g1 : g2).push_back(it.members[i]);
            if (O[x].result.is_dual && !g1.empty() && !g2.empty()) {
                Item a; a.members = std::move(g1); a.level = it.level; a.key = it.key + "0"; next[j].push_back(std::move(a));
                Item b; b.members = std::move(g2); b.level = it.level; b.key = it.key + "1"; next[j].push_back(std::move(b));
            } else {
                if (it.retry == 0 && !O[x].result.is_dual && !O[x].result.gave_up) {
                    it.kept.resize(NL); it.have.resize(NL, 0);
                    it.kept[it.level] = std::string(text[x].data()); it.have[it.level] = 1;
                }
                if (it.level + 1 < NL) { it.level += 1; it.key += "_"; it.retry = 0; next[j].push_back(std::move(it)); }
                else S[j].done.push_back(std::move(it));
            }
        }
        for (uint32_t j = 0; j < n_jobs; ++j) if (S[j].live) {
            S[j].work.swap(next[j]);
            if (S[j].done.size() + S[j].work.size() > (size_t)jobs[j].problem->n) { jobs[j].status = SP_ERR_INVALID_ARG; S[j].live = false; S[j].work.clear(); }
        }
    }
    std::vector<sp_cons_problem> P; std::vector<sp_cons_output> O;
    std::vector<std::vector<int32_t>> offs, s1, s2; std::vector<std::vector<uint8_t>> is1; std::vector<std::vector<char>> spare;
    size_t k = 0;
    auto has_kept = [](const Item& it, uint32_t l) { return l < it.have.size() && it.have[l]; };
    for (uint32_t j = 0; j < n_jobs; ++j) {
        if (!S[j].live) continue;
        sp_priority_job& J = jobs[j];
        auto& done = S[j].done;
        std::sort(done.begin(), done.end(), [](const Item& a, const Item& b) { return a.key < b.key; });
        *J.n_groups = (uint32_t)done.size();
        for (size_t g = 0; g < done.size(); ++g) for (uint32_t r : done[g].members) J.group_of[r] = (int32_t)g;
        if (done.size() > J.max_groups) { J.status = SP_ERR_CAPACITY; S[j].live = false; continue; }
        const uint32_t NL = J.problem->n_levels;
        for (size_t g = 0; g < done.size() && S[j].live; ++g) for (uint32_t l = 0; l < NL; ++l) {
            if (!has_kept(done[g], l)) { ++k; continue; }
            const std::string& c = done[g].kept[l];
            if (c.size() + 1 > (size_t)J.cap) { J.status = SP_ERR_CAPACITY; S[j].live = false; break; }
            std::memcpy(J.cons + (g * NL + l) * (size_t)J.cap, c.c_str(), c.size() + 1);
        }
    }
    k = 0;
    for (uint32_t j = 0; j < n_jobs; ++j) if (S[j].live) for (const Item& it : S[j].done) for (uint32_t l = 0; l < jobs[j].problem->n_levels; ++l) if (!has_kept(it, l)) ++k;
    P.resize(k); O.resize(k); offs.resize(k); s1.resize(k); s2.resize(k); is1.resize(k); spare.resize(k);
    size_t x = 0;
    for (uint32_t j = 0; j < n_jobs; ++j) {
        if (!S[j].live) continue;
        sp_priority_job& J = jobs[j]; const sp_priority_problem* pr = J.problem; const uint32_t NL = pr->n_levels;
        for (size_t g = 0; g < S[j].done.size(); ++g) for (uint32_t l = 0; l < NL; ++l) {
            const Item& it = S[j].done[g];
            if (has_kept(it, l)) continue;
            const bool has_off = rebased(j, it.members, l, offs[x]);
            s1[x].resize(it.members.size()); s2[x].resize(it.members.size()); is1[x].resize(it.members.size()); spare[x].assign(J.cap, 0);
            P[x].reads = pr->levels[l]; P[x].read_idx = it.members.data(); P[x].n = (uint32_t)it.members.size(); P[x].offsets = has_off ? offs[x].data() : nullptr;
            P[x].cfg = pr->cfg; P[x].cfg.allow_dual = 0;
            std::memset(&O[x], 0, sizeof O[x]);
            O[x].cons1 = J.cons + (g * NL + l) * (size_t)J.cap; O[x].cons2 = spare[x].data(); O[x].cap = J.cap; O[x].is_cons1 = is1[x].data(); O[x].score1 = s1[x].data(); O[x].score2 = s2[x].data();
            ++x;
        }
    }
    if (k == 0) return SP_OK;
    return sp_consensus_batch(ctx, (uint32_t)k, P.data(), O.data());
}

int32_t sp_consensus_priority(sp_ctx* ctx, const sp_priority_problem* pr, uint32_t max_groups, uint32_t cap,
                              uint32_t* n_groups, int32_t* group_of, char* cons) {
    if (!ctx) return SP_ERR_INVALID_ARG;
    if (!pr || !n_groups || !group_of || !cons || !pr->levels || pr->n_levels == 0 || cap < 2) return sp_fail(ctx, SP_ERR_INVALID_ARG, "sp_consensus_priority: null argument");
    for (uint32_t l = 0; l < pr->n_levels; ++l) if (!pr->levels[l] || pr->levels[l]->n != pr->n) return sp_fail(ctx, SP_ERR_INVALID_ARG, "sp_consensus_priority: every level needs one sequence per read");
    sp_priority_job J; J.problem = pr; J.max_groups = max_groups; J.cap = cap; J.n_groups = n_groups; J.group_of = group_of; J.cons = cons; J.status = SP_OK; J.gave_up = 0;
    const int32_t rc = sp_consensus_priority_many(ctx, 1, &J);
    if (rc != SP_OK) return rc;
    if (J.status == SP_ERR_CAPACITY) return sp_fail(ctx, SP_ERR_CAPACITY, "sp_consensus_priority: more groups than max_groups");
    if (J.status == SP_ERR_INVALID_ARG) return sp_fail(ctx, SP_ERR_INVALID_ARG, "sp_consensus_priority: more groups than reads");
    return J.status;
}

}
```

Before: 356,900 reads/s.

## Shrink control kernel LDS: tape slots, windowed processed copy, templated order count

Splits each search node into a header and a tape, and keeps only up to eight tapes in LDS slots. Nodes that do not get a slot fall back to their global-memory copy. The processed-counter array is now copied in and out only over the length window the live nodes can touch, not the whole cap. The side-order arrays are sized by a template parameter so the no-side launch uses less LDS, and the block drops from 1024 to 512 threads. The aim is less per-launch LDS traffic and smaller static LDS for the small serial control kernel, at the cost of slot-management logic, possible global spills and fewer threads for the bulk copies.

Result: slower. 350,800 reads/s (-1.7%).

```diff
diff --git a/pb-starphase_amd/csrc/sp_consensus.hip b/pb-starphase_amd/csrc/sp_consensus.hip
--- a/pb-starphase_amd/csrc/sp_consensus.hip
+++ b/pb-starphase_amd/csrc/sp_consensus.hip
@@ -53,7 +53,7 @@
     int8_t  kid_split[MAXKIDS];
     uint8_t spec[2][CW];
 };
-struct CNode {
+struct CNodeHead {
     int32_t used, id, complete;
     int32_t T, cur;
     int32_t dual, split_at, stopped[2], len[2];
@@ -67,13 +67,15 @@
     int32_t pex_n, pex_L;
     int8_t  pex_kid[MAXKIDS];
     int32_t pad_head[2];
+};
+struct CTape {
     int32_t dc[CW + 1];
     uint8_t spec[2][CW];
     int32_t pad_[3];
-    __device__ __forceinline__ long long cost_at(int j) const { return cost0 + (long long)dc[j]; }
 };
+struct CNode : CNodeHead { CTape tape; };
 constexpr int NODE_HEAD_WORDS = 40, NODE_WORDS = (int)(sizeof(CNode) / 4), NODE_TAPE_WORDS = NODE_WORDS - NODE_HEAD_WORDS;
-static_assert(offsetof(CNode, dc) == 4 * NODE_HEAD_WORDS && sizeof(CNode) % 16 == 0, "CNode layout");
+static_assert(sizeof(CNodeHead) == 4 * NODE_HEAD_WORDS && sizeof(CTape) == 4 * NODE_TAPE_WORDS && sizeof(CNode) % 16 == 0, "CNode layout");
 struct CSearch {
     int32_t threshold, farthest, next_id, best_node, inflight, max_queue, per_size, wo_constraint;
     int32_t windows, cut_windows, expansions, pops_mod;
@@ -83,6 +85,7 @@
     int32_t compound, compound_ok;
     long long gap_ctl_ticks;
     int32_t steps, side_windows, side_expansions, adopted;
+    int32_t tapes_peak, tape_spills;
 #ifdef SP_K8_PF_PROBE
     int32_t pf_win, pf_replay, pf_exp, pf_pad;
     unsigned long long idle_mask;
@@ -1212,25 +1215,32 @@
     return n;
 }
 
-template <int MAXP>
+constexpr int CTL_THREADS = 512;
+constexpr int NSLOT = 8;
+template <int MAXP, int NORD>
 __device__ __forceinline__ void cons_control_body(const ConsBatchT<MAXP>& B) {
     extern __shared__ uint8_t proc[];
     __shared__ uint32_t acc[QE];
     uint32_t (*sv)[CW + 1][5] = reinterpret_cast<uint32_t (*)[CW + 1][5]>(acc);
     uint32_t (*sl)[CW][4] = reinterpret_cast<uint32_t (*)[CW][4]>(acc + QSV);
     uint32_t* sc = acc + QSV + QSL; uint32_t* sr = sc + (CW + 1);
-    __shared__ CNode nh[NQ];
-    __shared__ CWork wks[NWORK];
+    __shared__ CNodeHead nh[NQ];
+    __shared__ CTape tapes[NSLOT];
+    __shared__ int8_t slot_of[NQ], slot_node[NSLOT];
+    __shared__ CWork wks[NORD];
     __shared__ CSearch ss;
-    __shared__ int copy_from[NWORK], copy_len[NWORK], need_la[NWORK], replay_of[NWORK];
+    __shared__ int copy_from[NORD], copy_len[NORD], need_la[NORD], replay_of[NORD];
     struct KidCopy { int from, T, n, nk, dual; int8_t node[4], b0[4], b1[4], sp[4]; uint8_t spec[2][CW]; };
     static_assert(KID_LA_KIDS <= 4, "KidCopy");
-    __shared__ KidCopy kcopy[NWORK];
+    __shared__ KidCopy kcopy[NORD];
+    static_assert(sizeof(uint32_t) * QE + sizeof(CNodeHead) * NQ + sizeof(CTape) * NSLOT + (sizeof(CWork) + sizeof(KidCopy) + 16) * NORD + sizeof(CSearch) + NQ + NSLOT <= 48 * 1024 - 64, "control kernel: static LDS");
+    static_assert(NSLOT <= 8 && NQ <= 64 && NQ < 128, "tape slots: a byte per slot in one 64-bit word, a lane per node");
     const int pi = blockIdx.x;
     const ConsParams P = B.p[pi];
     const int tid = threadIdx.x;
+    const int lane = tid & (SP_WAVE - 1);
     const bool coh = B.sync != nullptr;
-    const int nside = (coh || P.n_blocks > DIRECT_BLOCKS) ? 0 : (B.nside < NWORK - 1 ? B.nside : NWORK - 1);
+    const int nside = (coh || P.n_blocks > DIRECT_BLOCKS) ? 0 : (B.nside < NORD - 1 ? B.nside : NORD - 1);
     const int n_orders = 1 + nside;
     CWork& wk = wks[0];
     const long long tk0 = wall_clock64();
@@ -1238,23 +1248,46 @@
         ((uint32_t*)&nh[x / NODE_HEAD_WORDS])[x % NODE_HEAD_WORDS] = ((const uint32_t*)&P.nodes[x / NODE_HEAD_WORDS])[x % NODE_HEAD_WORDS];
     for (int x = tid; x < n_orders * (int)(sizeof(CWork) / 4); x += blockDim.x) ((uint32_t*)wks)[x] = ((const uint32_t*)P.work)[x];
     for (int x = tid; x < (int)(sizeof(CSearch) / 4); x += blockDim.x) ((uint32_t*)&ss)[x] = ((const uint32_t*)P.srch)[x];
-    const int proc_words = (P.cap + 2 + 3) / 4;
-    for (int x = tid; x < proc_words; x += blockDim.x) ((uint32_t*)proc)[x] = ((const uint32_t*)P.processed)[x];
     for (int x = tid; x < QE; x += blockDim.x) acc[x] = 0;
-    if (tid < NWORK) { copy_from[tid] = -1; copy_len[tid] = 0; need_la[tid] = -1; replay_of[tid] = -1; kcopy[tid].nk = 0; if (tid >= n_orders) wks[tid].mode = M_NONE; }
+    if (tid < NORD) { copy_from[tid] = -1; copy_len[tid] = 0; need_la[tid] = -1; replay_of[tid] = -1; kcopy[tid].nk = 0; if (tid >= n_orders) wks[tid].mode = M_NONE; }
     __syncthreads();
     if (wk.done) return;
-    auto tape_word_used = [](const CNode& x, int w) {
-        if (!x.used) return false;
-        if (w == 0) return true;
-        if (x.n <= 0) return false;
+    int proc_w0 = 0, proc_w1 = 0;
+    {
+        int t_lo = 0x7FFFFFFF, t_hi = -1;
+        if (lane < NQ && nh[lane].used) { t_lo = nh[lane].T + nh[lane].q; t_hi = nh[lane].T; }
+        if (lane >= NQ && lane - NQ < n_orders && wks[lane - NQ].mode != M_NONE) t_lo = t_hi = wks[lane - NQ].T;
+        static_assert(NQ + NWORK <= SP_WAVE, "a lane per node and order");
+#pragma unroll
+        for (int o = 32; o > 0; o >>= 1) { const int a = __shfl_xor(t_lo, o), b = __shfl_xor(t_hi, o); t_lo = a < t_lo ? a : t_lo; t_hi = b > t_hi ? b : t_hi; }
+        if (t_hi >= 0) {
+            const int hi = t_hi + CW + 2 < P.cap + 2 ? t_hi + CW + 2 : P.cap + 2, lo = t_lo < 0 ? 0 : t_lo < hi ? t_lo : hi;
+            proc_w0 = lo / 4; proc_w1 = (hi + 3) / 4;
+        }
+    }
+    for (int x = proc_w0 + tid; x < proc_w1; x += blockDim.x) ((uint32_t*)proc)[x] = ((const uint32_t*)P.processed)[x];
+    auto tape_word_used = [](const CNodeHead& x, int w) {
+        if (!x.used || x.n <= 0 || w == 0) return false;
         if (w < CW + 1) return w <= x.n;
         const int sw = w - (CW + 1);
         return sw < 2 * (CW / 4) && (sw % (CW / 4)) * 4 < x.n;
     };
-    for (int x = tid; x < NQ * NODE_TAPE_WORDS; x += blockDim.x) {
-        const int k = x / NODE_TAPE_WORDS, w = x % NODE_TAPE_WORDS;
-        if (tape_word_used(nh[k], w)) ((uint32_t*)&nh[k])[NODE_HEAD_WORDS + w] = ((const uint32_t*)&P.nodes[k])[NODE_HEAD_WORDS + w];
+    unsigned long long slot_nodes = ~0ull;
+    int n_slots = 0;
+    {
+        const unsigned long long taped = __ballot(lane < NQ && nh[lane].used && nh[lane].n > 0);
+        for (unsigned long long m = taped; m && n_slots < NSLOT; m &= m - 1, ++n_slots)
+            slot_nodes = (slot_nodes & ~(0xFFull << (8 * n_slots))) | ((unsigned long long)__builtin_ctzll(m) << (8 * n_slots));
+        if (tid < NQ) {
+            const int before = __builtin_popcountll(taped & ((1ull << tid) - 1ull));
+            slot_of[tid] = (int8_t)((((taped >> tid) & 1ull) && before < NSLOT) ? before : -1);
+        }
+        if (tid < NSLOT) slot_node[tid] = (int8_t)(tid < n_slots ? (int)((slot_nodes >> (8 * tid)) & 0xFFull) : -1);
+        if (tid == 0) { const int n_taped = __builtin_popcountll(taped); if (n_taped > ss.tapes_peak) ss.tapes_peak = n_taped; ss.tape_spills += n_taped - n_slots; }
+    }
+    for (int x = tid; x < n_slots * NODE_TAPE_WORDS; x += blockDim.x) {
+        const int s = x / NODE_TAPE_WORDS, w = x % NODE_TAPE_WORDS, k = (int)((slot_nodes >> (8 * s)) & 0xFFull);
+        if (tape_word_used(nh[k], w)) ((uint32_t*)&tapes[s])[w] = ((const uint32_t*)&P.nodes[k].tape)[w];
     }
     auto load_votes = [&](const int w) {
         const int mode_in = wks[w].mode, n_in = (mode_in == M_WINDOW || mode_in == M_EXPAND) ? wks[w].n : 0;
@@ -1300,11 +1333,26 @@
             }
         }
     };
-    const int lane = tid & (SP_WAVE - 1);
+    auto tape_dc = [&](const int k, const int j) -> int32_t { const int s = slot_of[k]; return s >= 0 ? tapes[s].dc[j] : P.nodes[k].tape.dc[j]; };
+    auto tape_spec = [&](const int k, const int i, const int j) -> uint8_t { const int s = slot_of[k]; return s >= 0 ? tapes[s].spec[i][j] : P.nodes[k].tape.spec[i][j]; };
+    auto cost_at = [&](const int k, const int j) -> long long { return nh[k].cost0 + (j > 0 ? (long long)tape_dc(k, j) : 0ll); };
+    auto claim_slot = [&](const int k) {
+        if (slot_of[k] < 0) {
+            const int o = lane < NSLOT ? (int)slot_node[lane] : 0;
+            const unsigned long long free_slots = __ballot(lane < NSLOT && (o < 0 || !nh[o].used || nh[o].n <= 0));
+            if (free_slots && lane == 0) {
+                const int s = __builtin_ctzll(free_slots), was = slot_node[s];
+                if (was >= 0) slot_of[was] = -1;
+                slot_node[s] = (int8_t)k; slot_of[k] = (int8_t)s;
+            }
+            if (!free_slots && lane == 0) ss.tape_spills += 1;
+            spw::wave_lds_sync();
+        }
+    };
     auto cands = [&](const uint32_t* w5, int col, int out[4]) { return col_candidates(w5, col, P.cap, P.et, P.min_count, P.min_af, out); };
     auto node_free = [&](int k) {
         const int np = nh[k].pex_n;
-        for (int j = 0; j < np; ++j) { CNode& c = nh[nh[k].pex_kid[j]]; c.used = 0; c.complete = 0; }
+        for (int j = 0; j < np; ++j) { CNodeHead& c = nh[nh[k].pex_kid[j]]; c.used = 0; c.complete = 0; }
         nh[k].pex_n = 0; nh[k].used = 0; nh[k].complete = 0;
     };
     uint8_t* Cb = P.C;
@@ -1327,7 +1375,7 @@
         const int others = __builtin_popcountll(__ballot(lane < NQ && nh[lane].used == 1 && !nh[lane].complete)) - 1 - (kids_wait ? n_kids : 0);
         const int kid_w0 = others <= KID_CALM ? KID_LA : KID_W0;
         if (lane < n_kids) {
-            CNode& c = nh[kid(lane)];
+            CNodeHead& c = nh[kid(lane)];
             c.used = 1; c.id = ss.next_id + lane;
             c.wcap = n_kids <= KID_LA_KIDS ? kid_w0 : WRAMP0;
         }
@@ -1343,7 +1391,7 @@
     };
     struct Plan { int kind, nk, nc0, nc1, cut, L; uint32_t cd0, cd1; bool ends; };
     auto cands_p = [&](const uint32_t* w5, int col, uint32_t& packed) { return col_candidates_packed(w5, col, P.cap, P.et, P.min_count, P.min_af, packed); };
-    auto plan_of = [&](const CNode& x) -> Plan {
+    auto plan_of = [&](const CNodeHead& x) -> Plan {
         Plan p;
         const bool has = x.q > 0 || x.n > 0, stood = !has || (x.a == x.n && x.have_out);
         p.cut = stood ? -1 : x.a;
@@ -1366,9 +1414,9 @@
     };
     auto kids_from_sums = [&](const CWork& w, const int mark, const int L, const long long par_cost, const int my_j, const int s0) {
         if (my_j >= 0) {
-            const CNode& par = nh[w.node];
+            const CNodeHead& par = nh[w.node];
             const int k = my_j;
-            CNode& c = nh[w.kid_node[k]];
+            CNodeHead& c = nh[w.kid_node[k]];
             c.used = mark; c.complete = 0; c.id = 0; c.T = L + 1; c.cur = 0; c.pex_n = 0; c.pex_L = 0;
             c.dual = par.dual || w.kid_split[k]; c.split_at = w.kid_split[k] ? L : par.split_at;
 #pragma unroll
@@ -1381,7 +1429,7 @@
             }
             if (!c.dual) c.stopped[1] = 1;
             c.n = c.a = c.q = 0; c.have_out = 0; c.la_valid = w.n_kids <= KID_LA_KIDS ? 1 : 0; c.wcap = WRAMP0;
-            c.cost0 = par_cost + (long long)sc[s0 + k]; c.dc[0] = 0; c.rest = sr[s0 + k]; c.rest_out = 0;
+            c.cost0 = par_cost + (long long)sc[s0 + k]; c.rest = sr[s0 + k]; c.rest_out = 0;
             for (int i = 0; i < 2; ++i) for (int bq = 0; bq < 5; ++bq) c.ev[i][bq] = sv[i][s0 + k][bq];
         }
         if (w.n_kids <= KID_LA_KIDS) {
@@ -1400,16 +1448,16 @@
         const bool side = w > 0;
         if (mode_in == M_INIT) {
             la_fresh = wo.node;
-            CNode& x = nh[wo.node];
+            CNodeHead& x = nh[wo.node];
             if (lane == 0) {
                 x.used = 1; x.id = ss.next_id++; x.complete = 0; x.T = 0; x.cur = wo.in_slot; x.dual = 0; x.split_at = -1;
                 x.stopped[0] = 0; x.stopped[1] = 1; x.len[0] = x.len[1] = 0; x.n = x.a = x.q = 0; x.have_out = 0; x.la_valid = 1; x.wcap = CW;
-                x.cost0 = 0; x.dc[0] = 0; x.rest = sr[0]; x.rest_out = 0; x.pex_n = 0; x.pex_L = 0;
+                x.cost0 = 0; x.rest = sr[0]; x.rest_out = 0; x.pex_n = 0; x.pex_L = 0;
             }
             if (lane < 10) x.ev[lane / 5][lane % 5] = sv[lane / 5][0][lane % 5];
             for (int y = lane; y < 2 * CW * 4; y += SP_WAVE) P.la[(size_t)wo.node * 2 * CW * 4 + y] = (&sl[0][0][0])[y];
         } else if (mode_in == M_WINDOW) {
-            CNode& x = nh[wo.node];
+            CNodeHead& x = nh[wo.node];
             const int n = n_in, T = wo.T;
             int a = n;
             if (!wo.replay && n > 1) {
@@ -1435,16 +1483,20 @@
                 for (int i = 0; i < 2; ++i) if ((i == 0 || x.dual) && wo.go[i]) put(&Cb[((size_t)wo.node * 2 + i) * P.cs + T + col], wo.spec[i][col], coh);
             }
             if (!wo.replay) {
+                claim_slot(wo.node);
+                const int ts = slot_of[wo.node];
+                CTape* const tp = ts >= 0 ? &tapes[ts] : &P.nodes[wo.node].tape;
                 long long carry = 0;
                 for (int base = 0; base < a; base += SP_WAVE) {
                     const int col = base + lane;
                     long long c = col < a ? (long long)sc[col + 1] : 0;
 #pragma unroll
                     for (int o = 1; o < SP_WAVE; o <<= 1) { const long long up = __shfl_up(c, o); if (lane >= o) c += up; }
-                    if (col < a) x.dc[col + 1] = (int32_t)(carry + c);
+                    if (col < a) tp->dc[col + 1] = (int32_t)(carry + c);
                     carry += __shfl(c, SP_WAVE - 1);
                 }
-                for (int col = lane; col < n; col += SP_WAVE) { x.spec[0][col] = wo.spec[0][col]; x.spec[1][col] = wo.spec[1][col]; }
+                for (int col = lane; col < n; col += SP_WAVE) { tp->spec[0][col] = wo.spec[0][col]; tp->spec[1][col] = wo.spec[1][col]; }
+                if (ts < 0) __threadfence_block();
             }
             if (lane < 10) x.ev[lane / 5][lane % 5] = sv[lane / 5][a][lane % 5];
             if (lane == 0) {
@@ -1477,7 +1529,7 @@
                     }
                 }
                 if (take) {
-                    kids_from_sums(wo, 2, T + n, x.cost_at(n), lane < nk ? my_j : -1, n + 1);
+                    kids_from_sums(wo, 2, T + n, cost_at(wo.node, n), lane < nk ? my_j : -1, n + 1);
                     for (int k = 0; k < nk; ++k) { const int j = __builtin_amdgcn_readlane(my_j, k); if (lane == 0) x.pex_kid[k] = (int8_t)wo.kid_node[j]; }
                     if (lane < wo.n_kids) { bool mine = false; for (int k = 0; k < nk; ++k) mine = mine || __builtin_amdgcn_readlane(my_j, k) == lane; if (!mine) { nh[wo.kid_node[lane]].used = 0; nh[wo.kid_node[lane]].complete = 0; } }
                     if (lane == 0) {
@@ -1496,16 +1548,16 @@
             }
         } else if (mode_in == M_EXPAND) {
 #ifdef SP_K8_TRACE
-            if (lane == 0 && pi == 0) { printf("EXP%s L %d pre %d kids %d parcost %lld :", side ? " (side)" : "", wo.T + n_in, n_in, wo.n_kids, nh[wo.node].cost_at(nh[wo.node].q)); for (int k = 0; k < wo.n_kids; ++k) printf(" [%d/%d sc %u sr %u ev %u %u %u %u %u]", wo.kid_base[k][0], wo.kid_base[k][1], sc[k], sr[k], sv[0][k][0], sv[0][k][1], sv[0][k][2], sv[0][k][3], sv[0][k][4]); printf("\n"); }
-#endif
-            const long long par_cost = nh[wo.node].cost_at(nh[wo.node].q);
+            if (lane == 0 && pi == 0) { printf("EXP%s L %d pre %d kids %d parcost %lld :", side ? " (side)" : "", wo.T + n_in, n_in, wo.n_kids, cost_at(wo.node, nh[wo.node].q)); for (int k = 0; k < wo.n_kids; ++k) printf(" [%d/%d sc %u sr %u ev %u %u %u %u %u]", wo.kid_base[k][0], wo.kid_base[k][1], sc[k], sr[k], sv[0][k][0], sv[0][k][1], sv[0][k][2], sv[0][k][3], sv[0][k][4]); printf("\n"); }
+#endif
+            const long long par_cost = cost_at(wo.node, nh[wo.node].q);
             if (!side) {
                 kids_from_sums(wo, 1, wo.T + n_in, par_cost, lane < wo.n_kids ? lane : -1, 0);
                 adopt(wo.node, wo.n_kids, true, [&](int k) { return (int)wo.kid_node[k]; });
             } else {
                 kids_from_sums(wo, 2, wo.T + n_in, par_cost, lane < wo.n_kids ? lane : -1, 0);
                 if (lane == 0) {
-                    CNode& par = nh[wo.node];
+                    CNodeHead& par = nh[wo.node];
                     par.pex_n = wo.n_kids; par.pex_L = wo.T + n_in;
                     for (int k = 0; k < wo.n_kids; ++k) par.pex_kid[k] = (int8_t)wo.kid_node[k];
                 }
@@ -1557,16 +1609,16 @@
         if (lane == 0) { const int steps_made = wk.pad + 1; for (int w = 0; w < n_orders; ++w) { wks[w].mode = M_NONE; wks[w].n = 0; wks[w].replay = 0; wks[w].n_kids = 0; } wk.pad = steps_made; }
         spw::wave_lds_sync();
         auto act = [&](const int xi, const int w, const Plan& pl, unsigned long long& free_bits) -> int {
-            CNode& x = nh[xi];
+            CNodeHead& x = nh[xi];
             CWork& W = wks[w];
             const bool side = w > 0;
             const int cut = pl.cut;
             if ((x.q > 0 || x.n > 0) && cut < 0) {
                 const int xn = x.n;
                 if (xn > 1) x.wcap = SP_K8_RAMP * x.wcap < CW ? SP_K8_RAMP * x.wcap : CW;
-                const long long c_end = x.cost_at(xn);
+                const long long c_end = cost_at(xi, xn);
                 const int la_ok = x.have_out == 1 ? 1 : 0;
-                x.T += xn; x.cur ^= 1; x.cost0 = c_end; x.dc[0] = 0; x.rest = x.rest_out; x.n = x.a = x.q = 0; x.have_out = 0; x.la_valid = la_ok;
+                x.T += xn; x.cur ^= 1; x.cost0 = c_end; x.rest = x.rest_out; x.n = x.a = x.q = 0; x.have_out = 0; x.la_valid = la_ok;
             }
             const int dual = x.dual, cur = x.cur, split_at = x.split_at, xT = x.T;
             const int pre_go0 = !x.stopped[0] ? 1 : 0, pre_go1 = (dual && !x.stopped[1]) ? 1 : 0;
@@ -1630,7 +1682,7 @@
             int xi = ss.inflight;
             if (xi < 0) {
                 long long kc = 0x7FFFFFFFFFFFFFFFll; int kt = -1, kid = 0x7FFFFFFF, kx = -1;
-                if (lane < NQ && nh[lane].used == 1 && !nh[lane].complete) { const CNode& p = nh[lane]; kc = p.cost_at(p.q); kt = p.T + p.q; kid = p.id; kx = lane; }
+                if (lane < NQ && nh[lane].used == 1 && !nh[lane].complete) { const CNodeHead& p = nh[lane]; kc = cost_at(lane, p.q); kt = p.T + p.q; kid = p.id; kx = lane; }
                 auto less = [](long long c1, int t1, int i1, long long c2, int t2, int i2) { return c1 < c2 || (c1 == c2 && (t1 > t2 || (t1 == t2 && i1 < i2))); };
                 long long bc = kc; int bt = kt, bid = kid, bx = kx;
                 long long sc2 = 0x7FFFFFFFFFFFFFFFll; int st2 = -1, sid2 = 0x7FFFFFFF, sx2 = -1;
@@ -1655,7 +1707,7 @@
                         if (ox >= 0 && (sx2 < 0 || less(oc, ot, oi, sc2, st2, sid2))) { sc2 = oc; st2 = ot; sid2 = oi; sx2 = ox; }
                     }
                 }
-                CNode& x = nh[xi];
+                CNodeHead& x = nh[xi];
                 if (ss.best_node >= 0 && bc >= ss.best_final) { if (lane == 0) wk.done = 1; break; }
                 const int linear0 = x.a - x.q;
                 bool again = false, freed = false;
@@ -1668,7 +1720,7 @@
                     const int want = linear > 0 ? (linear < SP_WAVE ? linear : SP_WAVE) : 1;
                     bool can = lane < want && L + lane >= ss.threshold && proc[L + lane] < ss.per_size && lane <= jc;
                     if (can && (lane > 0 || again)) {
-                        const long long cj = x.cost_at(q + lane);
+                        const long long cj = cost_at(xi, q + lane);
                         can = (sx2 < 0 || less(cj, L + lane, ss.next_id + lane - 1, sc2, st2, sid2)) && !(ss.best_node >= 0 && cj >= ss.best_final);
                     }
                     const unsigned long long no = ~__ballot(can);
@@ -1695,7 +1747,7 @@
             const long long ts1 = wall_clock64(); ts_pick += ts1 - ts0;
 #endif
             {
-                const CNode& x = nh[xi];
+                const CNodeHead& x = nh[xi];
                 if (x.q < x.a) {
                     if (lane == 0) { nh[xi].q += 1; nh[xi].id = ss.next_id++; }
                     spw::wave_lds_sync();
@@ -1727,12 +1779,12 @@
             bool cand = false;
             long long kc = 0x7FFFFFFFFFFFFFFFll; int kt = -1, kid = 0x7FFFFFFF;
             if (lane < NQ && nh[lane].used == 1 && !nh[lane].complete && lane != wk.node && !((main_kids >> lane) & 1ull) && nh[lane].q >= nh[lane].a && nh[lane].pex_n == 0) {
-                const CNode& x = nh[lane];
+                const CNodeHead& x = nh[lane];
                 const int Lq = x.T + x.q;
                 if (Lq >= ss.threshold && Lq < P.cap + 2 && proc[Lq] < ss.per_size) {
                     pl = plan_of(x);
                     cand = !pl.ends && ((pl.kind == 1 && pl.cut < 0) || (pl.kind == 2 && pl.nk <= MAXKIDS));
-                    if (cand) { kc = x.cost_at(x.q); kt = Lq; kid = x.id; }
+                    if (cand) { kc = cost_at(lane, x.q); kt = Lq; kid = x.id; }
                 }
             }
             const unsigned long long cm = __ballot(cand);
@@ -1772,8 +1824,8 @@
         for (int w = 0; w < n_orders; ++w) {
             const int ro = replay_of[w];
             if (ro >= 0) {
-                const CNode& x = nh[ro];
-                for (int jq = lane; jq < x.a; jq += SP_WAVE) { wks[w].spec[0][jq] = x.spec[0][jq]; wks[w].spec[1][jq] = x.spec[1][jq]; }
+                const CNodeHead& x = nh[ro];
+                for (int jq = lane; jq < x.a; jq += SP_WAVE) { wks[w].spec[0][jq] = tape_spec(ro, 0, jq); wks[w].spec[1][jq] = tape_spec(ro, 1, jq); }
             }
         }
 #ifdef SP_K8_PF_PROBE
@@ -1915,21 +1967,21 @@
     __syncthreads();
     for (int x = tid; x < NQ * NODE_HEAD_WORDS; x += blockDim.x)
         put(&((uint32_t*)&P.nodes[x / NODE_HEAD_WORDS])[x % NODE_HEAD_WORDS], ((const uint32_t*)&nh[x / NODE_HEAD_WORDS])[x % NODE_HEAD_WORDS], coh);
-    for (int x = tid; x < NQ * NODE_TAPE_WORDS; x += blockDim.x) {
-        const int k = x / NODE_TAPE_WORDS, w = x % NODE_TAPE_WORDS;
-        if (tape_word_used(nh[k], w)) ((uint32_t*)&P.nodes[k])[NODE_HEAD_WORDS + w] = ((const uint32_t*)&nh[k])[NODE_HEAD_WORDS + w];
+    for (int x = tid; x < NSLOT * NODE_TAPE_WORDS; x += blockDim.x) {
+        const int s = x / NODE_TAPE_WORDS, w = x % NODE_TAPE_WORDS, k = slot_node[s];
+        if (k >= 0 && tape_word_used(nh[k], w)) ((uint32_t*)&P.nodes[k].tape)[w] = ((const uint32_t*)&tapes[s])[w];
     }
     for (int x = tid; x < n_orders * (int)(sizeof(CWork) / 4); x += blockDim.x) put(&((uint32_t*)P.work)[x], ((const uint32_t*)wks)[x], coh);
     for (int x = tid; x < (int)(sizeof(CSearch) / 4); x += blockDim.x) ((uint32_t*)P.srch)[x] = ((const uint32_t*)&ss)[x];
-    for (int x = tid; x < proc_words; x += blockDim.x) ((uint32_t*)P.processed)[x] = ((const uint32_t*)proc)[x];
+    for (int x = proc_w0 + tid; x < proc_w1; x += blockDim.x) ((uint32_t*)P.processed)[x] = ((const uint32_t*)proc)[x];
     if (tid == 0 && B.prog) {
         __hip_atomic_store(B.prog + 2 * pi, (uint32_t)wk.pad, __ATOMIC_RELAXED, __HIP_MEMORY_SCOPE_SYSTEM);
         if (wk.done) __hip_atomic_store(B.prog + 2 * pi + 1, 1u, __ATOMIC_RELAXED, __HIP_MEMORY_SCOPE_SYSTEM);
     }
 }
 
-template <int MAXP>
-__global__ void __launch_bounds__(1024) cons_control_kernel(ConsBatchT<MAXP> B) { cons_control_body<MAXP>(B); }
+template <int MAXP, int NORD>
+__global__ void __launch_bounds__(CTL_THREADS) cons_control_kernel(ConsBatchT<MAXP> B) { cons_control_body<MAXP, NORD>(B); }
 
 constexpr long long PERSIST_TIMEOUT = 400000000ll;
 constexpr double PERSIST_READY_S = 0.5;
@@ -1963,7 +2015,7 @@
 }
 
 template <int MAXP>
-__global__ void __launch_bounds__(1024) cons_control_persist_kernel(ConsBatchT<MAXP> B) {
+__global__ void __launch_bounds__(CTL_THREADS) cons_control_persist_kernel(ConsBatchT<MAXP> B) {
     __shared__ int go_on;
     const int pi = blockIdx.x;
     const uint32_t nb = (uint32_t)B.p[pi].n_blocks;
@@ -1977,7 +2029,7 @@
         __syncthreads();
         if (!go_on) break;
         __builtin_amdgcn_fence(__ATOMIC_ACQUIRE, "agent");
-        cons_control_body<MAXP>(B);
+        cons_control_body<MAXP, 1>(B);
         asm volatile("s_waitcnt vmcnt(0)" ::: "memory");
         __syncthreads();
         const bool done = coh_load(&B.p[pi].work->done) != 0;
@@ -2304,12 +2356,15 @@
     const dim3 grid((uint32_t)n_blocks, (uint32_t)(1 + B.nside)), block(CWAVES * SP_WAVE);
     const bool one_round = n_blocks <= (ctx->num_cus + ctx->num_cus / 4) * (8 / CWAVES);
     size_t proc_lds = ((size_t)max_cap + 2 + 15) & ~(size_t)15;
+    const void* const control_fn = B.nside > 0 ? (const void*)cons_control_kernel<MAXP, NWORK> : (const void*)cons_control_kernel<MAXP, 1>;
     {
         hipFuncAttributes fa;
-        SP_HIP_CHECK(ctx, hipFuncGetAttributes(&fa, (const void*)cons_control_kernel<MAXP>));
-        if (fa.sharedSizeBytes + proc_lds > 160 * 1024) return sp_fail(ctx, SP_ERR_TOO_LONG, "sp_consensus: cap must stay below ~65,000");
-    }
-    SP_HIP_CHECK(ctx, hipFuncSetAttribute((const void*)cons_control_kernel<MAXP>, hipFuncAttributeMaxDynamicSharedMemorySize, (int)proc_lds));
+        SP_HIP_CHECK(ctx, hipFuncGetAttributes(&fa, control_fn));
+        if (persist_rpw) { hipFuncAttributes fp; SP_HIP_CHECK(ctx, hipFuncGetAttributes(&fp, (const void*)cons_control_persist_kernel<MAXP>)); fa.sharedSizeBytes = std::max(fa.sharedSizeBytes, fp.sharedSizeBytes); }
+        if (fa.sharedSizeBytes + proc_lds > 160 * 1024)
+            return sp_fail(ctx, SP_ERR_TOO_LONG, "sp_consensus: cap must stay at or below " + std::to_string((((size_t)160 * 1024 - fa.sharedSizeBytes) & ~(size_t)15) - 1) + " (the control kernel keeps a counter per length in LDS)");
+    }
+    SP_HIP_CHECK(ctx, hipFuncSetAttribute(control_fn, hipFuncAttributeMaxDynamicSharedMemorySize, (int)proc_lds));
     uint64_t pairs = 0;
     bool persist_ran = false;
     hm.mark("host:k8_prologue");
@@ -2340,7 +2395,7 @@
             { void* dp = nullptr; SP_HIP_CHECK(ctx, hipHostGetDevicePointer(&dp, h_ready, 0)); B.ready = (uint32_t*)dp; }
             B.step_cap = (uint32_t)std::min<uint64_t>(limit, 0xFFFFFFFFull);
             auto drain = [&]() { (void)hipStreamSynchronize(ctx->ctl_stream); if (own_step_stream) (void)hipStreamSynchronize(step_st); (void)hipStreamSynchronize(st); };
-            hipLaunchKernelGGL(cons_control_persist_kernel<MAXP>, dim3(n_prob), dim3(1024), proc_lds, ctx->ctl_stream, B);
+            hipLaunchKernelGGL(cons_control_persist_kernel<MAXP>, dim3(n_prob), dim3(CTL_THREADS), proc_lds, ctx->ctl_stream, B);
             bool all_ready = true;
             {
                 const auto t_wait = std::chrono::steady_clock::now();
@@ -2386,7 +2441,8 @@
             if (one_round) hipLaunchKernelGGL(cons_step_wide_kernel<MAXP>, grid, block, 0, st, B);
             else hipLaunchKernelGGL(cons_step_kernel<MAXP>, grid, block, 0, st, B);
             if (need_reduce) hipLaunchKernelGGL(cons_reduce_kernel<MAXP>, dim3((uint32_t)n_clusters * RSLICES), dim3(512), 0, st, B);
-            hipLaunchKernelGGL(cons_control_kernel<MAXP>, dim3(n_prob), dim3(1024), proc_lds, st, B);
+            if (B.nside > 0) hipLaunchKernelGGL((cons_control_kernel<MAXP, NWORK>), dim3(n_prob), dim3(CTL_THREADS), proc_lds, st, B);
+            else hipLaunchKernelGGL((cons_control_kernel<MAXP, 1>), dim3(n_prob), dim3(CTL_THREADS), proc_lds, st, B);
             t_launch += std::chrono::duration<double, std::milli>(std::chrono::steady_clock::now() - tl0).count();
             ++pairs;
             uint64_t spins = 0;
@@ -2456,6 +2512,8 @@
         for (uint32_t p = 0; p < n_prob; ++p) {
             ctx->prof["cons_side_windows"].cells += (uint64_t)h_srch[p].side_windows; ctx->prof["cons_side_expansions"].cells += (uint64_t)h_srch[p].side_expansions;
             ctx->prof["cons_adopted"].cells += (uint64_t)h_srch[p].adopted;
+            ctx->prof["cons_tape_spills"].cells += (uint64_t)h_srch[p].tape_spills;
+            ctx->prof["cons_tapes_peak"].cells = std::max<uint64_t>(ctx->prof["cons_tapes_peak"].cells, (uint64_t)h_srch[p].tapes_peak);
             ctx->prof["cons_compound"].cells += (uint64_t)h_srch[p].compound; ctx->prof["cons_compound_ok"].cells += (uint64_t)h_srch[p].compound_ok;
         }
 #ifdef SP_K8_PF_PROBE
```
